# Aseeef/seq-align-gpu

Measured on AMD Instinct MI355X. Metric: GCUPS (DP cell updates/s) at 1/2/4/8 MI355X; bit-exact max scores vs CPU ref, higher is better.
Workload: dtype f16

## Files before the change

seq-align-gpu_amd/__init__.py:

```python
import ctypes as C
import os

import numpy as np

_HERE = os.path.dirname(os.path.abspath(__file__))
LIB_PATH = os.path.join(_HERE, "libswg.so")
DATA_DIR = os.path.join(_HERE, "data")
CLI_PATH = os.path.join(_HERE, "bin", "smith_waterman")

if not os.path.exists(LIB_PATH):
    raise ImportError(
        "libswg.so is not built: run `python seq-align-gpu_amd/build.py` "
        "(or __graft_entry__.build()); there is no Python/CPU fallback")

lib = C.CDLL(LIB_PATH, mode=C.RTLD_GLOBAL)

SWG_OK, SWG_ERR_ARG, SWG_ERR_HIP, SWG_ERR_NOMEM = 0, -1, -2, -3
SWG_ERR_STATE, SWG_ERR_RESIDUE, SWG_ERR_IO, SWG_ERR_NODEVICE = -4, -5, -6, -7

ABI_SYMBOLS = [
    "swg_create", "swg_destroy", "swg_last_error", "swg_global_error", "swg_abi_version", "swg_prune_last",
    "swg_set_option", "swg_set_scoring", "swg_set_query", "swg_set_query_pssm", "swg_db_pack", "swg_db_pack_shard", "swg_db_pack_shards", "swg_db_upload", "swg_db_view",
    "swg_db_free", "swg_db_save", "swg_db_load", "swg_db_count", "swg_db_total_count", "swg_db_residues",
    "swg_db_packed_bytes", "swg_db_order", "swg_search", "swg_search_begin", "swg_search_end", "swg_search_multi",
# ... 215 lines not shown
_sig("swg_synth_db_shard", C.c_int, [C.c_uint64, C.c_size_t, C.c_double, C.c_double, C.c_uint32, C.c_uint32,
                                     _vp, C.c_size_t, C.c_double, C.c_double, C.c_int, C.c_int,
                                     C.POINTER(_vp), C.POINTER(_vp), C.POINTER(_vp), C.POINTER(C.c_size_t),
                                     C.POINTER(C.c_uint64), C.POINTER(C.c_size_t)])
_sig("swg_synth_free", None, [_vp])
_sig("swg_pssm_load", C.c_int, [C.c_char_p, C.POINTER(Scoring), C.POINTER(_vp), C.POINTER(_vp), C.POINTER(C.c_size_t),
                                C.c_char_p, C.c_size_t])
_sig("swg_pssm_free", None, [_vp, _vp])
_sig("swg_debug_fail_alloc", None, [C.c_int])
_sig("swg_align_stats", C.c_int, [_vp, _vp, _vp, C.c_size_t, _vp, _vp])
_sig("swg_align_stats_multi", C.c_int, [_vp, _vp, _vp, _vp, C.c_size_t, _vp, C.c_size_t, _vp, _vp, _vp])
_sig("swg_align_stats_multi_pssm", C.c_int, [_vp, _vp, _vp, _vp, C.c_size_t, _vp, C.c_size_t, _vp, _vp, _vp])
_sig("swg_debug_bounds_last", C.c_int, [_vp, _vp])
_sig("swg_debug_sort_count", C.c_ulong, [])
_sig("swg_debug_engine", C.c_int, [_vp, C.c_size_t, C.c_int, C.c_int, _vp])
_sig("swg_debug_plan", C.c_int, [_vp, C.c_size_t, C.c_int, _vp])
_sig("swg_debug_plan_f16", C.c_int, [_vp, C.c_size_t, C.c_int, C.c_long, _vp])
_sig("swg_debug_plan_gapless", C.c_int, [_vp, C.c_size_t, C.c_int, _vp])
_sig("swg_debug_plan_forced", C.c_int, [_vp, C.c_size_t, C.c_int, C.c_long, C.c_long, C.c_long, C.c_int, C.c_long, C.c_int, _vp])
_sig("swg_debug_plan_streams", C.c_int, [_vp, _vp, _vp, C.c_size_t, C.c_int, C.c_long, C.c_long, C.c_long, C.c_long, _vp])
_sig("swg_debug_plan_systolic", C.c_int, [_vp, _vp, _vp, C.c_size_t, C.c_int, C.c_int, C.c_int, C.c_long, C.c_long, C.c_long, C.c_long, C.c_long, _vp])
_sig("swg_debug_systolic_variants", C.c_int, [C.c_int, _vp, C.c_size_t])
_sig("swg_debug_plan_batch", C.c_int, [_vp, C.c_size_t, C.c_size_t, C.c_int, C.c_int, C.c_int, C.c_long, C.c_long, C.c_long, _vp])
_sig("swg_debug_plan_lists", C.c_int, [_vp, C.c_size_t, C.c_size_t, C.c_int, C.c_int, C.c_long, C.c_long, C.c_long, _vp])
_sig("swg_debug_launch_log", None, [C.c_int])
_sig("swg_debug_launch_log_read", C.c_size_t, [_vp, C.c_size_t])
_sig("swg_debug_split", C.c_int, [_vp, C.c_size_t, C.c_uint64, _vp])
_sig("swg_debug_list_plan", C.c_int, [C.c_size_t, C.c_uint32, C.c_int, _vp, _vp])
_sig("swg_debug_pair_tokens", C.c_int, [_vp, _vp, C.c_int, _vp, C.c_size_t, C.POINTER(C.c_size_t)])
_sig("swg_debug_view_ranks", C.c_int, [_vp, _vp, C.c_size_t, _vp, C.POINTER(C.c_size_t)])
_sig("swg_debug_list_jobs", C.c_int, [_vp, _vp, _vp, C.c_size_t, _vp, C.c_size_t, C.POINTER(C.c_size_t), _vp])
_sig("swg_prune_last", C.c_int, [_vp, _vp])
_sig("swg_debug_prune_bound", C.c_int, [_vp, _vp, C.c_size_t, _vp, _vp, C.c_size_t, _vp, _vp])
_sig("swg_debug_prune_plan", C.c_int, [_vp, _vp])
_sig("swg_debug_prune_plan_above", C.c_int, [_vp, _vp])
_sig("swg_debug_above_multi_route", C.c_int, [C.c_long, C.c_int, C.c_int])
_sig("swg_debug_prune_stages", C.c_int, [_vp, _vp, C.c_size_t, C.POINTER(C.c_size_t)])
_sig("swg_debug_prune_kmer", C.c_int, [_vp, _vp, C.c_size_t, C.c_int, C.c_int, C.c_int, _vp, _vp, C.c_size_t, _vp, _vp])
_sig("swg_debug_prune_kmer_choice", C.c_int, [_vp, _vp])
_sig("swg_debug_prune_kmer_read", C.c_int, [_vp, _vp, C.c_int, _vp, _vp, C.c_size_t, _vp])
_sig("swg_debug_prune_kmer_seg", C.c_int, [_vp, _vp, C.c_size_t, C.c_int, C.c_int, C.c_int, C.c_int, _vp, _vp, C.c_size_t, _vp, _vp])
_sig("swg_debug_prune_kmer_choice_seg", C.c_int, [_vp, _vp])
_sig("swg_debug_prune_kmer_seg_read", C.c_int, [_vp, _vp, C.c_int, C.c_int, _vp, _vp, C.c_size_t, _vp])
_sig("swg_debug_prune_kmer_refine", C.c_int, [_vp, _vp, C.c_size_t, C.c_int, C.c_int, C.c_int, _vp, _vp, C.c_size_t, _vp, _vp])
_sig("swg_debug_prune_refine_choice", C.c_int, [_vp, _vp])
_sig("swg_debug_prune_refine_read", C.c_int, [_vp, _vp, C.c_int, _vp, _vp, _vp, C.c_size_t, _vp, C.c_size_t, _vp])
_sig("swg_debug_prune_stages3", C.c_int, [_vp, _vp, C.c_size_t, C.POINTER(C.c_size_t)])
_sig("swg_debug_prune_kmer_refine3", C.c_int, [_vp, _vp, C.c_size_t, C.c_int, C.c_int, C.c_int, _vp, _vp, C.c_size_t, _vp, _vp])
_sig("swg_debug_prune_refine3_choice", C.c_int, [_vp, _vp])
_sig("swg_debug_prune_kmer_refine4", C.c_int, [_vp, _vp, C.c_size_t, C.c_int, C.c_int, C.c_int, _vp, _vp, C.c_size_t, _vp])
_sig("swg_debug_prune_table_bits", C.c_int, [_vp, _vp, C.c_size_t, C.c_int])
_sig("swg_debug_prune_tables", C.c_int, [_vp, _vp])
_sig("swg_debug_prune_tables4", C.c_int, [_vp, _vp])
_sig("swg_debug_prune_refine4_read", C.c_int, [_vp, _vp, C.c_size_t, _vp])
_sig("swg_debug_prune_refine4_choice", C.c_int, [_vp, _vp])
_sig("swg_debug_prune_gate_choice", C.c_int, [_vp, _vp])
_sig("swg_debug_prune_gate", C.c_int, [_vp, _vp])
_sig("swg_debug_prune_stages5", C.c_int, [_vp, _vp, C.c_size_t, _vp])
_sig("swg_debug_prune_stages4", C.c_int, [_vp, _vp, C.c_size_t, C.POINTER(C.c_size_t)])
_sig("swg_debug_list_deal", C.c_int, [_vp, _vp, _vp, C.c_size_t, C.c_uint64, C.c_uint64, _vp, C.c_size_t, C.POINTER(C.c_size_t)])
_sig("swg_debug_calib_iters", C.c_int, [_vp, _vp, C.c_size_t, C.POINTER(C.c_size_t)])
_sig("swg_db_composition", C.c_int, [_vp, _vp, _vp])
_sig("swg_calibrate", C.c_int, [_vp, _vp, C.c_int, _vp])
_sig("swg_calibrate_multi", C.c_int, [_vp, _vp, _vp, C.c_size_t, _vp, C.c_int, _vp])
_sig("swg_calibrate_multi_pssm", C.c_int, [_vp, _vp, _vp, C.c_size_t, _vp, C.c_int, _vp])
_sig("swg_evalue", C.c_double, [_vp, C.c_uint64, C.c_int32])
_sig("swg_bitscore", C.c_double, [_vp, C.c_int32])
_sig("swg_evalue_min_score", C.c_int32, [_vp, C.c_uint64, C.c_double])
_sig("swg_synth_db_iid", C.c_int, [C.c_uint64, C.c_size_t, C.c_uint32, _vp, C.POINTER(_vp), C.POINTER(_vp)])
_sig("swg_gumbel_fit_hist", C.c_int, [_vp, C.c_size_t, C.POINTER(C.c_double), C.POINTER(C.c_double), C.POINTER(C.c_int)])
_sig("swg_matrix_lambda", C.c_int, [_vp, _vp, C.POINTER(C.c_double)])
_sig("swg_pssm_from_paths", C.c_int, [_vp, _vp, C.c_double, _vp, C.c_size_t, _vp, _vp, _vp, _vp, C.c_size_t, C.c_size_t, _vp, _vp, _vp])
_sig("swg_pssm_save", C.c_int, [C.c_char_p, _vp, _vp, C.c_size_t])
_sig("swg_pssm_build", C.c_int, [_vp, _vp, _vp, C.c_size_t, _vp, _vp, C.c_double, _vp, _vp, _vp])
_sig("swg_pssm_build_multi", C.c_int, [_vp, _vp, _vp, _vp, C.c_size_t, _vp, C.c_size_t, _vp, _vp, C.c_double, _vp, _vp, _vp])
_sig("swg_pssm_build_multi_pssm", C.c_int, [_vp, _vp, _vp, _vp, _vp, C.c_size_t, _vp, C.c_size_t, _vp, _vp, C.c_double, _vp, _vp, _vp])
_sig("swg_mask_params_default", None, [_vp])
_sig("swg_mask_tables", C.c_int, [_vp, _vp, C.POINTER(C.c_int64), C.POINTER(C.c_int64)])
_sig("swg_seg_mask", C.c_int, [_vp, C.c_size_t, _vp, _vp, C.POINTER(C.c_size_t)])
_sig("swg_seg_mask_segments", C.c_int, [_vp, C.c_size_t, _vp, _vp, C.POINTER(C.c_size_t), C.POINTER(C.c_size_t)])
_sig("swg_seg_mask_flat", C.c_int, [_vp, _vp, C.c_size_t, _vp, _vp])
_sig("swg_db_sequence", C.c_int, [_vp, C.c_uint32, _vp, C.c_size_t, C.POINTER(C.c_size_t)])
_sig("swg_db_mask", C.c_int, [_vp, _vp, _vp, C.POINTER(_vp)])
_sig("swg_db_mask_info", C.c_int, [_vp, _vp])
_sig("swg_debug_mask_fail_alloc", None, [C.c_int])


def _check(rc, ctx=None):
    if rc != SWG_OK:
        msg = lib.swg_last_error(ctx) if ctx else lib.swg_global_error()
        raise SwgError(rc, (msg or b"").decode("utf-8", "replace"))


def _i8(a):
    a = np.ascontiguousarray(a, dtype=np.int8)
    return a, a.ctypes.data_as(_vp)


def _pssm(pssm):
    a = np.asarray(pssm)
    if a.ndim != 2 or a.shape[1] != 32:
        raise ValueError("a PSSM is an (lq, 32) array, got shape %s" % (a.shape,))
    if a.dtype != np.int8 and a.size and (a.min() < -128 or a.max() > 127):
        raise ValueError("PSSM values must fit int8")
    p, pp = _i8(a)
    return p, pp, a.shape[0]
# ... 274 lines not shown


def debug_prune_kmer_choice(forced=0, pruned=1, lq=3000, pair_rows=1900000000, table_rate=0, fill_rate=0):
    a = np.array([forced, pruned, lq, pair_rows, table_rate, fill_rate], dtype=np.int64)
    out = np.zeros(1, dtype=np.int64)
    _check(lib.swg_debug_prune_kmer_choice(a.ctypes.data_as(_vp), out.ctypes.data_as(_vp)))
    return int(out[0])


KMER_MAX_SEGMENTS = 32
KMER_TABLE_BUDGET = 96 << 20


def debug_prune_kmer_seg(rows, query, gap_open, gap_extend, k, segments, flat, offsets, table=True):
    S = int(segments)
    return _prune_kmer_mirror(lib.swg_debug_prune_kmer_seg, rows, query, gap_open, gap_extend, (int(k), S), flat, offsets,
                              (KMER_CLASSES ** int(k), S) if table and k in (4, 5) and 1 <= S <= KMER_MAX_SEGMENTS else None)


def debug_prune_kmer_choice_seg(forced=0, segments=0, pruned=1, lq=3000, pair_rows=1900000000, table_rate=0, fill_rate=0):
    a = np.array([forced, pruned, lq, pair_rows, table_rate, fill_rate, segments], dtype=np.int64)
    out = np.zeros(4, dtype=np.int64)
    _check(lib.swg_debug_prune_kmer_choice_seg(a.ctypes.data_as(_vp), out.ctypes.data_as(_vp)))
    return int(out[0]), int(out[1]), int(out[2]), bool(out[3])


KMER_REFINE_SEGMENTS = 128
KMER_REFINE3_SEGMENTS = 256


def debug_prune_kmer_refine(rows, query, gap_open, gap_extend, segments, flat, offsets, table=True):
    S = int(segments)
    hook = lib.swg_debug_prune_kmer_refine3 if S == KMER_REFINE3_SEGMENTS else lib.swg_debug_prune_kmer_refine
    return _prune_kmer_mirror(hook, rows, query, gap_open, gap_extend, (S,), flat, offsets,
                              (KMER_CLASSES ** 4, S) if table and S in (32, 64, 128, 256) else None)


def debug_prune_kmer_refine4(rows, query, gap_open, gap_extend, segments, flat, offsets):
    r, rp = _i8(rows)
    lq = r.size // 32
    qp = None
    if query is not None:
        q, qp = _i8(query)
        lq = q.size
    f, fp = _i8(flat)
    off = np.ascontiguousarray(offsets, dtype=np.uint64)
    n = off.size - 1
    u = np.zeros(max(n, 1), dtype=np.uint64)
    _check(lib.swg_debug_prune_kmer_refine4(rp, qp, lq, int(gap_open), int(gap_extend), int(segments), fp, off.ctypes.data_as(_vp), n,
                                            u.ctypes.data_as(_vp)))
    return u[:n]


def debug_prune_table_bits(rows, query, k=4):
    r, rp = _i8(rows)
    lq = r.size // 32
    qp = None
    if query is not None:
        q, qp = _i8(query)
        lq = q.size
    rc = lib.swg_debug_prune_table_bits(rp, qp, lq, int(k))
    if rc < 0:
        _check(rc)
    return rc


def debug_prune_refine3_choice(forced=0, segments=0, refine=0, refine3=0, table_bits=8, pruned=1, lq=3000, pair_rows=1900000000,
                               table_rate=0, fill_rate=0):
    a = np.array([forced, pruned, lq, pair_rows, table_rate, fill_rate, segments, refine, refine3, table_bits], dtype=np.int64)
    out = np.zeros(4, dtype=np.int64)
    _check(lib.swg_debug_prune_refine3_choice(a.ctypes.data_as(_vp), out.ctypes.data_as(_vp)))
    return int(out[0]), int(out[1]), int(out[2]), int(out[3])


KMER_REFINE4_SEGMENTS = 256
PRUNE_REFINE4_FORCED = 5256


def debug_prune_refine4_choice(forced=0, segments=0, refine=0, refine3=0, refine4=0, table_bits=8, table_bits5=8, pruned=1, lq=3000,
                               pair_rows=1900000000, table_rate=0, fill_rate=0):
    a = np.array([forced, pruned, lq, pair_rows, table_rate, fill_rate, segments, refine, refine3, table_bits, refine4, table_bits5], dtype=np.int64)
    out = np.zeros(5, dtype=np.int64)
    _check(lib.swg_debug_prune_refine4_choice(a.ctypes.data_as(_vp), out.ctypes.data_as(_vp)))
    return tuple(int(v) for v in out)


def debug_prune_gate_choice(forced=0, segments=0, gate=0, pruned=1, lq=3000, pair_rows=1900000000, table_rate=0, fill_rate=0):
    a = np.array([forced, pruned, lq, pair_rows, table_rate, fill_rate, segments, 0, gate], dtype=np.int64)
    out = np.zeros(3, dtype=np.int64)
    _check(lib.swg_debug_prune_gate_choice(a.ctypes.data_as(_vp), out.ctypes.data_as(_vp)))
    return int(out[0]), int(out[1]), bool(out[2])


def debug_prune_refine_choice(forced=0, segments=0, refine=0, pruned=1, lq=3000, pair_rows=1900000000, table_rate=0, fill_rate=0):
    a = np.array([forced, pruned, lq, pair_rows, table_rate, fill_rate, segments, refine], dtype=np.int64)
    out = np.zeros(3, dtype=np.int64)
    _check(lib.swg_debug_prune_refine_choice(a.ctypes.data_as(_vp), out.ctypes.data_as(_vp)))
    return int(out[0]), int(out[1]), int(out[2])


def prune_list(bounds, begin, end, threshold):
    b = np.asarray(bounds)[begin:end]
    return (begin + np.nonzero(b >= threshold)[0]).astype(np.uint32)


PRUNE_PLAN_KEYS = ("mode", "k", "want_scores", "gap_open", "gap_extend", "bits", "use_diag", "n_classes", "work_queue", "both_forms",
                   "gapless", "batch", "range_pairs", "groups", "prune_head", "n_segments")


def debug_prune_plan(**ask):
    d = dict(mode=1, k=100, want_scores=0, gap_open=-2, gap_extend=-1, bits=16, use_diag=1, n_classes=1, work_queue=1, both_forms=0,
             gapless=0, batch=0, range_pairs=1000000, groups=1024, prune_head=4, n_segments=8)
    unknown = set(ask) - set(d)
    if unknown:
        raise TypeError("debug_prune_plan: unknown arguments %s" % sorted(unknown))
    d.update(ask)
    a = np.array([int(d[k]) for k in PRUNE_PLAN_KEYS], dtype=np.int64)
    out = np.zeros(2, dtype=np.int64)
    _check(lib.swg_debug_prune_plan(a.ctypes.data_as(_vp), out.ctypes.data_as(_vp)))
    return bool(out[0]), int(out[1])


PRUNE_PLAN_ABOVE_KEYS = ("mode", "gap_open", "gap_extend", "bits", "use_diag", "n_classes", "work_queue", "both_forms", "gapless", "batch",
                         "range_pairs", "groups", "n_segments", "prune_head")


def debug_prune_plan_above(**ask):
    d = dict(mode=1, gap_open=-2, gap_extend=-1, bits=16, use_diag=1, n_classes=1, work_queue=1, both_forms=0, gapless=0, batch=0,
             range_pairs=1000000, groups=1024, n_segments=8, prune_head=4)
    unknown = set(ask) - set(d)
    if unknown:
        raise TypeError("debug_prune_plan_above: unknown arguments %s" % sorted(unknown))
    d.update(ask)
    a = np.array([int(d[k]) for k in PRUNE_PLAN_ABOVE_KEYS], dtype=np.int64)
    out = np.zeros(2, dtype=np.int64)
    _check(lib.swg_debug_prune_plan_above(a.ctypes.data_as(_vp), out.ctypes.data_as(_vp)))
    return bool(out[0]), int(out[1])


def debug_above_multi_route(option=0, admitted=True, single_pruned=False):
    rc = lib.swg_debug_above_multi_route(int(option), 1 if admitted else 0, 1 if single_pruned else 0)
    if rc < 0:
        _check(rc)
    return rc


PRUNE_STAGE_QUEUED = ("threshold", "prefix_cut", "gate", "refine", "list")
_PRUNE_STAGE_BITS = ((0, "threshold"), (7, "bound"), (1, "prefix_cut"), (2, "gate"), (3, "refine"), (5, "refine3"), (6, "refine4"), (4, "list"))


def debug_prune_stages(segments, head_pairs=0, fixed=False, refine=0, prefix_cut=False, refine3=0, refine4=0, gate=False):
    head = [head_pairs, fixed, refine, prefix_cut, refine3, refine4] + ([1] if gate else [])
    a = np.array(head + [len(segments)] + [int(v) for sg in segments for v in sg], dtype=np.int64)
    out = np.zeros((2 * len(segments) + 1, 4), dtype=np.int64)
    n = C.c_size_t(0)
    hook = lib.swg_debug_prune_stages5 if gate else lib.swg_debug_prune_stages4
    _check(hook(a.ctypes.data_as(_vp), out.ctypes.data_as(_vp), out.shape[0], C.byref(n)))
    return [(int(b), int(e), int(sg), tuple(name for i, name in _PRUNE_STAGE_BITS if int(qd) >> i & 1))
            for b, e, sg, qd in out[:n.value]]


LAUNCH_FAMILIES = ("dyn", "lists", "q32", "qq", "streams", "systolic")


def debug_systolic_variants(bits):
    out = np.zeros((16, 2), dtype=np.int32)
    n = lib.swg_debug_systolic_variants(bits, out.ctypes.data_as(_vp), 16)
    assert 0 < n <= 16
    return [(int(k), int(w)) for k, w in out[:n]]


def debug_launch_log(on):
    lib.swg_debug_launch_log(1 if on else 0)


def debug_launch_log_read():
    seen = lib.swg_debug_launch_log_read(None, 0)
    out = np.zeros((max(seen, 1), 10), dtype=np.int32)
    lib.swg_debug_launch_log_read(out.ctypes.data_as(_vp), seen)
    kept = int(np.count_nonzero(out[:seen, 1]))
    if kept < seen:
        raise SwgError(SWG_ERR_STATE, "launch log: %d launches, %d kept" % (seen, kept))
    keys = ("family", "K", "G", "W", "form", "edges", "flag", "workgroups", "grid_rows", "list")
    recs = []
    for row in out[:seen]:
        r = dict(zip(keys, (int(v) for v in row)))
        r["family"] = LAUNCH_FAMILIES[r["family"]]
        r["fma"] = r["exact"] = r.pop("flag")
        recs.append(r)
    return recs


def synth_query(seed, lq):
    out = np.empty(lq, dtype=np.int8)
    lib.swg_synth_query(seed, lq, out.ctypes.data_as(_vp))
    return out


def hit_key(score, index):
    return int(lib.swg_hit_key(int(score), int(index)))


def key_hit(key):
    h = Hit()
    lib.swg_key_hit(int(key), C.byref(h))
    return int(h.score), int(h.index)


def topk_merge_keys(keys, k):
# ... 632 lines not shown
        t = np.zeros(KMER_CLASSES ** int(k), dtype=np.uint16) if k else None
        n = 0
        if bounds:
            _check(lib.swg_debug_prune_kmer_read(self.handle, db.handle, 0, None, None, 0, info.ctypes.data_as(_vp)), self.handle)
            n = int(info[2])
        b = np.zeros(max(n, 1), dtype=np.uint32) if bounds else None
        _check(lib.swg_debug_prune_kmer_read(self.handle, db.handle, int(k or 0), t.ctypes.data_as(_vp) if t is not None else None,
                                             b.ctypes.data_as(_vp) if b is not None else None, n, info.ctypes.data_as(_vp)), self.handle)
        return {"k": int(info[0]), "builds": int(info[1]), "pairs": int(info[2]), "table": t, "bounds": None if b is None else b[:int(info[2])]}

    def debug_prune_kmer_seg_read(self, db, k=None, segments=1, bounds=False):
        info = np.zeros(4, dtype=np.uint64)
        S = int(segments)
        t = np.zeros((KMER_CLASSES ** int(k), S), dtype=np.uint16) if k else None
        n = 0
        if bounds:
            _check(lib.swg_debug_prune_kmer_seg_read(self.handle, db.handle, 0, 0, None, None, 0, info.ctypes.data_as(_vp)), self.handle)
            n = int(info[2])
        b = np.zeros(max(n, 1), dtype=np.uint32) if bounds else None
        _check(lib.swg_debug_prune_kmer_seg_read(self.handle, db.handle, int(k or 0), S, t.ctypes.data_as(_vp) if t is not None else None,
                                                 b.ctypes.data_as(_vp) if b is not None else None, n, info.ctypes.data_as(_vp)), self.handle)
        return {"k": int(info[0]), "builds": int(info[1]), "pairs": int(info[2]), "segments": int(info[3]), "table": t,
                "bounds": None if b is None else b[:int(info[2])]}

    def debug_prune_refine_read(self, db, segments=None, arrays=True):
        info = np.zeros(7, dtype=np.uint64)
        _check(lib.swg_debug_prune_refine_read(self.handle, db.handle, 0, None, None, None, 0, None, 0, info.ctypes.data_as(_vp)), self.handle)
        n = int(info[2])
        if not arrays:
            return {"k": int(info[0]), "builds": int(info[1]), "pairs": n, "segments": int(info[3]), "refine": int(info[4]),
                    "refine_builds": int(info[5]), "table": None, "bounds": None, "stages": []}
        S = int(segments or 0)
        t = np.zeros((KMER_CLASSES ** 4, S), dtype=np.uint16) if S else None
        b = np.zeros(max(n, 1), dtype=np.uint32)
        l = np.zeros(max(n, 1), dtype=np.uint32)
        st = np.zeros((256, 4), dtype=np.uint32)
        _check(lib.swg_debug_prune_refine_read(self.handle, db.handle, S, t.ctypes.data_as(_vp) if t is not None else None, b.ctypes.data_as(_vp),
                                               l.ctypes.data_as(_vp), n, st.ctypes.data_as(_vp), 256, info.ctypes.data_as(_vp)), self.handle)
        stages = [(int(r[0]), int(r[1]), int(r[2]), l[int(r[0]):int(r[0]) + int(r[3])].copy()) for r in st[:int(info[6])]]
        return {"k": int(info[0]), "builds": int(info[1]), "pairs": n, "segments": int(info[3]), "refine": int(info[4]),
                "refine_builds": int(info[5]), "table": t, "bounds": b[:n], "stages": stages}

    def debug_prune_tables(self):
        out = np.zeros(7, dtype=np.int64)
        _check(lib.swg_debug_prune_tables(self.handle, out.ctypes.data_as(_vp)), self.handle)
        return {"refine3": int(out[0]), "refine3_builds": int(out[1]),
                "bits": dict(zip(("first4", "first5", "second", "third"), (int(v) for v in out[2:6]))), "auto_bits": int(out[6])}

    def debug_prune_tables4(self):
        out = np.zeros(4, dtype=np.int64)
        _check(lib.swg_debug_prune_tables4(self.handle, out.ctypes.data_as(_vp)), self.handle)
        return {"refine4": int(out[0]), "refine4_builds": int(out[1]), "bits": int(out[2]), "refused": bool(out[3])}

    def debug_prune_gate(self):
        out = np.zeros(1, dtype=np.int64)
        _check(lib.swg_debug_prune_gate(self.handle, out.ctypes.data_as(_vp)), self.handle)
        return bool(out[0])

    def debug_prune_refine4_read(self, blocks):
        b = np.ascontiguousarray(blocks, dtype=np.uint32)
        out = np.zeros((max(b.size, 1), KMER_REFINE4_SEGMENTS), dtype=np.uint16)
        _check(lib.swg_debug_prune_refine4_read(self.handle, b.ctypes.data_as(_vp), b.size, out.ctypes.data_as(_vp)), self.handle)
        return out[:b.size]

    def debug_bounds_last(self):
        out = np.zeros(4, dtype=np.uint32)
        _check(lib.swg_debug_bounds_last(self.handle, out.ctypes.data_as(_vp)), self.handle)
        return dict(zip(("kernel_pairs", "fallback_pairs", "launches", "column_limit"), (int(v) for v in out)))

    def _align_multi(self, fn, db, qflat, qoff, hits, want_ops, ops_stride, bounds=False, stats=False):
        nq = len(qoff) - 1
        if len(hits) != nq:
            raise ValueError("hits: %d rows for %d queries" % (len(hits), nq))
        k = max((len(row) for row in hits), default=0)
        arr = (Hit * max(nq * k, 1))()
        nh = (C.c_size_t * max(nq, 1))()
        for i, row in enumerate(hits):
            nh[i] = len(row)
            for j, (sc, ix) in enumerate(row):
                arr[i * k + j].score, arr[i * k + j].index = int(sc), int(ix)
        out = (Alignment * max(nq * k, 1))()
        stride = 0 if bounds else int(ops_stride if ops_stride is not None else
                                      lib.swg_align_ops_bound_multi(db.handle, qoff.ctypes.data_as(_vp), nq))
        ops = C.create_string_buffer(max(1, nq * k * stride)) if want_ops else None
        args = (self.handle, db.handle, qflat.ctypes.data_as(_vp), qoff.ctypes.data_as(_vp), nq, C.cast(arr, _vp), k,
                C.cast(nh, _vp), C.cast(out, _vp))
        if stats:
            cnt = (AlignCounts * max(nq * k, 1))()
            _check(fn(*args, C.cast(cnt, _vp)), self.handle)
            return [[self._stats_dict(out[i * k + j], cnt[i * k + j]) for j in range(len(row))] for i, row in enumerate(hits)]
        _check(fn(*args) if bounds else fn(*args, C.cast(ops, _vp) if want_ops else None, stride), self.handle)
        raw = ops.raw if want_ops else None
        res = []
        for i, row in enumerate(hits):
            r = []
            for j in range(len(row)):
                h = i * k + j
                a = {f: int(getattr(out[h], f)) for f, _ in Alignment._fields_ if f != "reserved"}
                if want_ops:
                    a["ops"] = raw[h * stride:h * stride + a["n_ops"]].decode()
                r.append(a)
            res.append(r)
        return res

    @staticmethod
    def _hit_keys(hits, k, n):
# ... 118 lines not shown
```

seq-align-gpu_amd/csrc/swg_api.cpp:

```cpp
#include "swg_host_internal.h"
#include "../../include/swg_host.h"

#include <algorithm>
#include <atomic>
#include <chrono>
#include <climits>
#include <cmath>
#include <cstdarg>
#include <cstdio>
#include <cstdlib>
#include <cstring>
#include <new>
#include <vector>

static thread_local std::string g_err;
static std::atomic<uint64_t> g_epoch{1};

int swg_set_global_error(int code, const char *fmt, ...)
{
    char buf[512];
    va_list ap;
    va_start(ap, fmt);
    vsnprintf(buf, sizeof buf, fmt, ap);
    va_end(ap);
// ... 139 lines not shown
    const bool timing = getenv("SWG_TIMING") != nullptr;
    clk::time_point tp = clk::now();
    auto lap = [&](const char *what) {
        if (!timing) return;
        const clk::time_point t = clk::now();
        fprintf(stderr, "[swg_create] %-44s %8.2f ms\n", what, std::chrono::duration<double, std::milli>(t - tp).count());
        tp = t;
    };
    if (timing) fprintf(stderr, "[swg_create] %-44s %8.2f ms\n", "hipGetDeviceCount (HIP runtime start-up)", std::chrono::duration<double, std::milli>(tp - t_enter).count());
    int rc = [&]() -> int {
        HIP_TRY(ctx, hipSetDevice(dev));
        hipDeviceProp_t prop;
        HIP_TRY(ctx, hipGetDeviceProperties(&prop, dev));
        ctx->n_cu = prop.multiProcessorCount;
        lap("hipSetDevice + device properties");
        HIP_TRY(ctx, hipStreamCreateWithFlags(&ctx->stream, hipStreamNonBlocking));
        lap("the fill stream");
        const int rs = ensure_slot(ctx, &ctx->slots[0]);
        if (rs != SWG_OK) return rs;
        lap("events + pinned buffers of one search slot");
        ctx->cur = &ctx->slots[0];
        HIP_TRY(ctx, hipMalloc(&ctx->d_sub, 32 * 32));
        lap("first device allocation");
        if (timing) {
            HIP_TRY(ctx, swg_launch_zero2(ctx->d_sub, 16, reinterpret_cast<uint8_t *>(ctx->d_sub) + 16, 16, ctx->stream));
            HIP_TRY(ctx, hipStreamSynchronize(ctx->stream));
            lap("first kernel launch (code object load)");
        }
        return SWG_OK;
    }();
    if (rc != SWG_OK) {
        g_err = ctx->err;
        swg_destroy(ctx);
        return rc;
    }
    *out = ctx;
    return SWG_OK;
}

extern "C" void swg_destroy(swg_ctx *ctx)
{
    if (!ctx) return;
    (void)hipSetDevice(ctx->device);
    if (ctx->stream) (void)hipStreamSynchronize(ctx->stream);
    (void)hipFree(ctx->d_sub);
    (void)hipFree(ctx->d_query);
    (void)hipFree(ctx->d_pssm);
    (void)hipFree(ctx->d_kmer_cprof);
    (void)hipFree(ctx->kmer_first[0].d);
    (void)hipFree(ctx->kmer_first[1].d);
    (void)hipFree(ctx->kmer_second.d);
    (void)hipFree(ctx->kmer_third.d);
    (void)hipFree(ctx->kmer_fourth.d);
    (void)hipFree(ctx->d_profile[0]);
    (void)hipFree(ctx->d_profile[1]);
    (void)hipFree(ctx->d_profile[2]);
    (void)hipFree(ctx->d_profile[3]);
    (void)hipFree(ctx->d_profile[4]);
    (void)hipFree(ctx->d_profile[5]);
    (void)hipFree(ctx->d_profile[6]);
    (void)hipFree(ctx->d_profile[7]);
    (void)hipFree(ctx->d_scratch);
    for (SwgSlot &sl : ctx->slots) {
        for (auto &ev : sl.ev)
            if (ev) (void)hipEventDestroy(ev);
        if (sl.ev_done) (void)hipEventDestroy(sl.ev_done);
        (void)hipHostFree(sl.h_cand);
        (void)hipHostFree(sl.h_counters);
        (void)hipHostFree(sl.h_scores);
    }
    if (ctx->b16.db) swg_db_free(ctx->b16.db);
    if (ctx->calib.db) swg_db_free(ctx->calib.db);
    (void)hipHostFree(ctx->b16.h_stage);
    (void)hipHostFree(ctx->b16.h_meta);
    (void)hipFree(ctx->b16.d_stage);
    (void)hipFree(ctx->b16.d_pair_src);
    (void)hipFree(ctx->b16.d_pair_len);
    for (int i = 0; i < 4; ++i) {
        (void)hipHostFree(ctx->h_query_stage[i]);
        if (ctx->ev_query_stage[i]) (void)hipEventDestroy(ctx->ev_query_stage[i]);
    }
    if (ctx->stream2) (void)hipStreamDestroy(ctx->stream2);
    if (ctx->stream3) (void)hipStreamDestroy(ctx->stream3);
    if (ctx->stream) (void)hipStreamDestroy(ctx->stream);
    delete ctx;
}

extern "C" int swg_set_option(swg_ctx *ctx, const char *key, long value)
{
    if (!ctx || !key) return swg_set_ctx_error(ctx, SWG_ERR_ARG, "swg_set_option: NULL argument");
    if (!strcmp(key, "force_bits")) {
        if (value != 0 && value != 16 && value != 32)
            return swg_set_ctx_error(ctx, SWG_ERR_ARG, "force_bits must be 0, 16 or 32");
        ctx->opt_force_bits = value;
    } else if (!strcmp(key, "cols_per_wave")) {
        ctx->opt_cols = value;
    } else if (!strcmp(key, "max_waves")) {
        if (value < 0 || value > 16) return swg_set_ctx_error(ctx, SWG_ERR_ARG, "max_waves must be 0..16");
        ctx->opt_max_waves = value;
    } else if (!strcmp(key, "engine")) {
        if (value < 0 || value > 2) return swg_set_ctx_error(ctx, SWG_ERR_ARG, "engine must be 0 (auto), 1 (systolic) or 2 (diagonal)");
        ctx->opt_engine = value;
    } else if (!strcmp(key, "group_lanes")) {
        if (value != 0 && value != 16 && value != 32 && value != 64)
            return swg_set_ctx_error(ctx, SWG_ERR_ARG, "group_lanes must be 0, 16, 32 or 64");
        ctx->opt_group = value;
// ... 10 lines not shown
    } else if (!strcmp(key, "wide16")) {
        ctx->opt_wide = value != 0;
    } else if (!strcmp(key, "f16")) {
        if (value < 0 || value > 2) return swg_set_ctx_error(ctx, SWG_ERR_ARG, "f16 must be 0 (off), 1 (auto) or 2 (whenever the gap scores allow)");
        ctx->opt_f16 = value;
    } else if (!strcmp(key, "f16_pair")) {
        if (value < 0 || value > 2)
            return swg_set_ctx_error(ctx, SWG_ERR_ARG, "f16_pair must be 0 (auto), 1 (v_perm_b32) or 2 (v_pk_fma_f16 wherever it fits)");
        ctx->opt_f16_pair = value;
    } else if (!strcmp(key, "bounds_groups")) {
        if (value < 0) return swg_set_ctx_error(ctx, SWG_ERR_ARG, "bounds_groups must be 0 (auto) or the most lane groups of a bounds launch");
        ctx->opt_bounds_groups = value;
    } else if (!strcmp(key, "last_pass")) {
        ctx->opt_last_pass = value != 0;
    } else if (!strcmp(key, "qq")) {
        ctx->opt_qq = value != 0;
    } else if (!strcmp(key, "batch_geometry")) {
        if (value != 0 && value != 1)
            return swg_set_ctx_error(ctx, SWG_ERR_ARG, "batch_geometry must be 0 (a forced geometry sends a batch one by one) or 1 (the batch takes it)");
        ctx->opt_batch_geometry = value;
    } else if (!strcmp(key, "long_helps")) {
        ctx->opt_long_helps = value != 0;
    } else if (!strcmp(key, "segment_blocks")) {
        if (value < 0 || value > (long)SWG_DYN_SEG_BLOCKS)
            return swg_set_ctx_error(ctx, SWG_ERR_ARG, "segment_blocks must be 0 (default) .. 2^26-64");
        ctx->opt_seg_blocks = value ? (uint32_t)value : SWG_DYN_SEG_BLOCKS;
    } else if (!strcmp(key, "prune")) {
        if (value < 0 || value > 2)
            return swg_set_ctx_error(ctx, SWG_ERR_ARG, "prune must be 0 (off), 1 (auto) or 2 (wherever it is structurally possible: diagnostic)");
        ctx->opt_prune = value;
    } else if (!strcmp(key, "prune_head")) {
        if (value < 0 || value > 4096) return swg_set_ctx_error(ctx, SWG_ERR_ARG, "prune_head must be 0..4096 (pairs per lane group)");
        ctx->opt_prune_head = value;
    } else if (!strcmp(key, "prune_kmer")) {
        if (value != 0 && value != 1 && value != 4 && value != 5)
            return swg_set_ctx_error(ctx, SWG_ERR_ARG, "prune_kmer must be 0 (auto), 1 (the colmax bound), 4 or 5 (the k-mer bound of that k)");
        ctx->opt_prune_kmer = value;
    } else if (!strcmp(key, "prune_segments")) {
        if (value < 0 || value > (long)SWG_KMER_MAX_SEGMENTS)
            return swg_set_ctx_error(ctx, SWG_ERR_ARG, "prune_segments must be 0 (auto) or 1..32 (the segments of the k-mer bound's table; 1: unsegmented)");
        ctx->opt_prune_segments = value;
    } else if (!strcmp(key, "prune_refine")) {
        if (!swg_prune_refine_value_ok(value))
            return swg_set_ctx_error(ctx, SWG_ERR_ARG, "prune_refine must be 0 (auto), 1 (off), 64 or 128 (the segments of the second-level bound's table)");
        ctx->opt_prune_refine = value;
    } else if (!strcmp(key, "prune_refine3")) {
        if (!swg_prune_refine3_value_ok(value))
            return swg_set_ctx_error(ctx, SWG_ERR_ARG, "prune_refine3 must be 0 (auto), 1 (off) or 256 (the segments of the third-level bound's table)");
        ctx->opt_prune_refine3 = value;
    } else if (!strcmp(key, "prune_refine4")) {
        if (!swg_prune_refine4_value_ok(value))
            return swg_set_ctx_error(ctx, SWG_ERR_ARG, "prune_refine4 must be 0 (auto), 1 (off) or 5256 (the fourth-level bound's table: k = 5 in 256 segments)");
        ctx->opt_prune_refine4 = value;
    } else if (!strcmp(key, "prune_gate")) {
        if (!swg_prune_gate_value_ok(value))
            return swg_set_ctx_error(ctx, SWG_ERR_ARG, "prune_gate must be 0 (auto), 1 (off) or 2 (wherever the first-level bound is a segmented k-mer bound)");
        ctx->opt_prune_gate = value;
    } else if (!strcmp(key, "prune_table_bits")) {
        if (value != 0 && value != 16)
            return swg_set_ctx_error(ctx, SWG_ERR_ARG, "prune_table_bits must be 0 (auto: bytes where they hold every entry) or 16");
        ctx->opt_prune_table_bits = value;
    } else if (!strcmp(key, "prune_cut")) {
        if (value != 0 && value != 1)
            return swg_set_ctx_error(ctx, SWG_ERR_ARG, "prune_cut must be 0 (a stage's pairs are cut one by one) or 1 (the prefix of the length order)");
        ctx->opt_prune_cut = value;
    } else if (!strcmp(key, "above_batch")) {
        if (value < 0 || value > 2)
            return swg_set_ctx_error(ctx, SWG_ERR_ARG, "above_batch must be 0 (auto), 1 (one launch wherever the batch is admitted) or 2 (one query after another)");
        ctx->opt_above_batch = value;
    } else if (!strcmp(key, "calib_seqs")) {
        if (value < 2 || value > (1l << 20)) return swg_set_ctx_error(ctx, SWG_ERR_ARG, "calib_seqs must be 2..1048576 (random sequences a calibration scores)");
        ctx->opt_calib_seqs = value;
    } else if (!strcmp(key, "pssm_msa_mb")) {
        if (value < 0 || value > 65536) return swg_set_ctx_error(ctx, SWG_ERR_ARG, "pssm_msa_mb must be 0..65536 (MiB of device rows one group of queries of swg_pssm_build* may take; 0: every query alone)");
        ctx->opt_pssm_msa_mb = value;
    } else if (!strcmp(key, "calib_len")) {
        if (value < 8 || value > (1l << 14)) return swg_set_ctx_error(ctx, SWG_ERR_ARG, "calib_len must be 8..16384 (residues of a calibration's random sequences)");
        ctx->opt_calib_len = value;
    } else if (!strcmp(key, "calib_seed")) {
        if (value < 0) return swg_set_ctx_error(ctx, SWG_ERR_ARG, "calib_seed must be >= 0");
        ctx->opt_calib_seed = value;
    } else if (!strcmp(key, "q32_waves")) {
        ctx->opt_q32_waves = value;
    } else if (!strcmp(key, "wave_budget")) {
        ctx->opt_wave_budget = value;
    } else if (!strcmp(key, "batch")) {
        if (value < 0 || value > 8) return swg_set_ctx_error(ctx, SWG_ERR_ARG, "batch must be 0..8 (pairs one queue request claims; 0 and 1: one)");
        ctx->opt_batch = value;
    } else if (!strcmp(key, "batch_blocks")) {
        if (value < 0) return swg_set_ctx_error(ctx, SWG_ERR_ARG, "batch_blocks must be >= 0 (token blocks; 0: from the geometry)");
        ctx->opt_batch_blocks = value;
    } else if (!strcmp(key, "work_queue")) {
        ctx->opt_dynamic = value != 0;
    } else if (!strcmp(key, "prio_share")) {
        if (value < 0) return swg_set_ctx_error(ctx, SWG_ERR_ARG, "prio_share must be >= 0 (percent)");
        ctx->opt_prio_share = value;
    } else if (!strcmp(key, "long_split")) {
        if (value < -1) return swg_set_ctx_error(ctx, SWG_ERR_ARG, "long_split must be -1 (off), 0 (auto) or a row count");
        ctx->opt_long_split = value;
    } else if (!strcmp(key, "workgroups")) {
        if (value < 0) return swg_set_ctx_error(ctx, SWG_ERR_ARG, "workgroups must be >= 0");
        ctx->opt_workgroups = value;
    } else {
        return swg_set_ctx_error(ctx, SWG_ERR_ARG, "swg_set_option: unknown key '%s'", key);
    }
    return SWG_OK;
// ... 734 lines not shown
    if (F->cut) {
        q.q2_begin = q.q2_end = 0;
        q.queue2 = nullptr;
    }
    return SWG_OK;
}

static int enqueue_pruned_fill(swg_ctx *ctx, swg_db *db, const SwgPrunePlan &pr, size_t k, DynFill *F)
{
    const SwgPairTokens &T = db->ptok;
    const SwgDiagPlan &pl = F->wk.plan[F->c];
    hipStream_t qs = F->qs;
    uint32_t *thr = db->d_counters + SWG_PRUNE_WORD_T, *cut_word = db->d_counters + SWG_PRUNE_WORD_CUT, *gate = db->d_counters + SWG_PRUNE_WORD_GATE;
    const uint32_t n_pairs = (uint32_t)swg_db_pair_count(db);
    const SwgPruneLayout L = swg_prune_layout(db->d_pair_bound, n_pairs);
    if (pr.fixed) HIP_TRY(ctx, hipMemsetD32Async(reinterpret_cast<hipDeviceptr_t>(thr), (int)pr.fixed_T, 1, qs));
    const std::vector<SwgPruneStage> stages = swg_prune_stages(pr, F->segs);
    auto first_level = [&](uint32_t b, uint32_t en, const uint32_t *gated_by) -> int {
        if (pr.kmer > 1 && pr.segments > 1)
            HIP_TRY(ctx, swg_launch_pair_bound_kmer_seg(T.d_tok, T.d_pair_off, b, en, pr.kmer, (uint32_t)pr.segments, ctx->prune_colmax, ctx->kmer_first[pr.kmer - 4].d,
                                                        ctx->kmer_first[pr.kmer - 4].bits, gated_by, L.bounds, L.ids, qs));
        else if (pr.kmer > 1)
            HIP_TRY(ctx, swg_launch_pair_bound_kmer(T.d_tok, T.d_pair_off, en, pr.kmer, ctx->prune_colmax, ctx->kmer_first[pr.kmer - 4].d,
                                                    ctx->kmer_first[pr.kmer - 4].bits, L.bounds, L.ids, qs));
        else
            HIP_TRY(ctx, swg_launch_pair_bound(T.d_tok, T.d_pair_off, en, ctx->prune_colmax, L.bounds, L.ids, qs));
        return SWG_OK;
    };
    const SwgPruneBoundRange br = swg_prune_bound_range(stages, n_pairs);
    if (br.stage == stages.size()) {
        const int rc = first_level(br.begin, br.end, nullptr);
        if (rc != SWG_OK) return rc;
    } else if (br.skip_end > br.skip_begin)
        HIP_TRY(ctx, hipMemsetD32Async(reinterpret_cast<hipDeviceptr_t>(L.bounds + br.skip_begin), (int)SWG_PRUNE_NOT_BOUNDED, br.skip_end - br.skip_begin, qs));
    db->prune_stages.clear();
    for (const SwgPruneStage &st : stages) {
        if (st.queued & SWG_STAGE_THRESHOLD)
            HIP_TRY(ctx, swg_launch_prune_threshold(db->d_scores, db->d_order, (uint32_t)((size_t)db->n_bins * SWG_BIN), (uint32_t)k, db->d_hist, thr, qs));
        if (st.queued & SWG_STAGE_BOUND) {
            const int rc = first_level(br.begin, br.end, thr);
            if (rc != SWG_OK) return rc;
        }
        if (st.queued & SWG_STAGE_PREFIX_CUT) HIP_TRY(ctx, swg_launch_prune_cut(L.bounds, T.d_pair_off, st.begin, st.end, thr, cut_word, qs));
        if (st.queued & SWG_STAGE_GATE) HIP_TRY(ctx, swg_launch_prune_refine_gate(L.bounds, st.begin, st.end, thr, gate, qs));
        if (st.queued & SWG_STAGE_REFINE)
            HIP_TRY(ctx, swg_launch_pair_bound_refine(T.d_tok, T.d_pair_off, st.begin, st.end, (uint32_t)pr.refine, ctx->prune_colmax, ctx->kmer_second.d,
                                                      ctx->kmer_second.bits, st.queued & SWG_STAGE_GATE ? gate : thr, L.bounds, qs));
        if (st.queued & SWG_STAGE_REFINE3)
            HIP_TRY(ctx, swg_launch_pair_bound_refine(T.d_tok, T.d_pair_off, st.begin, st.end, (uint32_t)pr.refine3, ctx->prune_colmax, ctx->kmer_third.d,
                                                      ctx->kmer_third.bits, st.queued & SWG_STAGE_GATE ? gate : thr, L.bounds, qs));
        if (st.queued & SWG_STAGE_REFINE4)
            HIP_TRY(ctx, swg_launch_pair_bound_refine(T.d_tok, T.d_pair_off, st.begin, st.end, (uint32_t)pr.refine4, ctx->prune_colmax, ctx->kmer_fourth.d,
                                                      ctx->kmer_fourth.bits, st.queued & SWG_STAGE_GATE ? gate : thr, L.bounds, qs, 5));
        if (st.queued & SWG_STAGE_LIST) {
            const size_t rec = db->prune_stages.size() / 2;
            HIP_TRY(ctx, swg_launch_prune_list(L.bounds, T.d_pair_off, st.begin, st.end, thr, L.tiles, L.lists + st.begin, cut_word,
                                               rec < SWG_PRUNE_STAGE_RECS ? L.recs + 2 * rec : nullptr, qs));
            db->prune_stages.push_back(st.begin), db->prune_stages.push_back(st.end);
        }
        F->q.list = st.queued & SWG_STAGE_PREFIX_CUT ? L.ids + st.begin : st.queued & SWG_STAGE_LIST ? L.lists + st.begin : nullptr;
        F->q.list_count = F->q.list ? cut_word : nullptr;
        for (int pass = 0; pass < pl.npass; ++pass) {
            const int rc = F->launch(pass, F->segs[st.segment], st.begin, st.end, F->form, ctx->d_profile[diag_profile_slot(pl, F->c)], false);
            if (rc != SWG_OK) return rc;
        }
    }
    F->q.list = nullptr, F->q.list_count = nullptr;
    return SWG_OK;
}

static int launch_diag(swg_ctx *ctx, swg_db *db, const SwgDiagWork &wk, int go, int ge, bool *two_ends,
                       const SwgPrunePlan *prune = nullptr, size_t prune_k = 0)
{
    hipStream_t s = ctx->stream;
    *two_ends = false;
    static const char *trace_path = getenv("SWG_TRACE");
    uint64_t *d_trace[2] = {nullptr, nullptr};
    if (trace_path)
        for (int c = 0; c < wk.n_classes; ++c) {
            const size_t bytes = (size_t)wk.plan[c].workgroups * wk.plan[c].W * 4 * 8;
            HIP_TRY(ctx, hipMalloc(&d_trace[c], bytes));
            HIP_TRY(ctx, hipMemsetAsync(d_trace[c], 0, bytes, s));
        }
    HIP_TRY(ctx, hipEventRecord(ctx->cur->ev[1], s));
    int rf = fork_long_class(ctx, wk);
    if (rf != SWG_OK) return rf;
    for (int c = wk.n_classes - 1; c >= 0; --c) {
        const SwgDiagLayout &L = db->diag[c];
        const SwgDiagPlan &pl = wk.plan[c];
        if (diag_class_is_dynamic(ctx, db, pl)) {
            DynFill F{ctx, db, wk, c};
            int rc = dyn_fill_begin(&F, go, ge, d_trace[c]);
            if (rc != SWG_OK) return rc;
            const uint32_t class_begin = F.q.q_begin, class_end = F.q.q_end;
            const bool split = c == 0 && wk.n_classes == 1 && F.form != 2 && pl.f16_from > class_begin && pl.f16_from < class_end;
            const bool pruned = prune && prune->on && c == 0 && wk.n_classes == 1 && !split && db->d_pair_bound;
            if (c == 0) ctx->cur->pruned = pruned;
            if (pruned) {
                if ((rc = enqueue_pruned_fill(ctx, db, *prune, prune_k, &F)) != SWG_OK) return rc;
            } else
            for (int part = 0; part < (split ? 2 : 1); ++part) {
                const int pform = split && part == 1 ? 2 : F.form;
                const uint32_t part_begin = split && part == 1 ? pl.f16_from : class_begin;
                const uint32_t part_end = split && part == 0 ? pl.f16_from : class_end;
                const uint8_t *prof = ctx->d_profile[split && part == 1 ? 7 : diag_profile_slot(pl, c)];
                F.q.go = gap_word(pform, go);
// ... 823 lines not shown
{
    P->prune = SwgPrunePlan();
    if (!P->use_diag || P->bits != 16) return SWG_OK;
    const SwgDiagWork &wk = P->wk;
    const SwgDiagPlan &pl = wk.plan[0];
    SwgPruneAsk a;
    a.mode = (int)ctx->opt_prune;
    a.k = k;
    a.want_scores = want_scores;
    a.gap_open = ctx->gap_open;
    a.gap_extend = ctx->gap_extend;
    a.bits = P->bits;
    a.use_diag = P->use_diag;
    a.n_classes = wk.n_classes;
    a.work_queue = diag_class_is_dynamic(ctx, db, pl) && db->ptok.ok;
    a.both_forms = P->split_at != 0u;
    a.gapless = P->gapless;
    a.batch = ctx->in_batch;
    a.prune_head = ctx->opt_prune_head;
    a.fixed = ctx->above_min > 0;
    if (a.mode == 0 || !a.work_queue || wk.n_classes != 1) return SWG_OK;
    a.range_pairs = wk.pair_end[0] - wk.pair_begin[0];
    a.groups = diag_class_streams(ctx, db, wk, 0);
    const int form = diag_class_form(ctx, db, pl);
    std::vector<std::pair<uint32_t, uint32_t>> segs;
    bool cut = false;
    if (!token_segments(db->ptok, (uint32_t)wk.pair_begin[0], (uint32_t)wk.pair_end[0], ctx->opt_seg_blocks, pl.npass > 1 || form == 1, &segs, &cut))
        return SWG_OK;
    a.n_segments = segs.size();
    P->prune = swg_prune_plan(a);
    ctx->prune_choice = SwgPruneChoice();
    if (!P->prune.on) return SWG_OK;
    P->prune.fixed_T = P->prune.fixed ? (uint32_t)ctx->above_min : 0u;
    SwgKmerAsk ka;
    ka.forced = ctx->opt_prune_kmer;
    ka.forced_segments = ctx->opt_prune_segments;
    ka.forced_refine = ctx->opt_prune_refine;
    ka.forced_refine3 = ctx->opt_prune_refine3;
    ka.forced_refine4 = ctx->opt_prune_refine4;
    ensure_prune_colmax(ctx);
    ka.table_bits = kmer_table_bits(ctx, 4);
    ka.table_bits5 = kmer_table_bits(ctx, 5);
    ka.pruned = true;
    ka.lq = ctx->query_len();
    ka.pair_rows = 4ull * (db->ptok.pair_blocks_prefix[wk.pair_end[0]] - db->ptok.pair_blocks_prefix[wk.pair_begin[0]]);
    ka.fill_rate = swg_kmer_fill_rate(ka.lq);
    P->prune.kmer = swg_prune_kmer_choice(ka, &P->prune.segments);
    P->prune.prefix_cut = ctx->opt_prune_cut == 1 && !P->prune.fixed;
    P->prune.refine = P->prune.prefix_cut ? 0 : swg_prune_refine_choice(ka, P->prune.kmer, P->prune.segments);
    P->prune.refine3 = P->prune.prefix_cut ? 0 : swg_prune_refine3_choice(ka, P->prune.kmer, P->prune.segments, P->prune.refine);
    P->prune.refine4 = P->prune.prefix_cut || ctx->kmer_fourth_refused
                           ? 0
                           : swg_prune_refine4_choice(ka, P->prune.kmer, P->prune.segments, P->prune.refine, P->prune.refine3);
    ka.forced_gate = ctx->opt_prune_gate;
    P->prune.gate = !P->prune.prefix_cut && swg_prune_gate_choice(ka, P->prune.kmer, P->prune.segments);
    ctx->prune_choice = SwgPruneChoice{P->prune.kmer, P->prune.segments, P->prune.refine, P->prune.refine3, P->prune.refine4, P->prune.gate ? 1 : 0};
    return SWG_OK;
}

static int ensure_kmer_table(swg_ctx *ctx, SwgKmerTable *t, int k, int S)
{
    const int bits = kmer_table_bits(ctx, k);
    if (t->holds(ctx->epoch, k, S, bits)) return SWG_OK;
    const size_t lq = ctx->query_len();
    int rc;
    if ((rc = device_grow(ctx, &ctx->d_kmer_cprof, &ctx->d_kmer_cprof_cap, lq * 32)) != SWG_OK) return rc;
    const size_t bytes = (size_t)swg_kmer_entries(k) * (size_t)S * (size_t)(bits / 8);
    if (t->cap < bytes) t->epoch = 0;
    if ((rc = device_grow(ctx, &t->d, &t->cap, bytes)) != SWG_OK) return rc;
    const long go = (long)ctx->gap_open + ctx->gap_extend, ge = ctx->gap_extend;
    HIP_TRY(ctx, swg_launch_kmer_table(ctx->d_sub, ctx->d_query, ctx->query_pssm ? ctx->d_pssm : nullptr, (uint32_t)lq, (uint32_t)-go, (uint32_t)-ge, k,
                                       (uint32_t)S, ctx->d_kmer_cprof, t->d, bits, ctx->stream));
    t->epoch = ctx->epoch, t->k = k, t->segments = S, t->bits = bits;
    ++(t == &ctx->kmer_fourth  ? ctx->kmer_refine4_builds
       : t == &ctx->kmer_third ? ctx->kmer_refine3_builds
       : t == &ctx->kmer_second ? ctx->kmer_refine_builds
                                : ctx->kmer_builds);
    return SWG_OK;
}

static bool reserve_kmer_fourth(swg_ctx *ctx)
{
    SwgKmerTable *t = &ctx->kmer_fourth;
    const size_t bytes = (size_t)swg_kmer_entries(5) * SWG_KMER_REFINE4_SEGMENTS;
    if (t->d && t->cap >= bytes) return true;
    (void)hipFree(t->d);
    t->d = nullptr, t->cap = 0, t->epoch = 0;
    uint8_t *d = nullptr;
    if (hipSetDevice(ctx->device) != hipSuccess || hipMalloc(&d, bytes) != hipSuccess) {
        (void)hipGetLastError();
        ctx->kmer_fourth_refused = true;
        return false;
    }
    t->d = d, t->cap = bytes;
    return true;
}

static int prepare_prune(swg_ctx *ctx, swg_db *db, const SwgPrunePlan &pr)
{
    int rc;
    ensure_prune_colmax(ctx);
    if (pr.kmer > 1) {
        const int k = pr.kmer, S = pr.segments;
        if (S < 1 || S > (int)SWG_KMER_MAX_SEGMENTS) return swg_set_ctx_error(ctx, SWG_ERR_ARG, "the k-mer bound's table: %d segments (1..32)", S);
        if (!swg_kmer_table_admitted(k, S))
            return swg_set_ctx_error(ctx, SWG_ERR_ARG, "the k-mer bound's table of k = %d in %d segments is %zu MB: above its budget of %zu MB (prune_kmer, prune_segments)", k,
                                     S, (size_t)swg_kmer_entries(k) * (size_t)S * sizeof(uint16_t) >> 20, (size_t)(SWG_KMER_TABLE_BUDGET >> 20));
        if ((rc = ensure_kmer_table(ctx, &ctx->kmer_first[k - 4], k, S)) != SWG_OK) return rc;
    }
    if (pr.refine) {
        if (pr.refine != 64 && pr.refine != 128) return swg_set_ctx_error(ctx, SWG_ERR_ARG, "the second-level bound's table: %d segments (64 or 128)", pr.refine);
        if ((rc = ensure_kmer_table(ctx, &ctx->kmer_second, 4, pr.refine)) != SWG_OK) return rc;
    }
    if (pr.refine3) {
        if (pr.refine3 != 256) return swg_set_ctx_error(ctx, SWG_ERR_ARG, "the third-level bound's table: %d segments (256)", pr.refine3);
        if ((rc = ensure_kmer_table(ctx, &ctx->kmer_third, 4, pr.refine3)) != SWG_OK) return rc;
    }
    if (pr.refine4) {
        if (pr.refine4 != (int)SWG_KMER_REFINE4_SEGMENTS || !swg_kmer_refine4_admitted(kmer_table_bits(ctx, 5)))
            return swg_set_ctx_error(ctx, SWG_ERR_ARG, "the fourth-level bound's table: %d segments (256) of bytes", pr.refine4);
        if ((rc = ensure_kmer_table(ctx, &ctx->kmer_fourth, 5, pr.refine4)) != SWG_OK) return rc;
    }
    swg_db::Bufs &b = db->bufs[ctx->cur - ctx->slots];
    const size_t n_pairs = (size_t)swg_db_pair_count(db);
    if ((rc = device_grow(ctx, &b.d_pair_bound, &b.pair_bound_cap, n_pairs, swg_prune_layout(b.d_pair_bound, n_pairs).words - n_pairs)) != SWG_OK) return rc;
    db->d_pair_bound = b.d_pair_bound;
    return SWG_OK;
}

static int prepare_search(swg_ctx *ctx, swg_db *db, const SwgSearchPlan &P)
{
    int rc = SWG_OK;
    const bool systolic_fill = !P.use_diag && !P.use_q32 && !(P.bits == 32 && P.use_diag32);
    const bool systolic_rescore = P.may_saturate && !P.use_diag32;
    const size_t bin32_scratch = P.bin32 && P.npass32 > 1 ? ((size_t)db->max_nblk * 4 + 4) * 4 * 16 * (size_t)ctx->n_cu : 0;
    if (P.bin32) {
        rc = ensure_profile_cols(ctx, 1, (uint32_t)(P.npass32 * 64 * SWG_DIAG32_K), 4, (1ull << 30) ^ (uint64_t)P.npass32);
        if (rc != SWG_OK) return rc;
        if ((rc = ensure_scratch(ctx, bin32_scratch)) != SWG_OK) return rc;
    }
    if (P.use_diag) {
        if ((rc = prepare_diag(ctx, db, P.wk)) == SWG_OK && P.prune.on) rc = prepare_prune(ctx, db, P.prune);
    } else if (systolic_fill) rc = ensure_profile(ctx, P.main_pl);
    if (rc != SWG_OK) return rc;
    if (systolic_rescore && (rc = ensure_profile(ctx, P.re_pl)) != SWG_OK) return rc;
    size_t need = bin32_scratch;
    if (systolic_fill && P.main_pl.npass > 1)
        need = std::max(need, (size_t)P.main_pl.workgroups * db->max_nblk * SWG_ROWS_PER_BLK * 64 * P.main_pl.info.nb);
    if (systolic_rescore && P.re_pl.npass > 1)
        need = std::max(need, (size_t)P.re_pl.workgroups * db->max_nblk * SWG_ROWS_PER_BLK * 64 * P.re_pl.info.nb);
    if ((rc = ensure_scratch(ctx, need)) != SWG_OK) return rc;
    if ((!P.use_diag && !P.use_q32) || (P.int32_level && !P.q32_ok)) return ensure_bins(ctx, db);
    return SWG_OK;
}

static int enqueue_fill(swg_ctx *ctx, swg_db *db, const SwgSearchPlan &P, SwgSlot *S)
{
    hipStream_t s = ctx->stream;
    const size_t n_slots = (size_t)db->n_bins * SWG_BIN;
    HIP_TRY(ctx, hipEventRecord(S->ev[0], s));
    HIP_TRY(ctx, swg_launch_zero2(db->d_scores, n_slots * 4, db->d_counters, SWG_COUNTER_BYTES, s));
    S->two_ends = false;
    S->fill_launches = 0;
    S->pruned = false;
    if (P.use_diag) return launch_diag(ctx, db, P.wk, P.go, P.ge, &S->two_ends, &P.prune, S->k);
    if (P.use_q32)
        return launch_q32(ctx, db, P.wk32, P.go, P.ge, nullptr, nullptr, 0, db->d_counters + SWG_QUEUE_WORD(0), &S->two_ends, true, P.exact32);
    if (!(P.bits == 32 && P.use_diag32)) return launch_systolic(ctx, db, P.main_pl, P.go, P.ge);
    SwgFillParams p = fill_params_base(ctx, db);
    p.profile = ctx->d_profile[1];
    p.queue = db->d_counters + SWG_WORD_WORK_QUEUE;
    p.n_items = (uint32_t)n_slots;
    p.npass = (uint32_t)P.npass32;
    p.go = P.go;
// ... 79 lines not shown
    }
    ++ctx->n_begun;
    S->dev_topk = k > 0 && !S->want_scores && k <= SWG_TOPK_CAND_CAP / 2;
    S->above_min = ctx->above_min;
    if (S->above_min > 0) {
        const swg_db::Bufs &b = db->bufs[S - ctx->slots];
        S->above_cap = b.d_above ? b.above_cap : SWG_ABOVE_KEYS_FLOOR;
        HIP_TRY(ctx, swg_launch_above_compact(db->d_scores, db->d_order, (uint32_t)n_slots, S->above_min, b.d_above ? b.d_above : db->d_keys,
                                              (uint32_t)S->above_cap, db->d_counters + SWG_ABOVE_WORD_COUNT, s));
    }
    if (S->dev_topk)
        HIP_TRY(ctx, swg_launch_topk(db->d_scores, db->d_order, (uint32_t)n_slots, (uint32_t)k, db->d_hist,
                                     db->d_counters + SWG_WORD_TOPK_THR, db->d_keys, SWG_TOPK_CAND_CAP, db->d_counters + SWG_WORD_TOPK_COUNT, s));
    HIP_TRY(ctx, hipEventRecord(S->ev[4], s));
    S->need_scores = S->want_scores || (k > 0 && !S->dev_topk);
    S->first_chunk = SWG_TOPK_CAND_CAP;
    if (S->dev_topk)
        HIP_TRY(ctx, hipMemcpyAsync(S->h_cand, db->d_keys, S->first_chunk * 8, hipMemcpyDeviceToHost, s));
    if (S->need_scores) {
        const int rc = slot_scores(ctx, S, n_slots);
        if (rc != SWG_OK) return rc;
        HIP_TRY(ctx, hipMemcpyAsync(S->h_scores, db->d_scores, n_slots * 4, hipMemcpyDeviceToHost, s));
    }
    HIP_TRY(ctx, hipMemcpyAsync(S->h_counters, db->d_counters, 128, hipMemcpyDeviceToHost, s));
    HIP_TRY(ctx, hipEventRecord(S->ev_done, s));
    return SWG_OK;
}

static int search_begin(swg_ctx *ctx, swg_db *db, bool want_scores, size_t k, bool allow_autotune, SwgSlot *S)
{
    if (!ctx || !db) return swg_set_ctx_error(ctx, SWG_ERR_ARG, "swg_search: NULL argument");
    if (!ctx->have_scoring) return swg_set_ctx_error(ctx, SWG_ERR_STATE, "swg_search: no scoring set");
    if (ctx->query_len() == 0) return swg_set_ctx_error(ctx, SWG_ERR_STATE, "swg_search: no query set");
    if (db->device != ctx->device || !db->d_codes)
        return swg_set_ctx_error(ctx, SWG_ERR_STATE, "swg_search: database is not resident on device %d",
                                 ctx->device);
    HIP_TRY(ctx, hipSetDevice(ctx->device));
    int rc = ensure_slot(ctx, S);
    if (rc != SWG_OK) return rc;
    ctx->cur = S;
    if ((rc = select_bufs(ctx, db, (int)(S - ctx->slots))) != SWG_OK) return rc;
    S->bufs = db->bufs[S - ctx->slots];
    S->db = db;
    S->k = k;
    S->want_scores = want_scores;
    memset(&S->st, 0, sizeof S->st);
    S->st.cells = (uint64_t)ctx->query_len() * db->residues;
    S->st.bytes_alg = db->residues + 8ull * db->n_local + 32ull * ctx->query_len() + 1024ull;
    S->plan = SwgSearchPlan();
    if (db->n_bins == 0) return SWG_OK;
    if ((rc = plan_search(ctx, db, allow_autotune, &S->plan)) != SWG_OK) return rc;
    if ((rc = plan_prune(ctx, db, want_scores, k, &S->plan)) != SWG_OK) return rc;
    if (S->plan.prune.refine4 && !reserve_kmer_fourth(ctx)) S->plan.prune.refine4 = 0, ctx->prune_choice.refine4 = 0;
    if ((rc = prepare_search(ctx, db, S->plan)) != SWG_OK) return rc;
    if ((rc = enqueue_fill(ctx, db, S->plan, S)) != SWG_OK) return rc;
    if ((rc = enqueue_rescore(ctx, db, S->plan, S)) != SWG_OK) return rc;
    return enqueue_readout(ctx, db, S);
}

static void deliver_scores(const swg_db *db, const int32_t *h_scores, size_t n_slots, int32_t *scores_out, swg_hit *topk_out,
                           size_t k, size_t *n_hits)
{
    if (scores_out)
        for (size_t i = 0; i < n_slots; ++i) {
            const uint32_t oi = db->order[i];
            if (oi != 0xFFFFFFFFu) scores_out[oi] = h_scores[i];
        }
    if (k > 0 && topk_out) {
        std::vector<uint64_t> keys;
        keys.reserve(db->n_local);
        for (size_t i = 0; i < n_slots; ++i) {
            const uint32_t oi = db->order[i];
            if (oi != 0xFFFFFFFFu) keys.push_back(swg_hit_key(h_scores[i], oi));
        }
        const size_t m = std::min(k, keys.size());
        std::partial_sort(keys.begin(), keys.begin() + m, keys.end(), std::greater<uint64_t>());
        for (size_t i = 0; i < m; ++i) swg_key_hit(keys[i], &topk_out[i]);
        if (n_hits) *n_hits = m;
    } else if (n_hits) {
        *n_hits = 0;
    }
}

struct SwgAboveOut {
    swg_hit *hits_out = nullptr;
    size_t cap = 0;
    uint64_t n_total = 0;
};

static int deliver_above(swg_ctx *ctx, SwgSlot *S, hipStream_t s, SwgAboveOut *out, size_t *n_hits)
{
    swg_db *db = S->db;
    const size_t n_slots = (size_t)db->n_bins * SWG_BIN;
    const size_t count = S->h_counters[SWG_ABOVE_WORD_COUNT], kept = std::min(count, S->above_cap);
    out->n_total = count;
    const size_t m = std::min(out->cap, count);
    if (count > S->above_cap) {
        swg_db::Bufs &b = db->bufs[S - ctx->slots];
        const size_t want = std::min<size_t>(db->n_local, std::max<size_t>(count + count / 4, 2 * (size_t)SWG_ABOVE_KEYS_FLOOR));
        uint64_t *grown = nullptr;
        if (hipMalloc(&grown, want * 8) == hipSuccess) {
            (void)hipFree(b.d_above);
            b.d_above = grown;
            b.above_cap = want;
        } else
            (void)hipGetLastError();
// ... 210 lines not shown
            const size_t n = std::min<size_t>(std::min<size_t>(db->prune_stages.size() / 2, SWG_PRUNE_STAGE_RECS), stages_cap);
            std::vector<uint32_t> recs(2 * n);
            if (n) HIP_TRY(ctx, hipMemcpy(recs.data(), L.recs, 2 * n * sizeof(uint32_t), hipMemcpyDeviceToHost));
            for (size_t i = 0; i < n; ++i)
                stages_out[4 * i] = db->prune_stages[2 * i], stages_out[4 * i + 1] = db->prune_stages[2 * i + 1], stages_out[4 * i + 2] = recs[2 * i],
                               stages_out[4 * i + 3] = recs[2 * i + 1];
            info[6] = n;
        }
    }
    return SWG_OK;
}
extern "C" int swg_debug_prune_kmer_read(swg_ctx *ctx, const swg_db *db, int k, uint16_t *table_out, uint32_t *bound_out, size_t bound_cap,
                                         uint64_t *info)
{
    return debug_prune_read(ctx, db, "swg_debug_prune_kmer_read", ctx && (k == 4 || k == 5) ? &ctx->kmer_first[k - 4] : nullptr, k, 1, table_out, bound_out, nullptr,
                            bound_cap, nullptr, 0, 3, info);
}
extern "C" int swg_debug_prune_kmer_seg_read(swg_ctx *ctx, const swg_db *db, int k, int S, uint16_t *table_out, uint32_t *bound_out, size_t bound_cap,
                                             uint64_t *info)
{
    return debug_prune_read(ctx, db, "swg_debug_prune_kmer_seg_read", ctx && (k == 4 || k == 5) ? &ctx->kmer_first[k - 4] : nullptr, k, S, table_out, bound_out, nullptr,
                            bound_cap, nullptr, 0, 4, info);
}
extern "C" int swg_debug_prune_refine_read(swg_ctx *ctx, const swg_db *db, int S2, uint16_t *table_out, uint32_t *bound_out, uint32_t *list_out, size_t pair_cap,
                                           uint32_t *stages_out, size_t stages_cap, uint64_t *info)
{
    return debug_prune_read(ctx, db, "swg_debug_prune_refine_read", ctx ? (S2 == 256 ? &ctx->kmer_third : &ctx->kmer_second) : nullptr, 4, S2, table_out, bound_out,
                            list_out, pair_cap, stages_out, stages_cap, 7, info);
}
extern "C" int swg_debug_prune_tables(swg_ctx *ctx, int64_t *out)
{
    if (!ctx || !out) return swg_set_ctx_error(ctx, SWG_ERR_ARG, "swg_debug_prune_tables: NULL argument");
    const SwgKmerTable *t[4] = {&ctx->kmer_first[0], &ctx->kmer_first[1], &ctx->kmer_second, &ctx->kmer_third};
    out[0] = ctx->prune_choice.refine3;
    out[1] = (int64_t)ctx->kmer_refine3_builds;
    for (int i = 0; i < 4; ++i) out[2 + i] = t[i]->d && t[i]->epoch == ctx->epoch ? t[i]->bits : 0;
    out[6] = 0;
    if (ctx->query_len() > 0) {
        ensure_prune_colmax(ctx);
        out[6] = swg_kmer_table_bits(ctx->prune_colmax, 4);
    }
    return SWG_OK;
}

extern "C" int swg_debug_prune_tables4(swg_ctx *ctx, int64_t *out)
{
    if (!ctx || !out) return swg_set_ctx_error(ctx, SWG_ERR_ARG, "swg_debug_prune_tables4: NULL argument");
    out[0] = ctx->prune_choice.refine4;
    out[1] = (int64_t)ctx->kmer_refine4_builds;
    out[2] = ctx->kmer_fourth.d && ctx->kmer_fourth.epoch == ctx->epoch ? ctx->kmer_fourth.bits : 0;
    out[3] = ctx->kmer_fourth_refused ? 1 : 0;
    return SWG_OK;
}
extern "C" int swg_debug_prune_gate(swg_ctx *ctx, int64_t *out)
{
    if (!ctx || !out) return swg_set_ctx_error(ctx, SWG_ERR_ARG, "swg_debug_prune_gate: NULL argument");
    out[0] = ctx->prune_choice.gate;
    return SWG_OK;
}
extern "C" int swg_debug_prune_refine4_read(swg_ctx *ctx, const uint32_t *blocks, size_t n, uint16_t *out)
{
    if (!ctx || (n > 0 && (!blocks || !out))) return swg_set_ctx_error(ctx, SWG_ERR_ARG, "swg_debug_prune_refine4_read: NULL argument");
    const SwgKmerTable &t = ctx->kmer_fourth;
    HIP_TRY(ctx, hipSetDevice(ctx->device));
    HIP_TRY(ctx, hipDeviceSynchronize());
    if (!t.holds(ctx->epoch, 5, (int)SWG_KMER_REFINE4_SEGMENTS, 8))
        return swg_set_ctx_error(ctx, SWG_ERR_STATE, "swg_debug_prune_refine4_read: no fourth-level table for the current query and scoring");
    uint8_t row[SWG_KMER_REFINE4_SEGMENTS];
    for (size_t i = 0; i < n; ++i) {
        if (blocks[i] >= swg_kmer_entries(5)) return swg_set_ctx_error(ctx, SWG_ERR_ARG, "swg_debug_prune_refine4_read: block %u", blocks[i]);
        HIP_TRY(ctx, hipMemcpy(row, t.d + (size_t)blocks[i] * SWG_KMER_REFINE4_SEGMENTS, sizeof row, hipMemcpyDeviceToHost));
        std::copy(row, row + SWG_KMER_REFINE4_SEGMENTS, out + i * SWG_KMER_REFINE4_SEGMENTS);
    }
    return SWG_OK;
}

extern "C" int swg_prune_last(const swg_ctx *ctx, swg_prune_info *out)
{
    if (!ctx || !out) return SWG_ERR_ARG;
    *out = ctx->prune_last;
    return SWG_OK;
}

static int search_begin_ticket(swg_ctx *ctx, swg_db *db, bool want_scores, size_t k, bool allow_autotune, int *ticket)
{
    return ctx_guarded(ctx, "swg_search_begin", [&]() -> int {
        fail_alloc_here(1);
        if (!ctx || !db || !ticket) return swg_set_ctx_error(ctx, SWG_ERR_ARG, "swg_search_begin: NULL argument");
        int slot = -1;
        for (int i = 0; i < SWG_MAX_INFLIGHT; ++i) {
            const int c = (ctx->next_slot + i) % SWG_MAX_INFLIGHT;
            if (!ctx->slots[c].busy) {
                slot = c;
                break;
            }
        }
        if (slot < 0)
            return swg_set_ctx_error(ctx, SWG_ERR_STATE, "swg_search_begin: %d searches already in flight", SWG_MAX_INFLIGHT);
        const int rc = search_begin(ctx, db, want_scores, k, allow_autotune, &ctx->slots[slot]);
        if (rc != SWG_OK) return rc;
        ctx->slots[slot].busy = true;
        ctx->next_slot = (slot + 1) % SWG_MAX_INFLIGHT;
        *ticket = slot;
        return SWG_OK;
    });
}

extern "C" int swg_search_begin(swg_ctx *ctx, const swg_db *db, int want_scores, size_t k, int *ticket)
{
    return search_begin_ticket(ctx, const_cast<swg_db *>(db), want_scores != 0, k, ctx && ctx->opt_autotune != 0, ticket);
}

extern "C" int swg_search_end(swg_ctx *ctx, int ticket, int32_t *scores_out, swg_hit *topk_out, size_t *n_hits,
                              swg_stats *stats)
{
    bool valid = false;
    const int rc = ctx_guarded(ctx, "swg_search_end", [&]() -> int {
        fail_alloc_here(2);
        if (!ctx || ticket < 0 || ticket >= SWG_MAX_INFLIGHT || !ctx->slots[ticket].busy)
            return swg_set_ctx_error(ctx, SWG_ERR_ARG, "swg_search_end: no search in flight under that ticket");
        valid = true;
        return search_end(ctx, &ctx->slots[ticket], scores_out, topk_out, n_hits, stats);
    });
// ... 1835 lines not shown
```

seq-align-gpu_amd/csrc/swg_diag_host.cpp:

```cpp
#include "swg_host_internal.h"
#include "../../include/swg_host.h"

#include <algorithm>
#include <atomic>
#include <cmath>
#include <cstring>
#include <mutex>
#include <queue>

static std::mutex g_plan_cache_mutex;

static const double kCyclesPerInstr[5] = {0.0, 6.8, 4.55, 4.27, 4.35};
static const double kHotCycles = 13.0;

uint64_t swg_db_pair_count(const swg_db *db) { return (db->n_local + 1) / 2; }

uint64_t swg_db_pair_rows(const swg_db *db, uint64_t pair_begin, uint64_t pair_end, uint64_t *longest_rows)
{
    const uint64_t n = swg_db_pair_count(db);
    std::vector<uint64_t> &pre = const_cast<swg_db *>(db)->pair_rows_prefix;
    if (pre.size() != n + 1) {
        pre.assign(n + 1, 0);
        for (uint64_t p = 0; p < n; ++p) pre[p + 1] = pre[p] + 2ull + db->lens[2 * p];
    }
// ... 491 lines not shown
    }
    r.on = true;
    r.head_pairs = (uint32_t)head;
    return r;
}

extern "C" int swg_debug_prune_plan(const int64_t *in, int64_t *out)
{
    if (!in || !out || in[1] < 0 || in[12] < 0 || in[13] < 0 || in[15] < 0) return SWG_ERR_ARG;
    SwgPruneAsk a;
    a.mode = (int)in[0], a.k = (size_t)in[1], a.want_scores = in[2] != 0, a.gap_open = (int)in[3], a.gap_extend = (int)in[4];
    a.bits = (int)in[5], a.use_diag = in[6] != 0, a.n_classes = (int)in[7], a.work_queue = in[8] != 0, a.both_forms = in[9] != 0;
    a.gapless = in[10] != 0, a.batch = in[11] != 0, a.range_pairs = (uint64_t)in[12], a.groups = (uint64_t)in[13], a.prune_head = (long)in[14];
    a.n_segments = (size_t)in[15];
    const SwgPrunePlan r = swg_prune_plan(a);
    out[0] = r.on ? 1 : 0;
    out[1] = (int64_t)r.head_pairs;
    return SWG_OK;
}

extern "C" int swg_debug_prune_plan_above(const int64_t *in, int64_t *out)
{
    if (!in || !out || in[10] < 0 || in[11] < 0 || in[12] < 0) return SWG_ERR_ARG;
    SwgPruneAsk a;
    a.fixed = true;
    a.mode = (int)in[0], a.gap_open = (int)in[1], a.gap_extend = (int)in[2], a.bits = (int)in[3], a.use_diag = in[4] != 0, a.n_classes = (int)in[5];
    a.work_queue = in[6] != 0, a.both_forms = in[7] != 0, a.gapless = in[8] != 0, a.batch = in[9] != 0, a.range_pairs = (uint64_t)in[10];
    a.groups = (uint64_t)in[11], a.n_segments = (size_t)in[12], a.prune_head = (long)in[13];
    const SwgPrunePlan r = swg_prune_plan(a);
    out[0] = r.on ? 1 : 0;
    out[1] = (int64_t)r.head_pairs;
    return SWG_OK;
}

std::vector<SwgPruneStage> swg_prune_stages(const SwgPrunePlan &plan, const std::vector<std::pair<uint32_t, uint32_t>> &segments)
{
    std::vector<SwgPruneStage> stages;
    for (size_t i = 0; i < segments.size(); ++i) {
        const uint32_t b = segments[i].first, en = segments[i].second;
        const uint32_t mid = segments.size() == 1 && plan.head_pairs > 0 ? std::min(en, b + plan.head_pairs) : en;
        stages.push_back(SwgPruneStage{b, mid, (uint32_t)i, 0u});
        if (mid < en) stages.push_back(SwgPruneStage{mid, en, (uint32_t)i, 0u});
    }
    for (size_t si = 0; si < stages.size(); ++si) {
        if (si == 0 && !plan.fixed) continue;
        uint32_t q = plan.fixed ? 0u : SWG_STAGE_THRESHOLD;
        if (plan.gate && si == (plan.fixed ? 0u : 1u)) q |= SWG_STAGE_BOUND;
        if (plan.prefix_cut) q |= SWG_STAGE_PREFIX_CUT;
        else {
            if (plan.refine && plan.fixed && si == 0 && stages.size() > 1) q |= SWG_STAGE_GATE;
            if (plan.refine) q |= SWG_STAGE_REFINE;
            if (plan.refine3) q |= SWG_STAGE_REFINE3;
            if (plan.refine4) q |= SWG_STAGE_REFINE4;
            q |= SWG_STAGE_LIST;
        }
        stages[si].queued = q;
    }
    return stages;
}

SwgPruneBoundRange swg_prune_bound_range(const std::vector<SwgPruneStage> &stages, uint32_t n_pairs)
{
    for (size_t i = 0; i < stages.size(); ++i)
        if (stages[i].queued & SWG_STAGE_BOUND) return SwgPruneBoundRange{i, stages[i].begin, stages.back().end, stages.front().begin, stages[i].begin};
    return SwgPruneBoundRange{stages.size(), 0u, n_pairs, 0u, 0u};
}

static int debug_prune_stages(const int64_t *in, int head, int64_t *out, size_t cap, size_t *n_out)
{
    if (!in || !n_out || (cap > 0 && !out) || in[0] < 0 || in[head - 1] < 0) return SWG_ERR_ARG;
    SwgPrunePlan plan;
    plan.on = true;
    plan.head_pairs = (uint32_t)in[0], plan.fixed = in[1] != 0, plan.refine = (int)in[2], plan.prefix_cut = in[3] != 0;
    plan.refine3 = head >= 6 ? (int)in[4] : 0;
    plan.refine4 = head >= 7 ? (int)in[5] : 0;
    plan.gate = head == 8 && in[6] != 0;
    std::vector<std::pair<uint32_t, uint32_t>> segments;
    for (int64_t i = 0; i < in[head - 1]; ++i) segments.emplace_back((uint32_t)in[head + 2 * i], (uint32_t)in[head + 1 + 2 * i]);
    const std::vector<SwgPruneStage> stages = swg_prune_stages(plan, segments);
    for (size_t i = 0; i < stages.size() && i < cap; ++i)
        out[4 * i] = stages[i].begin, out[4 * i + 1] = stages[i].end, out[4 * i + 2] = stages[i].segment, out[4 * i + 3] = stages[i].queued;
    *n_out = stages.size();
    return SWG_OK;
}
extern "C" int swg_debug_prune_stages(const int64_t *in, int64_t *out, size_t cap, size_t *n_out) { return debug_prune_stages(in, 5, out, cap, n_out); }
extern "C" int swg_debug_prune_stages3(const int64_t *in, int64_t *out, size_t cap, size_t *n_out) { return debug_prune_stages(in, 6, out, cap, n_out); }
extern "C" int swg_debug_prune_stages4(const int64_t *in, int64_t *out, size_t cap, size_t *n_out) { return debug_prune_stages(in, 7, out, cap, n_out); }
extern "C" int swg_debug_prune_stages5(const int64_t *in, int64_t *out, size_t cap, size_t *n_out) { return debug_prune_stages(in, 8, out, cap, n_out); }

void swg_kmer_cprof(const int8_t *rows, const int8_t *idx, size_t lq, int8_t *cprof)
{
    for (size_t i = 0; i < lq; ++i) {
        const int8_t *row = idx ? rows + 32 * ((uint8_t)idx[i] & 31) : rows + 32 * i;
        int8_t *out = cprof + SWG_KMER_CLASSES * i;
        for (uint32_t c = 0; c < SWG_KMER_CLASSES; ++c) out[c] = SWG_KMER_PAD_SCORE;
        for (uint32_t r = 1; r < 32; ++r) {
            const uint32_t c = swg_kmer_class(r);
            out[c] = std::max(out[c], row[r]);
        }
    }
}

static void kmer_row(const int8_t *cprof, size_t lq, int g, int e, size_t S, uint32_t c, const int *Mp, const int *Bp, const int *best_p, int *Mn,
                     int *Bn, int *best)
{
    const size_t W = (lq + S - 1) / S;
    int a = 0, up = 0;
    for (size_t s = 0; s < S; ++s) best[s] = best_p ? best_p[s] : 0;
    for (size_t s = 0, i = 0; i < lq; ++s) {
        int bs = best[s];
        for (const size_t end = std::min(lq, i + W); i < end; ++i) {
            const int sc = cprof[SWG_KMER_CLASSES * i + c];
            a = std::max(std::max(up - g, a - e), 0);
            const int b = Mp ? std::max(std::max(Mp[i] - g, Bp[i] - e), 0) : 0;
            const int diag = Mp && i ? Mp[i - 1] : 0;
            const int m = std::max(std::max(diag + sc, a), b);
            Mn[i] = m, Bn[i] = b, up = m;
            bs = std::max(bs, m);
        }
        best[s] = bs;
    }
}

static void kmer_extend(const int8_t *cprof, size_t lq, int g, int e, int k, size_t S, int depth, size_t prefix, const int *Mp, const int *Bp,
                        const int *best_p, std::vector<int> &work, uint16_t *table, uint32_t c_begin, uint32_t c_end)
{
    int *Mn = work.data() + (size_t)depth * (2 * lq + S), *Bn = Mn + lq, *best = Bn + lq;
    for (uint32_t c = c_begin; c < c_end; ++c) {
        kmer_row(cprof, lq, g, e, S, c, depth ? Mp : nullptr, Bp, best_p, Mn, Bn, best);
        const size_t at = prefix * SWG_KMER_CLASSES + c;
        if (depth + 1 == k)
            for (size_t s = 0; s < S; ++s) table[at * S + s] = (uint16_t)std::min(best[s], 65535);
        else kmer_extend(cprof, lq, g, e, k, S, depth + 1, at, Mn, Bn, best, work, table, 0, SWG_KMER_CLASSES);
    }
}

void swg_kmer_table_seg(const int8_t *cprof, size_t lq, int g, int e, int k, size_t S, uint16_t *table)
{
    g = std::min(g, 65536), e = std::min(e, 65536);
#pragma omp parallel for schedule(dynamic, 1)
    for (int c = 0; c < (int)SWG_KMER_CLASSES; ++c) {
        std::vector<int> work((size_t)k * (2 * lq + S));
        kmer_extend(cprof, lq, g, e, k, S, 0, 0, nullptr, nullptr, nullptr, work, table, (uint32_t)c, (uint32_t)c + 1u);
    }
}

template <class Entries>
static uint64_t kmer_bound_walk(Entries entries, int k, size_t S, const SwgColMax &cm, const int8_t *seq, size_t len)
{
    const size_t n_blocks = (2 + len + 3) / 4, n_rows = 4 * n_blocks;
    auto res = [&](size_t row) -> uint32_t { return row < 2 || row >= 2 + len ? 0u : (uint8_t)seq[row - 2] & 31u; };
    const size_t rows5 = k == 5 ? 20 * (n_blocks / 5) : 0;
    std::vector<uint64_t> H(S, 0);
    for (size_t r = 0; r < n_rows;) {
        const size_t rows = r < rows5 ? 5 : 4;
        size_t ix = 0;
        uint64_t sum = 0, run = 0;
        for (size_t j = 0; j < rows; ++j) ix = ix * SWG_KMER_CLASSES + swg_kmer_class(res(r + j)), sum += cm.v[res(r + j)];
        if (k == 5 && rows == 4) ix *= SWG_KMER_CLASSES;
        const uint16_t *t = entries(ix);
        for (size_t s = 0; s < S; ++s) {
            run = std::max(run, H[s]);
            H[s] = run + std::min<uint64_t>(t[s], sum);
        }
        r += rows;
    }
    return *std::max_element(H.begin(), H.end());
}

uint64_t swg_kmer_bound_seg(const uint16_t *table, int k, size_t S, const SwgColMax &cm, const int8_t *seq, size_t len)
{
    return kmer_bound_walk([&](size_t ix) { return table + ix * S; }, k, S, cm, seq, len);
}

static int debug_prune_kmer(bool admitted, const int8_t *rows, const int8_t *idx, size_t lq, int gap_open, int gap_extend, int k, int S,
                            const int8_t *flat, const uint64_t *offsets, size_t n, uint16_t *table_out, uint64_t *u_out)
{
    if (!admitted || !rows || lq == 0 || gap_open > 0 || gap_extend > 0 || (n > 0 && (!flat || !offsets || !u_out))) return SWG_ERR_ARG;
    std::vector<int8_t> cprof(lq * SWG_KMER_CLASSES);
    swg_kmer_cprof(rows, idx, lq, cprof.data());
    std::vector<uint16_t> own;
    if (!table_out) {
        own.resize(swg_kmer_entries(k) * (size_t)S);
        table_out = own.data();
    }
    swg_kmer_table_seg(cprof.data(), lq, -(gap_open + gap_extend), -gap_extend, k, (size_t)S, table_out);
    const SwgColMax cm = swg_prune_colmax(rows, idx, lq);
    for (size_t i = 0; i < n; ++i) u_out[i] = swg_kmer_bound_seg(table_out, k, (size_t)S, cm, flat + offsets[i], (size_t)(offsets[i + 1] - offsets[i]));
    return SWG_OK;
}
extern "C" int swg_debug_prune_kmer(const int8_t *rows, const int8_t *idx, size_t lq, int gap_open, int gap_extend, int k, const int8_t *flat,
                                    const uint64_t *offsets, size_t n, uint16_t *table_out, uint64_t *u_out)
{
    return debug_prune_kmer(k == 4 || k == 5, rows, idx, lq, gap_open, gap_extend, k, 1, flat, offsets, n, table_out, u_out);
}
extern "C" int swg_debug_prune_kmer_seg(const int8_t *rows, const int8_t *idx, size_t lq, int gap_open, int gap_extend, int k, int S,
                                        const int8_t *flat, const uint64_t *offsets, size_t n, uint16_t *table_out, uint64_t *u_out)
{
    return debug_prune_kmer((k == 4 || k == 5) && S >= 1 && S <= (int)SWG_KMER_MAX_SEGMENTS, rows, idx, lq, gap_open, gap_extend, k, S, flat, offsets, n,
                            table_out, u_out);
}
extern "C" int swg_debug_prune_kmer_refine(const int8_t *rows, const int8_t *idx, size_t lq, int gap_open, int gap_extend, int S2, const int8_t *flat,
                                           const uint64_t *offsets, size_t n, uint16_t *table_out, uint64_t *u_out)
{
    return debug_prune_kmer(S2 == 32 || S2 == 64 || S2 == 128, rows, idx, lq, gap_open, gap_extend, 4, S2, flat, offsets, n, table_out, u_out);
}
extern "C" int swg_debug_prune_kmer_refine3(const int8_t *rows, const int8_t *idx, size_t lq, int gap_open, int gap_extend, int S3, const int8_t *flat,
                                            const uint64_t *offsets, size_t n, uint16_t *table_out, uint64_t *u_out)
{
    return debug_prune_kmer(S3 == 256, rows, idx, lq, gap_open, gap_extend, 4, S3, flat, offsets, n, table_out, u_out);
}
#define SWG_REFINE4_BATCH 32768u
extern "C" int swg_debug_prune_kmer_refine4(const int8_t *rows, const int8_t *idx, size_t lq, int gap_open, int gap_extend, int S4, const int8_t *flat,
                                            const uint64_t *offsets, size_t n, uint64_t *u_out)
{
    if ((S4 != 128 && S4 != 256) || !rows || lq == 0 || gap_open > 0 || gap_extend > 0 || (n > 0 && (!flat || !offsets || !u_out))) return SWG_ERR_ARG;
    const size_t S = (size_t)S4, C = SWG_KMER_CLASSES;
    std::vector<int8_t> cprof(lq * C);
    swg_kmer_cprof(rows, idx, lq, cprof.data());
    const SwgColMax cm = swg_prune_colmax(rows, idx, lq);
    const int g = std::min(-(gap_open + gap_extend), 65536), e = std::min(-gap_extend, 65536);
    std::vector<size_t> batch{0};
    for (size_t i = 0, blocks = 0; i < n; ++i) {
        const size_t nb = (2 + (size_t)(offsets[i + 1] - offsets[i]) + 3) / 4;
        if (blocks > 0 && blocks + nb > SWG_REFINE4_BATCH) batch.push_back(i), blocks = 0;
        blocks += nb;
    }
    batch.push_back(n);
#pragma omp parallel for schedule(dynamic, 1)
    for (long bi = 0; bi < (long)batch.size() - 1; ++bi) {
        std::vector<uint32_t> held;
        const uint16_t none = 0;
        for (size_t i = batch[bi]; i < batch[bi + 1]; ++i)
            kmer_bound_walk([&](size_t ix) { held.push_back((uint32_t)ix); return &none; }, 5, 1, cm, flat + offsets[i],
                            (size_t)(offsets[i + 1] - offsets[i]));
        std::sort(held.begin(), held.end());
        held.erase(std::unique(held.begin(), held.end()), held.end());
        std::vector<uint16_t> entries(held.size() * S);
        std::vector<int> work(5 * (2 * lq + S));
        uint32_t prev[5] = {0, 0, 0, 0, 0};
        for (size_t h = 0; h < held.size(); ++h) {
            uint32_t c[5];
            for (uint32_t j = 5, v = held[h]; j-- > 0; v /= (uint32_t)C) c[j] = v % (uint32_t)C;
            int d = 0;
            while (h > 0 && d < 4 && c[d] == prev[d]) ++d;
            for (; d < 5; ++d) {
                int *Mn = work.data() + (size_t)d * (2 * lq + S), *Mp = d ? Mn - (2 * lq + S) : nullptr;
                kmer_row(cprof.data(), lq, g, e, S, c[d], Mp, Mp ? Mp + lq : nullptr, Mp ? Mp + 2 * lq : nullptr, Mn, Mn + lq, Mn + 2 * lq);
                prev[d] = c[d];
            }
            const int *best = work.data() + 4 * (2 * lq + S) + 2 * lq;
            for (size_t s = 0; s < S; ++s) entries[h * S + s] = (uint16_t)std::min(best[s], 65535);
        }
        for (size_t i = batch[bi]; i < batch[bi + 1]; ++i)
            u_out[i] = kmer_bound_walk(
                [&](size_t ix) { return entries.data() + (size_t)(std::lower_bound(held.begin(), held.end(), (uint32_t)ix) - held.begin()) * S; }, 5, S, cm,
                flat + offsets[i], (size_t)(offsets[i + 1] - offsets[i]));
    }
    return SWG_OK;
}
extern "C" int swg_debug_prune_table_bits(const int8_t *rows, const int8_t *idx, size_t lq, int k)
{
    if (!rows || lq == 0 || (k != 4 && k != 5)) return SWG_ERR_ARG;
    return swg_kmer_table_bits(swg_prune_colmax(rows, idx, lq), k);
}

struct SwgKmerCandidate {
    int k, S;
    double gain;
    double bound_row;
};
static const SwgKmerCandidate SWG_KMER_CANDIDATES[] = {
    {1, 1, 0.0, 0.0},         {4, 1, 0.1426, 3.1e-12},  {5, 1, 0.2006, 3.1e-12},
    {4, 16, 0.2493, 4.0e-12}, {4, 32, 0.2741, 6.1e-12}, {5, 8, 0.2760, 9.0e-12},
};
int swg_prune_kmer_choice(const SwgKmerAsk &a, int *segments)
{
    int S_out = 1;
    int k = 0;
    if (a.pruned) {
        const bool forced_k = a.forced == 1 || a.forced == 4 || a.forced == 5;
        const long forced_S = a.forced_segments >= 1 && a.forced_segments <= (long)SWG_KMER_MAX_SEGMENTS ? a.forced_segments : 0;
        if (forced_k) {
            k = (int)a.forced;
            S_out = k > 1 && forced_S ? (int)forced_S : 1;
        } else if (a.table_rate <= 0 || a.fill_rate <= 0 || a.lq == 0) {
            k = 1;
        } else {
            auto cost = [&](const SwgKmerCandidate &c) {
                return c.k == 1 ? 0.0 : swg_kmer_table_cells(c.k) * (double)a.lq / a.table_rate + c.bound_row * (double)a.pair_rows;
            };
            auto gain = [&](const SwgKmerCandidate &c) { return c.gain * (double)a.pair_rows / a.fill_rate; };
            const SwgKmerCandidate *cur = &SWG_KMER_CANDIDATES[0];
            for (const SwgKmerCandidate &c : SWG_KMER_CANDIDATES) {
                if (forced_S && c.S != 1) continue;
                if (c.gain > cur->gain && cost(c) - cost(*cur) <= 0.5 * (gain(c) - gain(*cur))) cur = &c;
            }
            k = cur->k, S_out = cur->S;
            if (forced_S && k > 1) {
                if (k == 5 && !swg_kmer_table_admitted(5, forced_S)) k = 4;
                S_out = (int)forced_S;
            }
        }
    }
    if (segments) *segments = k > 1 ? S_out : (k ? 1 : 0);
    return k;
}

static bool debug_kmer_ask(const int64_t *in, int64_t *out, int n_in, SwgKmerAsk *a)
{
// ... 77 lines not shown
    return refine3_pays(a) ? 256 : 0;
}

bool swg_prune_gate_choice(const SwgKmerAsk &a, int k, int S)
{
    if (!a.pruned || k <= 1 || S <= 1 || a.forced_gate == 1) return false;
    if (a.forced_gate == 2) return true;
    if (a.forced != 0 || a.forced_segments != 0) return false;
    return refine3_pays(a);
}

extern "C" int swg_debug_prune_gate_choice(const int64_t *in, int64_t *out)
{
    SwgKmerAsk a;
    if (!debug_kmer_ask(in, out, 8, &a)) return SWG_ERR_ARG;
    if (!swg_prune_gate_value_ok((long)in[8])) return SWG_ERR_ARG;
    a.forced_gate = (long)in[8];
    int S = 0;
    out[0] = swg_prune_kmer_choice(a, &S);
    out[1] = S;
    out[2] = swg_prune_gate_choice(a, (int)out[0], S) ? 1 : 0;
    return SWG_OK;
}

extern "C" int swg_debug_prune_refine3_choice(const int64_t *in, int64_t *out)
{
    SwgKmerAsk a;
    if (!debug_kmer_ask(in, out, 8, &a)) return SWG_ERR_ARG;
    if (!swg_prune_refine3_value_ok((long)in[8]) || (in[9] != 0 && in[9] != 8 && in[9] != 16)) return SWG_ERR_ARG;
    a.forced_refine3 = (long)in[8];
    a.table_bits = in[9] == 16 ? 16 : 8;
    int S = 0;
    out[0] = swg_prune_kmer_choice(a, &S);
    out[1] = S;
    out[2] = swg_prune_refine_choice(a, (int)out[0], S);
    out[3] = swg_prune_refine3_choice(a, (int)out[0], S, (int)out[2]);
    return SWG_OK;
}

#define SWG_REFINE4_GAIN 0.0374
#define SWG_REFINE4_BOUND_ROW 1.31e-12
int swg_prune_refine4_choice(const SwgKmerAsk &a, int k, int S, int S2, int S3)
{
    if (!a.pruned || k < 1 || !swg_kmer_refine4_admitted(a.table_bits5)) return 0;
    if (a.forced_refine4 == SWG_REFINE4_FORCED) return (int)SWG_KMER_REFINE4_SEGMENTS;
    if (a.forced_refine4 != 0 || a.forced != 0 || a.forced_segments != 0 || a.forced_refine != 0 || a.forced_refine3 != 0) return 0;
    if (k != 4 || S <= 1 || S2 != 128 || S3 != 256 || a.table_bits != 8) return 0;
    if (a.table_rate <= 0 || a.fill_rate <= 0 || a.lq == 0) return 0;
    const double cost = swg_kmer_table_cells(5) * (double)a.lq / a.table_rate + SWG_REFINE4_BOUND_ROW * (double)a.pair_rows;
    const double gain = SWG_REFINE4_GAIN * (double)a.pair_rows / a.fill_rate;
    return cost <= 0.5 * gain ? (int)SWG_KMER_REFINE4_SEGMENTS : 0;
}

extern "C" int swg_debug_prune_refine4_choice(const int64_t *in, int64_t *out)
{
    SwgKmerAsk a;
    if (!debug_kmer_ask(in, out, 8, &a)) return SWG_ERR_ARG;
    if (!swg_prune_refine3_value_ok((long)in[8]) || (in[9] != 0 && in[9] != 8 && in[9] != 16)) return SWG_ERR_ARG;
    if (!swg_prune_refine4_value_ok((long)in[10]) || (in[11] != 0 && in[11] != 8 && in[11] != 16)) return SWG_ERR_ARG;
    a.forced_refine3 = (long)in[8], a.forced_refine4 = (long)in[10];
    a.table_bits = in[9] == 16 ? 16 : 8, a.table_bits5 = in[11] == 16 ? 16 : 8;
    int S = 0;
    out[0] = swg_prune_kmer_choice(a, &S);
    out[1] = S;
    out[2] = swg_prune_refine_choice(a, (int)out[0], S);
    out[3] = swg_prune_refine3_choice(a, (int)out[0], S, (int)out[2]);
    out[4] = swg_prune_refine4_choice(a, (int)out[0], S, (int)out[2], (int)out[3]);
    return SWG_OK;
}

uint32_t swg_split_rows(size_t lq, uint64_t qbound)
{
    if (qbound == 0) return 0u;
    return (uint32_t)std::min<uint64_t>(((uint64_t)SWG_F16_CEILING * lq + qbound - 1) / qbound, 1u << 30);
}

void swg_db_split_at(swg_db *db, uint32_t rows)
{
    if (db->split_rows == rows) return;
    const size_t n = db->lens.size();
    const size_t first_short = (size_t)(std::partition_point(db->lens.begin(), db->lens.end(), [rows](uint32_t l) { return l >= rows; }) -
                                        db->lens.begin());
    db->split_rows = rows;
    db->split_pair = (uint32_t)((first_short + 1) / 2);
    uint64_t sum = 0;
    for (size_t i = std::min(n, (size_t)db->split_pair * 2); i < n; ++i) sum += db->lens[i];
    db->split_residues = sum;
}

extern "C" int swg_debug_split(swg_db *db, size_t lq, uint64_t qbound, uint64_t *out)
{
    if (!db || !out || lq == 0 || qbound == 0) return SWG_ERR_ARG;
    const uint32_t rows = swg_split_rows(lq, qbound);
    swg_db_split_at(db, rows);
    out[0] = rows;
    out[1] = db->split_pair;
    out[2] = db->split_residues;
    return SWG_OK;
}

double swg_systolic_estimate_ms(const swg_db *db, size_t lq, int n_cu, int *best_K, bool f16)
{
    *best_K = 0;
    if (db->n_bins == 0 || db->bin_nblk.size() != db->n_bins) return 1e300;
    uint64_t blocks = 0;
    for (uint32_t b : db->bin_nblk) blocks += b;
    const double rows = 4.0 * (double)blocks, longest = 4.0 * (double)db->max_nblk;
    double best = 1e300;
    for (int v = 0; v < swg_num_variants(16); ++v) {
        const SwgKernelInfo info = swg_variant_info(16, v);
        const int W = (int)((lq + (size_t)info.K - 1) / (size_t)info.K);
        if (W > info.max_waves) continue;
        if (info.K > 32) continue;
        const size_t lds = info.lds_per_wave * (size_t)W + info.lds_fixed;
        const int per_cu = swg_workgroups_per_cu(info.max_waves, W, lds);
        const double waves_per_simd = std::max(1.0, per_cu * W / 4.0);
        const double instr = (f16 ? 8.5 : 10.0) * info.K + 12.0;
        const double thr = (rows * W * instr * 4.06 + (double)db->n_bins * W * 5000.0) / (4.0 * n_cu);
        const double wps = std::min(4.0, waves_per_simd);
        const double n_wgs = std::max(1.0, (double)n_cu * per_cu);
// ... 142 lines not shown
```

seq-align-gpu_amd/csrc/swg_host_internal.h:

```cpp
#pragma once
#include "../../include/swg.h"
#include "swg_internal.h"

#include <algorithm>
#include <functional>
#include <map>
#include <memory>
#include <new>
#include <string>
#include <utility>
#include <vector>

template <class T> struct SwgNoInit {
    using value_type = T;
    SwgNoInit() = default;
    template <class U> SwgNoInit(const SwgNoInit<U> &) {}
    T *allocate(size_t n) { return static_cast<T *>(::operator new(n * sizeof(T))); }
    void deallocate(T *p, size_t) { ::operator delete(p); }
    template <class U> void construct(U *p) noexcept { ::new ((void *)p) U; }
    template <class U, class A0, class... A> void construct(U *p, A0 &&a0, A &&...a)
    {
        ::new ((void *)p) U(std::forward<A0>(a0), std::forward<A>(a)...);
    }
    template <class U> bool operator==(const SwgNoInit<U> &) const { return true; }
// ... 128 lines not shown
    uint32_t *d_counters = nullptr;
    uint64_t *d_keys = nullptr;
    uint32_t *d_hist = nullptr;
    uint32_t *d_pair_bound = nullptr;
    std::vector<uint32_t> prune_stages;
};

#define SWG_F16_GAP_MAX 2048
#define SWG_F16_CEILING 4096
#define SWG_I16_CEILING 32767
#define SWG_WIDE_CEILING 65535
inline bool swg_f16_gaps_ok(int go, int ge) { return -go <= SWG_F16_GAP_MAX && -ge <= SWG_F16_GAP_MAX; }

#define SWG_LDS_PER_CU ((size_t)160 * 1024)
inline int swg_workgroups_per_cu(int wave_budget, int W, size_t lds)
{
    return std::max(1, std::min<int>(wave_budget / W, (int)(SWG_LDS_PER_CU / lds)));
}

struct SwgScoreBound {
    uint64_t qbound = 0, bound = 0;
    int smax = 0;
};
SwgScoreBound swg_score_bound(const int8_t *rows, const int8_t *idx, size_t lq, uint64_t longest);
extern "C" int swg_debug_score_bound(const int8_t *rows, const int8_t *idx, size_t lq, uint64_t longest, uint64_t *out);

SwgColMax swg_prune_colmax(const int8_t *rows, const int8_t *idx, size_t lq);
uint64_t swg_prune_bound(const SwgColMax &cm, const int8_t *seq, size_t len);
struct SwgPruneAsk {
    int mode = 1;
    size_t k = 0;
    bool want_scores = false;
    int gap_open = 0, gap_extend = 0;
    int bits = 16;
    bool use_diag = true;
    int n_classes = 1;
    bool work_queue = true;
    bool both_forms = false;
    bool gapless = false;
    bool batch = false;
    uint64_t range_pairs = 0, groups = 0;
    long prune_head = 4;
    size_t n_segments = 1;
    bool fixed = false;
};
struct SwgPrunePlan {
    bool on = false;
    uint32_t head_pairs = 0;
    int kmer = 0;
    int segments = 0;
    int refine = 0;
    int refine3 = 0;
    int refine4 = 0;
    bool prefix_cut = false;
    bool gate = false;
    bool fixed = false;
    uint32_t fixed_T = 0;
};
#define SWG_PRUNE_STAGE_RECS 256u
struct SwgPruneLayout {
    uint32_t *bounds, *ids, *lists, *tiles, *recs;
    size_t words;
};
inline SwgPruneLayout swg_prune_layout(uint32_t *base, size_t n_pairs)
{
    const size_t tiles = 3 * n_pairs, recs = tiles + n_pairs / SWG_PRUNE_TILE + 2;
    auto at = [base](size_t word) { return base ? base + word : nullptr; };
    return SwgPruneLayout{base, at(n_pairs), at(2 * n_pairs), at(tiles), at(recs), recs + 2 * SWG_PRUNE_STAGE_RECS};
}
SwgPrunePlan swg_prune_plan(const SwgPruneAsk &a);
enum : uint32_t {
    SWG_STAGE_THRESHOLD = 1u, SWG_STAGE_PREFIX_CUT = 2u, SWG_STAGE_GATE = 4u, SWG_STAGE_REFINE = 8u, SWG_STAGE_LIST = 16u, SWG_STAGE_REFINE3 = 32u,
    SWG_STAGE_REFINE4 = 64u, SWG_STAGE_BOUND = 128u
};
struct SwgPruneStage {
    uint32_t begin, end;
    uint32_t segment;
    uint32_t queued;
};
std::vector<SwgPruneStage> swg_prune_stages(const SwgPrunePlan &plan, const std::vector<std::pair<uint32_t, uint32_t>> &segments);
#define SWG_PRUNE_NOT_BOUNDED 0xFFFFFFFFu
struct SwgPruneBoundRange {
    size_t stage;
    uint32_t begin, end, skip_begin, skip_end;
};
SwgPruneBoundRange swg_prune_bound_range(const std::vector<SwgPruneStage> &stages, uint32_t n_pairs);
extern "C" int swg_debug_prune_stages(const int64_t *in, int64_t *out, size_t cap, size_t *n_out);
extern "C" int swg_debug_prune_stages3(const int64_t *in, int64_t *out, size_t cap, size_t *n_out);
extern "C" int swg_debug_prune_stages4(const int64_t *in, int64_t *out, size_t cap, size_t *n_out);
extern "C" int swg_debug_prune_stages5(const int64_t *in, int64_t *out, size_t cap, size_t *n_out);
#define SWG_PRUNE_ABOVE_AUTO_PAIRS 16u
inline bool swg_prune_above_auto(uint64_t range_pairs, uint64_t groups) { return range_pairs >= SWG_PRUNE_ABOVE_AUTO_PAIRS * std::max<uint64_t>(1, groups); }
inline int swg_above_multi_route(long option, bool admitted, bool single_pruned)
{
    if (option == 2 || !admitted) return 2;
    if (option == 1) return 1;
    return single_pruned ? 2 : 1;
}
extern "C" int swg_debug_above_multi_route(long option, int admitted, int single_pruned);
extern "C" int swg_debug_prune_bound(const int8_t *rows, const int8_t *idx, size_t lq, const int8_t *flat, const uint64_t *offsets, size_t n,
                                     uint8_t *colmax_out, uint64_t *u_out);
extern "C" int swg_debug_prune_plan(const int64_t *in, int64_t *out);
extern "C" int swg_debug_prune_plan_above(const int64_t *in, int64_t *out);
void swg_kmer_cprof(const int8_t *rows, const int8_t *idx, size_t lq, int8_t *cprof);
void swg_kmer_table_seg(const int8_t *cprof, size_t lq, int g, int e, int k, size_t S, uint16_t *table);
uint64_t swg_kmer_bound_seg(const uint16_t *table, int k, size_t S, const SwgColMax &cm, const int8_t *seq, size_t len);
#define SWG_KMER_TABLE_RATE 4.6e12
#define SWG_KMER_FILL_PASS_RATE 9.4e9
inline double swg_kmer_table_cells(int k)
{
    return k == 5 ? (double)swg_kmer_entries(4) * (4 + SWG_KMER_CLASSES) : (double)swg_kmer_entries(k) * k;
}
inline double swg_kmer_fill_rate(size_t lq) { return SWG_KMER_FILL_PASS_RATE / (double)std::max<size_t>(1, (lq + 511) / 512); }
struct SwgKmerAsk {
    long forced = 0;
    long forced_segments = 0;
    long forced_refine = 0;
    long forced_refine3 = 0;
    long forced_refine4 = 0;
    long forced_gate = 0;
    int table_bits5 = 8;
    int table_bits = 8;
    bool pruned = false;
    size_t lq = 0;
    uint64_t pair_rows = 0;
    double table_rate = SWG_KMER_TABLE_RATE, fill_rate = 0;
};
inline bool swg_kmer_table_admitted(int k, long S)
{
    return S >= 1 && S <= (long)SWG_KMER_MAX_SEGMENTS && swg_kmer_entries(k) * (uint64_t)S * sizeof(uint16_t) <= SWG_KMER_TABLE_BUDGET;
}
int swg_prune_kmer_choice(const SwgKmerAsk &a, int *segments = nullptr);
extern "C" int swg_debug_prune_kmer(const int8_t *rows, const int8_t *idx, size_t lq, int gap_open, int gap_extend, int k, const int8_t *flat,
                                    const uint64_t *offsets, size_t n, uint16_t *table_out, uint64_t *u_out);
extern "C" int swg_debug_prune_kmer_seg(const int8_t *rows, const int8_t *idx, size_t lq, int gap_open, int gap_extend, int k, int S,
                                        const int8_t *flat, const uint64_t *offsets, size_t n, uint16_t *table_out, uint64_t *u_out);
extern "C" int swg_debug_prune_kmer_choice(const int64_t *in, int64_t *out);
extern "C" int swg_debug_prune_kmer_choice_seg(const int64_t *in, int64_t *out);
int swg_prune_refine_choice(const SwgKmerAsk &a, int k, int S);
inline bool swg_prune_refine_value_ok(long v) { return v == 0 || v == 1 || v == 64 || v == 128; }
extern "C" int swg_debug_prune_refine_choice(const int64_t *in, int64_t *out);
extern "C" int swg_debug_prune_kmer_refine(const int8_t *rows, const int8_t *idx, size_t lq, int gap_open, int gap_extend, int S2, const int8_t *flat,
                                           const uint64_t *offsets, size_t n, uint16_t *table_out, uint64_t *u_out);
int swg_prune_refine3_choice(const SwgKmerAsk &a, int k, int S, int S2);
inline bool swg_prune_refine3_value_ok(long v) { return v == 0 || v == 1 || v == 256; }
extern "C" int swg_debug_prune_refine3_choice(const int64_t *in, int64_t *out);
extern "C" int swg_debug_prune_kmer_refine3(const int8_t *rows, const int8_t *idx, size_t lq, int gap_open, int gap_extend, int S3, const int8_t *flat,
                                            const uint64_t *offsets, size_t n, uint16_t *table_out, uint64_t *u_out);
extern "C" int swg_debug_prune_table_bits(const int8_t *rows, const int8_t *idx, size_t lq, int k);
#define SWG_REFINE4_FORCED 5256
int swg_prune_refine4_choice(const SwgKmerAsk &a, int k, int S, int S2, int S3);
inline bool swg_prune_refine4_value_ok(long v) { return v == 0 || v == 1 || v == SWG_REFINE4_FORCED; }
extern "C" int swg_debug_prune_refine4_choice(const int64_t *in, int64_t *out);
extern "C" int swg_debug_prune_kmer_refine4(const int8_t *rows, const int8_t *idx, size_t lq, int gap_open, int gap_extend, int S4, const int8_t *flat,
                                            const uint64_t *offsets, size_t n, uint64_t *u_out);
bool swg_prune_gate_choice(const SwgKmerAsk &a, int k, int S);
inline bool swg_prune_gate_value_ok(long v) { return v == 0 || v == 1 || v == 2; }
extern "C" int swg_debug_prune_gate_choice(const int64_t *in, int64_t *out);
#define SWG_PRUNE_WORD_T 18u
#define SWG_PRUNE_WORD_CUT 20u
#define SWG_ABOVE_WORD_COUNT 24u
#define SWG_PRUNE_WORD_GATE 25u
#define SWG_ABOVE_KEYS_FLOOR SWG_TOPK_CAND_CAP

struct SwgSystolicPlan {
    int bits = 0, variant = 0, K = 0, W = 0, npass = 0, workgroups = 0;
    SwgKernelInfo info = {};
    int f16 = 0;
};

struct SwgSearchPlan {
    int bits = 0;
    bool fast_ok = false;
    int go = 0, ge = 0;
    int go32 = 0, ge32 = 0;
    bool gapless = false;
    bool gapless_cells = false;
    uint64_t score_bound = ~0ull, qbound = 0;
    uint64_t epoch = 0;
    bool use_f16 = false;
    bool wide = false;
    uint32_t split_at = 0, split_rows = 0;
    uint64_t split_residues = 0;
    bool rerun_wide = false;
    int32_t ceiling = 0;
    int32_t level_ceiling = 0;
    bool may_saturate = false;
    bool int32_level = false;
    bool q32_ok = false;
    bool bin32 = false;
    bool some_f16() const { return use_f16 || split_at != 0u; }
    bool use_diag = false, use_diag32 = false, use_q32 = false, exact32 = false;
    SwgDiagWork wk, wk32;
    SwgSystolicPlan main_pl, re_pl;
    int npass32 = 0;
    SwgPrunePlan prune;
};

struct SwgBatchPlan {
    bool one_launch = false;
    int go = 0, ge = 0;
    int form = 0;
    bool qq = false;
    SwgDiagWork wk;
    int qq_per_cu = 1;
    uint64_t bound_max = 0;
    size_t lq_max = 0;
    bool dev_topk = false;
    size_t n_slots = 0;
    size_t chunk_queries = 0, first_chunk = 0;
    size_t grid_rows(size_t Qb) const { return qq ? (Qb + 1) / 2 : Qb; }
    size_t score_rows(size_t Qb) const { return qq ? 2 * grid_rows(Qb) : Qb; }
    size_t score_rows_cap = 0, grid_rows_cap = 0;
    size_t order_entries = 0;
    uint32_t class_queue_dwords = 0;
    size_t rank_word_base = 0, queue_dwords = 0;
    size_t prof_row_bytes[2] = {0, 0};
};

struct SwgKmerTable {
    uint8_t *d = nullptr;
    size_t cap = 0;
    uint64_t epoch = 0;
    int k = 0, segments = 0;
    int bits = 0;
    bool holds(uint64_t e, int k_, int S, int bits_) const { return d && epoch == e && k == k_ && segments == S && bits == bits_; }
};
struct SwgPruneChoice {
    int kmer = 0, segments = 0, refine = 0, refine3 = 0, refine4 = 0;
    int gate = 0;
};

#define SWG_MAX_INFLIGHT 4
struct SwgSlot {
    hipEvent_t ev[8] = {nullptr, nullptr, nullptr, nullptr, nullptr, nullptr, nullptr, nullptr};
    hipEvent_t ev_done = nullptr;
    SwgSearchPlan plan;
    bool side = false;
    bool busy = false;
    swg_db *db = nullptr;
    swg_db::Bufs bufs;
    size_t k = 0, first_chunk = 0;
    bool want_scores = false, dev_topk = false, need_scores = false, two_ends = false;
    int fill_launches = 0;
    bool pruned = false;
    int32_t above_min = 0;
    size_t above_cap = 0;
    int fill_f16_launches = 0;
    swg_stats st;
    uint64_t *h_cand = nullptr;
    uint32_t *h_counters = nullptr;
    int32_t *h_scores = nullptr;
    size_t h_scores_cap = 0;
};

struct SwgBatch16Cache {
    swg_db *db = nullptr;
    size_t slots_cap = 0, pairs_cap = 0, stage_cap = 0;
    uint64_t blocks_cap = 0;
    uint8_t *h_stage = nullptr, *d_stage = nullptr;
    uint8_t *h_meta = nullptr;
    uint64_t *d_pair_src = nullptr;
    uint32_t *d_pair_len = nullptr;
};

struct swg_ctx {
    int device = 0;
    hipStream_t stream = nullptr;
    hipStream_t stream2 = nullptr;
    hipStream_t stream3 = nullptr;
    int n_cu = 0;
    unsigned long n_begun = 0;
    std::string err;
    bool have_scoring = false;
    int8_t sub[32][32];
    int gap_open = 0, gap_extend = 0;
    std::vector<int8_t> query;
    int8_t *h_query_stage[4] = {nullptr, nullptr, nullptr, nullptr};
    size_t h_query_stage_cap[4] = {0, 0, 0, 0};
    hipEvent_t ev_query_stage[4] = {nullptr, nullptr, nullptr, nullptr};
    int query_stage_next = 0;
    std::vector<int8_t> pssm;
    bool query_pssm = false;
    bool gapless = false;
    int32_t above_min = 0;
    size_t query_len() const { return query_pssm ? pssm.size() / 32 : query.size(); }
    long opt_force_bits = 0, opt_cols = 0, opt_max_waves = 0, opt_workgroups = 0, opt_engine = 0, opt_group = 0, opt_long_split = 0, opt_autotune = 1, opt_dynamic = 1, opt_prio_share = 150, opt_long_helps = 0, opt_wide = 1, opt_side_readout = 1, opt_f16 = 1, opt_qq = 1, opt_last_pass = 1, opt_f16_pair = 0;
    long opt_batch_geometry = 0;
    long opt_wave_budget = 0, opt_q32_waves = 0;
    long opt_bounds_groups = 0;
    uint32_t bounds_last[4] = {0, 0, 0, 0};
    long opt_batch = 8, opt_batch_blocks = 0;
    long opt_prune = 1, opt_prune_head = 4;
    bool in_batch = false;
    long opt_above_batch = 0;
    swg_prune_info prune_last = {};
    SwgPruneChoice prune_choice;
    SwgColMax prune_colmax;
    uint64_t prune_colmax_epoch = 0;
    long opt_prune_kmer = 0;
    long opt_prune_segments = 0;
    long opt_prune_refine = 0;
    long opt_prune_refine3 = 0;
    long opt_prune_refine4 = 0;
    long opt_prune_gate = 0;
    long opt_prune_table_bits = 0;
    long opt_prune_cut = 0;
    int8_t *d_kmer_cprof = nullptr;
    size_t d_kmer_cprof_cap = 0;
    SwgKmerTable kmer_first[2], kmer_second, kmer_third, kmer_fourth;
    uint64_t kmer_builds = 0, kmer_refine_builds = 0, kmer_refine3_builds = 0, kmer_refine4_builds = 0;
    bool kmer_fourth_refused = false;
    uint32_t opt_seg_blocks = SWG_DYN_SEG_BLOCKS;
    int8_t *d_sub = nullptr;
    int8_t *d_query = nullptr;
    size_t d_query_cap = 0;
    int8_t *d_pssm = nullptr;
    size_t d_pssm_cap = 0;
    uint8_t *d_profile[8] = {nullptr, nullptr, nullptr, nullptr, nullptr, nullptr, nullptr, nullptr};
    size_t d_profile_cap[8] = {0, 0, 0, 0, 0, 0, 0, 0};
    uint64_t profile_tag[8] = {0, 0, 0, 0, 0, 0, 0, 0};
    uint64_t epoch = 1;
    uint32_t *d_scratch = nullptr;
    size_t d_scratch_cap = 0;
    SwgBatch16Cache b16;
    long opt_calib_seqs = 8192, opt_calib_len = 384, opt_calib_seed = 1;
    struct {
        swg_db *db = nullptr;
        double freq[32] = {};
        long seqs = 0, len = 0, seed = 0;
    } calib;
    std::vector<int32_t> calib_iters;
    long opt_pssm_msa_mb = 1024;
    SwgSlot slots[SWG_MAX_INFLIGHT];
    SwgSlot *cur = nullptr;
    int next_slot = 0;
};

#define SWG_TAKE_HOST_ROUTE 1
int swg_set_global_error(int code, const char *fmt, ...) __attribute__((format(printf, 2, 3)));
int swg_set_ctx_error(swg_ctx *ctx, int code, const char *fmt, ...)
    __attribute__((format(printf, 3, 4)));
void swg_db_release_device(swg_db *db);
void swg_db_release_search_state(swg_db *db);
inline const uint8_t *swg_db_codes(const swg_db *db) { return (db->root ? db->root : db)->codes.data(); }
int swg_view_select(const swg_db *parent, const uint32_t *indices, size_t n, std::vector<uint32_t> *slots,
                    std::vector<uint8_t> *marks = nullptr);
swg_db *swg_view_host(swg_db *parent, const std::vector<uint32_t> &slots);
size_t swg_db_views_alive(const swg_db *db);
extern "C" int swg_debug_view_ranks(const swg_db *db, const uint32_t *indices, size_t n, uint32_t *out, size_t *n_out);
struct SwgListJobs {
    std::vector<uint32_t> slots;
    std::vector<uint64_t> row_pairs;
    std::vector<uint32_t> entry_job;
    std::vector<uint64_t> row_residues;
    std::vector<uint32_t> row_longest;
    std::vector<uint64_t> pair_blocks;
    uint64_t entry0 = 0;
};
int swg_list_jobs(const swg_db *db, const uint32_t *cand, const uint64_t *c_off, size_t q0, size_t nq, SwgListJobs *J);
void swg_lists_deal(const SwgListJobs &J, uint64_t per_wg, uint64_t resident, bool equal_shares, std::vector<uint2> *out);
extern "C" int swg_debug_list_deal(const swg_db *db, const uint32_t *cand, const uint64_t *c_off, size_t n_queries, uint64_t per_wg,
                                   uint64_t resident, uint32_t *out, size_t cap, size_t *n_wgs);
extern "C" int swg_debug_list_jobs(const swg_db *db, const uint32_t *cand, const uint64_t *c_off, size_t n_queries, uint32_t *slots_out,
                                   size_t cap, size_t *n_slots, uint64_t *row_pairs_out);
// ... 102 lines not shown
```

seq-align-gpu_amd/csrc/swg_internal.h:

```cpp
#pragma once
#include <hip/hip_runtime.h>
#include <stdint.h>

#define SWG_BIN 128
#define SWG_ROWS_PER_BLK 4
#define SWG_BIN_COLUMN(s) ((((s)&1u) * 64u) + ((s) >> 1))

struct SwgFillParams {
    const uint32_t *residues;
    const uint64_t *bin_off;
    const uint32_t *bin_nblk;
    uint32_t n_bins;
    const uint8_t *profile;
    int32_t *scores;
    uint32_t *queue;
    const uint32_t *list;
    const uint32_t *list_count;
    uint32_t n_items;
    uint32_t npass;
    int32_t go, ge;
    uint32_t *scratch;
    uint64_t scratch_wg_dwords;
};

// ... 166 lines not shown
                                 uint32_t *d_packed, hipStream_t stream);

hipError_t swg_launch_gather_view(const uint32_t *d_slots, uint32_t n_slots, uint32_t parent_slots, const uint64_t *p_code_off,
                                  const uint32_t *p_lens, const uint32_t *p_order, uint64_t *d_code_off, uint32_t *d_lens,
                                  uint32_t *d_order, hipStream_t stream);

hipError_t swg_launch_zero2(void *a, size_t a_bytes, void *b, size_t b_bytes, hipStream_t stream);
hipError_t swg_launch_collect_flagged_pairs(const int32_t *d_scores, uint32_t first_pair, uint32_t n_pairs, int32_t ceiling,
                                            uint32_t *d_list, uint32_t *d_count, uint32_t *d_seqs, const uint32_t *d_lens,
                                            uint32_t *d_rows16, hipStream_t stream);
hipError_t swg_launch_collect_saturated(const int32_t *d_scores, uint32_t n_slots, int32_t ceiling,
                                        uint32_t *d_list, uint32_t *d_count, const uint32_t *d_lens, uint32_t *d_rows16,
                                        hipStream_t stream);

#define SWG_TOPK_CAND_CAP 8192u
hipError_t swg_launch_topk(const int32_t *d_scores, const uint32_t *d_order, uint32_t n_slots, uint32_t k,
                           uint32_t *d_hist, uint32_t *d_thr, uint64_t *d_cand, uint32_t cap, uint32_t *d_count,
                           hipStream_t stream);
hipError_t swg_launch_above_compact(const int32_t *d_scores, const uint32_t *d_order, uint32_t n_slots, int32_t min_score, uint64_t *d_keys, uint32_t cap,
                                    uint32_t *d_count, hipStream_t stream);
hipError_t swg_launch_above_rows_count(const int32_t *d_scores, uint64_t row_stride, const uint32_t *d_order, uint32_t n_slots, uint32_t n_rows,
                                       const int32_t *d_thr, uint32_t *d_counts, hipStream_t stream);
hipError_t swg_launch_above_rows_scatter(const int32_t *d_scores, uint64_t row_stride, const uint32_t *d_order, uint32_t n_slots, uint32_t n_rows,
                                         const int32_t *d_thr, const uint32_t *d_counts, const uint64_t *d_offsets, uint32_t *d_cursors,
                                         uint64_t *d_keys, uint64_t keys_cap, hipStream_t stream);
struct SwgColMax {
    uint8_t v[32];
};
hipError_t swg_launch_pair_bound(const uint4 *d_tok, const uint32_t *d_pair_off, uint32_t n_pairs, const SwgColMax &cm,
                                 uint32_t *d_bound, uint32_t *d_ids, hipStream_t stream);
#define SWG_KMER_CLASSES 22u
#define SWG_KMER_STD_MASK 0x2DF7BFAu
#define SWG_KMER_PAD_SCORE (-128)
static inline __host__ __device__ uint32_t swg_kmer_class(uint32_t r)
{
    r &= 31u;
    if (r == 0u) return 0u;
    if (!((SWG_KMER_STD_MASK >> r) & 1u)) return SWG_KMER_CLASSES - 1u;
    uint32_t c = 0u;
    for (uint32_t i = 1u; i <= r; ++i) c += (SWG_KMER_STD_MASK >> i) & 1u;
    return c;
}
static inline uint64_t swg_kmer_entries(int k) { return k == 5 ? 5153632ull : k == 4 ? 234256ull : 0ull; }
#define SWG_KMER_MAX_SEGMENTS 32u
#define SWG_KMER_REFINE_SEGMENTS 256u
#define SWG_KMER_TABLE_BUDGET (96ull << 20)
static inline int swg_kmer_table_bits(const SwgColMax &cm, int k)
{
    uint32_t m = 0u;
    for (int r = 0; r < 32; ++r) m = cm.v[r] > m ? cm.v[r] : m;
    return (uint32_t)k * m <= 255u ? 8 : 16;
}
hipError_t swg_launch_kmer_table(const int8_t *d_sub, const int8_t *d_query, const int8_t *d_pssm, uint32_t lq, uint32_t g, uint32_t e,
                                 int k, uint32_t S, int8_t *d_cprof, void *d_table, int bits, hipStream_t stream);
hipError_t swg_launch_pair_bound_kmer(const uint4 *d_tok, const uint32_t *d_pair_off, uint32_t n_pairs, int k, const SwgColMax &cm,
                                      const void *d_table, int bits, uint32_t *d_bound, uint32_t *d_ids, hipStream_t stream);
hipError_t swg_launch_pair_bound_kmer_seg(const uint4 *d_tok, const uint32_t *d_pair_off, uint32_t begin, uint32_t end, int k, uint32_t S, const SwgColMax &cm,
                                          const void *d_table, int bits, const uint32_t *d_thr, uint32_t *d_bound, uint32_t *d_ids, hipStream_t stream);
hipError_t swg_launch_prune_threshold(const int32_t *d_scores, const uint32_t *d_order, uint32_t n_slots, uint32_t k, uint32_t *d_hist,
                                      uint32_t *d_thr, hipStream_t stream);
hipError_t swg_launch_prune_cut(const uint32_t *d_bound, const uint32_t *d_pair_off, uint32_t begin, uint32_t end, const uint32_t *d_thr,
                                uint32_t *d_out, hipStream_t stream);
hipError_t swg_launch_pair_bound_refine(const uint4 *d_tok, const uint32_t *d_pair_off, uint32_t begin, uint32_t end, uint32_t S2, const SwgColMax &cm,
                                        const void *d_table, int bits, const uint32_t *d_thr, uint32_t *d_bound, hipStream_t stream, int k = 4);
#define SWG_KMER_REFINE4_SEGMENTS 256u
#define SWG_KMER_REFINE4_BUDGET (2ull << 30)
static inline bool swg_kmer_refine4_admitted(int bits) { return bits == 8 && swg_kmer_entries(5) * SWG_KMER_REFINE4_SEGMENTS <= SWG_KMER_REFINE4_BUDGET; }
#define SWG_PRUNE_TILE 1024u
hipError_t swg_launch_prune_refine_gate(const uint32_t *d_bound, uint32_t begin, uint32_t end, const uint32_t *d_thr, uint32_t *d_gate, hipStream_t stream);
hipError_t swg_launch_prune_list(const uint32_t *d_bound, const uint32_t *d_pair_off, uint32_t begin, uint32_t end, const uint32_t *d_thr,
                                 uint32_t *d_tiles, uint32_t *d_list, uint32_t *d_out, uint32_t *d_rec, hipStream_t stream);
#define SWG_TOPK_MULTI_CAP 1024u
hipError_t swg_launch_topk_multi(const int32_t *d_scores, uint64_t score_stride, const uint32_t *d_order, uint32_t n_slots,
                                 uint32_t n_queries, uint32_t k, uint32_t *d_hist, uint32_t *d_meta, uint64_t *d_cand, uint32_t cap,
                                 hipStream_t stream);

hipError_t swg_launch_db_composition(const uint32_t *d_codes, const uint64_t *d_code_off, const uint32_t *d_lens, uint32_t n_slots,
                                     unsigned long long *d_counts, hipStream_t stream);
#define SWG_CALIB_BINS 4096u
struct SwgCalibFit {
    double lambda, mu;
    int32_t n_iter, status;
    uint32_t n, reserved;
};
hipError_t swg_launch_calib_fit(const int32_t *d_scores, uint64_t row_stride, const uint32_t *d_order, uint32_t n_slots, uint32_t n_rows,
                                SwgCalibFit *d_out, hipStream_t stream);
```

seq-align-gpu_amd/csrc/swg_kernels.hip:

```cpp
#include "swg_internal.h"
#include <type_traits>

#ifdef SWG_PART
#define SWG_HAS_PART(n) (SWG_PART == (n))
#else
#define SWG_HAS_PART(n) 1
#endif
#ifdef SWG_PROBE_VARIANT
#define SWG_APPLY(X, ...) X(__VA_ARGS__)
#define SWG_DIAG_VARIANTS(X) SWG_APPLY(X, SWG_PROBE_VARIANT)
#else
#define SWG_DIAG_VARIANTS(X)                                                                                          \
    X(24, 16) X(12, 16) X(8, 16) X(16, 16) X(32, 12) X(6, 16) X(10, 16) X(20, 16) X(28, 12) X(4, 16) X(14, 16) X(18, 16) \
    X(22, 16) X(2, 16) X(23, 16) X(21, 16) X(19, 16) X(17, 16) X(15, 16) X(13, 16) X(11, 16) X(9, 16) X(7, 16) X(31, 12)  \
    X(29, 12) X(27, 12) X(25, 12) X(30, 12) X(26, 12) X(5, 16) X(3, 16)
#endif

typedef short s16x2 __attribute__((ext_vector_type(2)));
typedef unsigned short u16x2 __attribute__((ext_vector_type(2)));

#define DEVINL __device__ __forceinline__

DEVINL uint32_t pk_add_i16_sat(uint32_t a, uint32_t b)
{
// ... 2408 lines not shown
#define SWG_KMER_CHUNK 256u
template <int K, class E>
__global__ __launch_bounds__(256) void swg_kmer_table_kernel(const int8_t *cprof, uint32_t lq, int g, int e, uint32_t n_entries, uint32_t S,
                                                             E *table)
{
    constexpr int top = sizeof(E) == 1 ? 255 : 65535;
    __shared__ uint4 rows4[SWG_KMER_CHUNK * 2u];
    const int8_t *rows = reinterpret_cast<const int8_t *>(rows4);
    const uint32_t idx = blockIdx.x * 256u + threadIdx.x;
    uint32_t c[K];
    {
        uint32_t v = idx < n_entries ? idx : 0u;
#pragma unroll
        for (int j = K - 1; j >= 0; --j) {
            c[j] = v % SWG_KMER_CLASSES;
            v /= SWG_KMER_CLASSES;
        }
    }
    int M[K], A[K], best = 0;
#pragma unroll
    for (int j = 0; j < K; ++j) M[j] = 0, A[j] = 0;
    const uint32_t W = (lq + S - 1u) / S;
    E *out = table + (size_t)(idx < n_entries ? idx : 0u) * S;
    uint32_t seg = 0u, seg_end = W < lq ? W : lq;
    for (uint32_t i0 = 0u; i0 < lq; i0 += SWG_KMER_CHUNK) {
        const uint32_t n = lq - i0 < SWG_KMER_CHUNK ? lq - i0 : SWG_KMER_CHUNK;
        __syncthreads();
        for (uint32_t w = threadIdx.x; w < n * 2u; w += 256u) rows4[w] = reinterpret_cast<const uint4 *>(cprof + 32u * (size_t)i0)[w];
        __syncthreads();
        for (uint32_t i = 0u; i < n; ++i) {
            const int8_t *row = rows + 32u * i;
            int diag = 0, left = 0, B = 0;
#pragma unroll
            for (int j = 0; j < K; ++j) {
                const int s = row[c[j]];
                const int a = max(max(M[j] - g, A[j] - e), 0);
                const int b = j ? max(max(left - g, B - e), 0) : 0;
                const int m = max(max(diag + s, a), b);
                diag = M[j];
                M[j] = m, A[j] = a, B = b, left = m;
                best = max(best, m);
            }
            if (i0 + i + 1u == seg_end) {
                if (idx < n_entries) out[seg] = (E)(best > top ? top : best);
                ++seg, best = 0;
                seg_end = seg_end + W < lq ? seg_end + W : lq;
            }
        }
    }
    if (idx < n_entries)
        for (; seg < S; ++seg) out[seg] = 0;
}

template <class E>
__global__ __launch_bounds__(256) void swg_kmer_table5_kernel(const int8_t *cprof, uint32_t lq, int g, int e, uint32_t n_prefixes, uint32_t S,
                                                              E *table)
{
    constexpr int top = sizeof(E) == 1 ? 255 : 65535;
    constexpr int NC = (int)SWG_KMER_CLASSES;
    constexpr uint32_t PACK = 8u / sizeof(E), EB = 8u * sizeof(E);
    __shared__ uint4 rows4[SWG_KMER_CHUNK * 2u];
    const int8_t *rows = reinterpret_cast<const int8_t *>(rows4);
    const uint32_t idx = blockIdx.x * 256u + threadIdx.x;
    const bool mine = idx < n_prefixes;
    uint32_t c[4];
    {
        uint32_t v = mine ? idx : 0u;
#pragma unroll
        for (int j = 3; j >= 0; --j) {
            c[j] = v % SWG_KMER_CLASSES;
            v /= SWG_KMER_CLASSES;
        }
    }
    int M[4], A[4], pbest = 0;
#pragma unroll
    for (int j = 0; j < 4; ++j) M[j] = 0, A[j] = 0;
    int M5[NC], A5[NC], best5[NC];
    uint32_t lo[NC], hi[NC];
#pragma unroll
    for (int k = 0; k < NC; ++k) M5[k] = 0, A5[k] = 0, best5[k] = 0, lo[k] = 0u, hi[k] = 0u;
    const uint32_t W = (lq + S - 1u) / S;
    const bool packed = S % PACK == 0u;
    E *out = table + (size_t)(mine ? idx : 0u) * NC * S;
    uint32_t seg = 0u, seg_end = W < lq ? W : lq;
    auto close_segment = [&](bool zero) {
        const uint32_t slot = seg % PACK;
#pragma unroll
        for (int k = 0; k < NC; ++k) {
            const int b = zero ? 0 : max(pbest, best5[k]);
            const uint32_t v = (uint32_t)(b > top ? top : b);
            best5[k] = 0;
            if (!packed) {
                if (mine) out[(size_t)k * S + seg] = (E)v;
                continue;
            }
            if (slot * EB < 32u) lo[k] |= v << ((slot * EB) & 31u);
            else hi[k] |= v << ((slot * EB) & 31u);
            if (slot == PACK - 1u) {
                if (mine) *reinterpret_cast<uint2 *>(out + (size_t)k * S + (seg - slot)) = make_uint2(lo[k], hi[k]);
                lo[k] = 0u, hi[k] = 0u;
            }
        }
        pbest = 0;
        ++seg;
    };
    for (uint32_t i0 = 0u; i0 < lq; i0 += SWG_KMER_CHUNK) {
        const uint32_t n = lq - i0 < SWG_KMER_CHUNK ? lq - i0 : SWG_KMER_CHUNK;
        __syncthreads();
        for (uint32_t w = threadIdx.x; w < n * 2u; w += 256u) rows4[w] = reinterpret_cast<const uint4 *>(cprof + 32u * (size_t)i0)[w];
        __syncthreads();
        for (uint32_t i = 0u; i < n; ++i) {
            const int8_t *row = rows + 32u * i;
            int diag = 0, left = 0, B = 0;
#pragma unroll
            for (int j = 0; j < 4; ++j) {
                const int s = row[c[j]];
                const int a = max(max(M[j] - g, A[j] - e), 0);
                const int b = j ? max(max(left - g, B - e), 0) : 0;
                const int m = max(max(diag + s, a), b);
                diag = M[j];
                M[j] = m, A[j] = a, B = b, left = m;
                pbest = max(pbest, m);
            }
            const int b5 = max(max(left - g, B - e), 0);
            const uint4 w0 = rows4[2u * i], w1 = rows4[2u * i + 1u];
            const uint32_t w[6] = {w0.x, w0.y, w0.z, w0.w, w1.x, w1.y};
#pragma unroll
            for (int k = 0; k < NC; ++k) {
                const int s = (int)(int8_t)(w[k >> 2] >> (8 * (k & 3)));
                const int a = max(max(M5[k] - g, A5[k] - e), 0);
                const int m = max(max(diag + s, a), b5);
                M5[k] = m, A5[k] = a;
                best5[k] = max(best5[k], m);
            }
            if (i0 + i + 1u == seg_end) {
                close_segment(false);
                seg_end = seg_end + W < lq ? seg_end + W : lq;
            }
        }
    }
    while (seg < S) close_segment(true);
}

hipError_t swg_launch_kmer_table(const int8_t *d_sub, const int8_t *d_query, const int8_t *d_pssm, uint32_t lq, uint32_t g, uint32_t e,
                                 int k, uint32_t S, int8_t *d_cprof, void *d_table, int bits, hipStream_t stream)
{
    const uint32_t n = (uint32_t)swg_kmer_entries(k);
    if (n == 0u || lq == 0u || lq > (1u << 24) || S == 0u || S > SWG_KMER_REFINE_SEGMENTS || (bits != 8 && bits != 16)) return hipErrorInvalidValue;
    const int gi = (int)(g > 65536u ? 65536u : g), ei = (int)(e > 65536u ? 65536u : e);
    hipLaunchKernelGGL(swg_kmer_cprof_kernel, dim3((lq * 32u + 255u) / 256u), dim3(256), 0, stream, d_sub, d_query, d_pssm, lq, d_cprof);
    const dim3 grid((n + 255u) / 256u);
    const uint32_t n4 = (uint32_t)swg_kmer_entries(4);
    if (k == 5 && bits == 8)
        hipLaunchKernelGGL((swg_kmer_table5_kernel<uint8_t>), dim3((n4 + 255u) / 256u), dim3(256), 0, stream, d_cprof, lq, gi, ei, n4, S, static_cast<uint8_t *>(d_table));
    else if (k == 5)
        hipLaunchKernelGGL((swg_kmer_table5_kernel<uint16_t>), dim3((n4 + 255u) / 256u), dim3(256), 0, stream, d_cprof, lq, gi, ei, n4, S, static_cast<uint16_t *>(d_table));
    else if (bits == 8)
        hipLaunchKernelGGL((swg_kmer_table_kernel<4, uint8_t>), grid, dim3(256), 0, stream, d_cprof, lq, gi, ei, n, S, static_cast<uint8_t *>(d_table));
    else
        hipLaunchKernelGGL((swg_kmer_table_kernel<4, uint16_t>), grid, dim3(256), 0, stream, d_cprof, lq, gi, ei, n, S, static_cast<uint16_t *>(d_table));
    return hipGetLastError();
}

template <int K, class E>
__global__ __launch_bounds__(256) void swg_pair_bound_kmer_kernel(const uint4 *tok, const uint32_t *pair_off, uint32_t n_pairs, SwgColMax cm,
                                                                  const E *table, uint32_t *bound, uint32_t *ids)
{
    __shared__ uint32_t lut[32];
    if (threadIdx.x < 32u) lut[threadIdx.x] = swg_kmer_class(threadIdx.x) | (uint32_t)cm.v[threadIdx.x] << 8;
    __syncthreads();
    const uint32_t p = blockIdx.x * 16u + (threadIdx.x >> 4), l = threadIdx.x & 15u;
    const uint32_t C = SWG_KMER_CLASSES;
    auto block4 = [&](uint32_t a, uint32_t b, uint32_t c, uint32_t d) -> uint32_t {
        const uint32_t ix = (((a & 255u) * C + (b & 255u)) * C + (c & 255u)) * C + (d & 255u);
        const uint32_t t = table[K == 5 ? ix * C : ix], u = (a >> 8) + (b >> 8) + (c >> 8) + (d >> 8);
        return t < u ? t : u;
    };
    auto block5 = [&](uint32_t a, uint32_t b, uint32_t c, uint32_t d, uint32_t e) -> uint32_t {
        const uint32_t ix = ((((a & 255u) * C + (b & 255u)) * C + (c & 255u)) * C + (d & 255u)) * C + (e & 255u);
        const uint32_t t = table[ix], u = (a >> 8) + (b >> 8) + (c >> 8) + (d >> 8) + (e >> 8);
        return t < u ? t : u;
    };
    uint32_t ux = 0u, uy = 0u;
    if (p < n_pairs) {
        const uint32_t b0 = pair_off[p], e = pair_off[p + 1u];
        uint32_t tail = b0;
        if (K == 5) {
            const uint32_t groups = (e - b0) / 5u;
            tail = b0 + 5u * groups;
            for (uint32_t gi = l; gi < groups; gi += 16u) {
                uint32_t x[20], y[20];
#pragma unroll
                for (int u = 0; u < 5; ++u) {
                    const uint4 k = tok[b0 + 5u * gi + (uint32_t)u];
                    x[4 * u] = lut[(k.x >> 3) & 31u], x[4 * u + 1] = lut[(k.y >> 3) & 31u], x[4 * u + 2] = lut[(k.z >> 3) & 31u], x[4 * u + 3] = lut[(k.w >> 3) & 31u];
                    y[4 * u] = lut[(k.x >> 11) & 31u], y[4 * u + 1] = lut[(k.y >> 11) & 31u], y[4 * u + 2] = lut[(k.z >> 11) & 31u], y[4 * u + 3] = lut[(k.w >> 11) & 31u];
                }
#pragma unroll
                for (int u = 0; u < 4; ++u) {
                    ux += block5(x[5 * u], x[5 * u + 1], x[5 * u + 2], x[5 * u + 3], x[5 * u + 4]);
                    uy += block5(y[5 * u], y[5 * u + 1], y[5 * u + 2], y[5 * u + 3], y[5 * u + 4]);
                }
            }
        }
        for (uint32_t b = tail + l; b < e; b += 16u) {
            const uint4 k = tok[b];
// ... 369 lines not shown
#pragma unroll
        for (int j = 0; j < PL; ++j) m = hx[j] > m ? hx[j] : m, m = hy[j] > m ? hy[j] : m;
        return (uint32_t)__shfl((int)swg_seg_prefix_max<32>(m, 0u, 0u, 0u), 31, 32);
    };
    const uint32_t b0 = pair_off[p], e = pair_off[p + 1u];
    constexpr int U = 4;
    uint32_t tail = b0;
    if (K == 5) {
        const uint32_t groups = (e - b0) / 5u;
        tail = b0 + 5u * groups;
        for (uint32_t g0 = 0u; g0 < groups; g0 += 32u) {
            uint32_t ux[4] = {0u, 0u, 0u, 0u}, uy[4] = {0u, 0u, 0u, 0u}, uc[4] = {0u, 0u, 0u, 0u};
            if (g0 + l < groups) {
                uint32_t x[20], y[20];
#pragma unroll
                for (int u = 0; u < 5; ++u) {
                    const uint4 k = tok[b0 + 5u * (g0 + l) + (uint32_t)u];
                    x[4 * u] = lut[(k.x >> 3) & 31u], x[4 * u + 1] = lut[(k.y >> 3) & 31u], x[4 * u + 2] = lut[(k.z >> 3) & 31u], x[4 * u + 3] = lut[(k.w >> 3) & 31u];
                    y[4 * u] = lut[(k.x >> 11) & 31u], y[4 * u + 1] = lut[(k.y >> 11) & 31u], y[4 * u + 2] = lut[(k.z >> 11) & 31u], y[4 * u + 3] = lut[(k.w >> 11) & 31u];
                }
#pragma unroll
                for (int u = 0; u < 4; ++u) {
                    uint32_t ix = 0u, iy = 0u, sx = 0u, sy = 0u;
#pragma unroll
                    for (int j = 0; j < 5; ++j) {
                        ix = ix * C + (x[5 * u + j] & 255u), sx += x[5 * u + j] >> 8;
                        iy = iy * C + (y[5 * u + j] & 255u), sy += y[5 * u + j] >> 8;
                    }
                    ux[u] = ix, uy[u] = iy, uc[u] = sx | sy << 16;
                }
            }
            const uint32_t cnt = groups - g0 < 32u ? groups - g0 : 32u;
            for (uint32_t j = 0u; j < cnt; ++j) swg_refine_round<PL, 4, true>(ux, uy, uc, (int)j, tl, S2, hx, hy, m0);
        }
    }
    for (uint32_t t0 = tail; t0 < e; t0 += 32u) {
        uint32_t ux[1] = {0u}, uy[1] = {0u}, uc[1] = {0u};
        if (t0 + l < e) {
            const uint4 k = tok[t0 + l];
            const uint32_t xa = lut[(k.x >> 3) & 31u], xb = lut[(k.y >> 3) & 31u], xc = lut[(k.z >> 3) & 31u], xd = lut[(k.w >> 3) & 31u];
            const uint32_t ya = lut[(k.x >> 11) & 31u], yb = lut[(k.y >> 11) & 31u], yc = lut[(k.z >> 11) & 31u], yd = lut[(k.w >> 11) & 31u];
            const uint32_t ix = (((xa & 255u) * C + (xb & 255u)) * C + (xc & 255u)) * C + (xd & 255u);
            const uint32_t iy = (((ya & 255u) * C + (yb & 255u)) * C + (yc & 255u)) * C + (yd & 255u);
            ux[0] = K == 5 ? ix * C : ix, uy[0] = K == 5 ? iy * C : iy;
            uc[0] = ((xa >> 8) + (xb >> 8) + (xc >> 8) + (xd >> 8)) | ((ya >> 8) + (yb >> 8) + (yc >> 8) + (yd >> 8)) << 16;
        }
        const uint32_t cnt = e - t0 < 32u ? e - t0 : 32u;
        for (uint32_t j0 = 0u; j0 < cnt; j0 += (uint32_t)U) swg_refine_round<PL, U, false>(ux, uy, uc, (int)j0, tl, S2, hx, hy, m0);
    }
    const uint32_t refined = group_max();
    if (l == 0u && refined < first) bound[p] = refined;
}

hipError_t swg_launch_pair_bound_refine(const uint4 *d_tok, const uint32_t *d_pair_off, uint32_t begin, uint32_t end, uint32_t S2, const SwgColMax &cm,
                                        const void *d_table, int bits, const uint32_t *d_thr, uint32_t *d_bound, hipStream_t stream, int k)
{
    if (end < begin || (S2 != 64u && S2 != 128u && S2 != 256u) || (bits != 8 && bits != 16)) return hipErrorInvalidValue;
    if (k != 4 && !(k == 5 && S2 == SWG_KMER_REFINE4_SEGMENTS && bits == 8)) return hipErrorInvalidValue;
    if (end == begin) return hipSuccess;
    const dim3 grid((end - begin + 7u) / 8u);
    const uint8_t *t8 = static_cast<const uint8_t *>(d_table);
    const uint16_t *t16 = static_cast<const uint16_t *>(d_table);
    if (k == 5) {
        hipLaunchKernelGGL((swg_pair_bound_refine_kernel<5, 8, uint8_t>), grid, dim3(256), 0, stream, d_tok, d_pair_off, begin, end, cm, t8, d_thr, d_bound);
        return hipGetLastError();
    }
#define SWG_REFINE_LAUNCH(PL, E, t) \
    hipLaunchKernelGGL((swg_pair_bound_refine_kernel<4, PL, E>), grid, dim3(256), 0, stream, d_tok, d_pair_off, begin, end, cm, t, d_thr, d_bound)
    if (S2 == 256u && bits == 8) SWG_REFINE_LAUNCH(8, uint8_t, t8);
    else if (S2 == 256u) SWG_REFINE_LAUNCH(8, uint16_t, t16);
    else if (S2 == 128u && bits == 8) SWG_REFINE_LAUNCH(4, uint8_t, t8);
    else if (S2 == 128u) SWG_REFINE_LAUNCH(4, uint16_t, t16);
    else if (bits == 8) SWG_REFINE_LAUNCH(2, uint8_t, t8);
    else SWG_REFINE_LAUNCH(2, uint16_t, t16);
#undef SWG_REFINE_LAUNCH
    return hipGetLastError();
}

__global__ __launch_bounds__(1024) void swg_prune_refine_gate_kernel(const uint32_t *bound, uint32_t begin, uint32_t end, const uint32_t *thr,
                                                                     uint32_t *gate)
{
    __shared__ uint32_t s_below[16];
    const uint32_t T = thr[0];
    uint32_t below = 0u;
    for (uint64_t p = (uint64_t)begin + threadIdx.x; p < end; p += 1024u) below += bound[p] < T ? 1u : 0u;
#pragma unroll
    for (int d = 32; d >= 1; d >>= 1) below += (uint32_t)__shfl_xor((int)below, d, 64);
    if ((threadIdx.x & 63u) == 0u) s_below[threadIdx.x >> 6] = below;
    __syncthreads();
    if (threadIdx.x == 0u) {
        uint64_t all = 0u;
        for (uint32_t w = 0u; w < 16u; ++w) all += s_below[w];
        gate[0] = all * 8u >= (uint64_t)(end - begin) && end > begin ? T : 0xFFFFFFFFu;
    }
}

hipError_t swg_launch_prune_refine_gate(const uint32_t *d_bound, uint32_t begin, uint32_t end, const uint32_t *d_thr, uint32_t *d_gate, hipStream_t stream)
{
    if (end < begin) return hipErrorInvalidValue;
    hipLaunchKernelGGL(swg_prune_refine_gate_kernel, dim3(1), dim3(1024), 0, stream, d_bound, begin, end, d_thr, d_gate);
    return hipGetLastError();
}

__device__ __forceinline__ uint32_t swg_prune_tile_keep(const uint32_t *bound, uint32_t begin, uint32_t end, uint32_t T, uint64_t &first)
{
    first = (uint64_t)begin + (uint64_t)blockIdx.x * SWG_PRUNE_TILE + threadIdx.x * 4u;
// ... 467 lines not shown
```

Baseline: 49790.

## Add fifth-level pruning bound using a second k=5 span table

Adds a new fifth-level refinement stage for the pair upper bound. It combines the existing k=5 segment table with a new 'spans' table and a diagonal-gap-aware step function, producing tighter bounds so more database pairs are pruned before the full DP fill. This costs an extra table build, extra device memory, and a heavier refine kernel per surviving pair. It is gated by an auto choice heuristic and an admission check, and it comes with debug hooks.

```diff
diff --git a/seq-align-gpu_amd/__init__.py b/seq-align-gpu_amd/__init__.py
--- a/seq-align-gpu_amd/__init__.py
+++ b/seq-align-gpu_amd/__init__.py
@@ -291,6 +291,11 @@
 _sig("swg_debug_prune_table_bits", C.c_int, [_vp, _vp, C.c_size_t, C.c_int])
 _sig("swg_debug_prune_tables", C.c_int, [_vp, _vp])
 _sig("swg_debug_prune_tables4", C.c_int, [_vp, _vp])
+_sig("swg_debug_prune_kmer_refine5", C.c_int, [_vp, _vp, C.c_size_t, C.c_int, C.c_int, C.c_int, C.c_int, _vp, _vp, C.c_size_t, _vp, _vp])
+_sig("swg_debug_prune_refine5_read", C.c_int, [_vp, _vp, C.c_size_t, _vp])
+_sig("swg_debug_prune_tables5", C.c_int, [_vp, _vp])
+_sig("swg_debug_prune_refine5_choice", C.c_int, [_vp, _vp])
+_sig("swg_debug_prune_stages6", C.c_int, [_vp, _vp, C.c_size_t, _vp])
 _sig("swg_debug_prune_refine4_read", C.c_int, [_vp, _vp, C.c_size_t, _vp])
 _sig("swg_debug_prune_refine4_choice", C.c_int, [_vp, _vp])
 _sig("swg_debug_prune_gate_choice", C.c_int, [_vp, _vp])
@@ -671,6 +676,26 @@
     return u[:n]
 
 
+REFINE5_EXPLICIT = 1
+
+
+def debug_prune_kmer_refine5(rows, query, gap_open, gap_extend, segments, flat, offsets, explicit=0):
+    r, rp = _i8(rows)
+    lq = r.size // 32
+    qp = None
+    if query is not None:
+        q, qp = _i8(query)
+        lq = q.size
+    f, fp = _i8(flat)
+    off = np.ascontiguousarray(offsets, dtype=np.uint64)
+    n = off.size - 1
+    u = np.zeros(max(n, 1), dtype=np.uint64)
+    on = C.c_int(0)
+    _check(lib.swg_debug_prune_kmer_refine5(rp, qp, lq, int(gap_open), int(gap_extend), int(segments), int(explicit), fp, off.ctypes.data_as(_vp), n,
+                                            u.ctypes.data_as(_vp), C.byref(on)))
+    return u[:n] if on.value else None
+
+
 def debug_prune_table_bits(rows, query, k=4):
     r, rp = _i8(rows)
     lq = r.size // 32
@@ -704,6 +729,18 @@
     return tuple(int(v) for v in out)
 
 
+PRUNE_REFINE5_FORCED = 5256
+
+
+def debug_prune_refine5_choice(forced=0, segments=0, refine=0, refine3=0, refine4=0, refine5=0, table_bits=8, table_bits5=8, admitted=True,
+                               fixed=False, pruned=1, lq=3000, pair_rows=1900000000, table_rate=0, fill_rate=0):
+    a = np.array([forced, pruned, lq, pair_rows, table_rate, fill_rate, segments, refine, refine3, table_bits, refine4, table_bits5, refine5,
+                  1 if admitted else 0, 1 if fixed else 0], dtype=np.int64)
+    out = np.zeros(6, dtype=np.int64)
+    _check(lib.swg_debug_prune_refine5_choice(a.ctypes.data_as(_vp), out.ctypes.data_as(_vp)))
+    return tuple(int(v) for v in out)
+
+
 def debug_prune_gate_choice(forced=0, segments=0, gate=0, pruned=1, lq=3000, pair_rows=1900000000, table_rate=0, fill_rate=0):
     a = np.array([forced, pruned, lq, pair_rows, table_rate, fill_rate, segments, 0, gate], dtype=np.int64)
     out = np.zeros(3, dtype=np.int64)
@@ -765,15 +802,16 @@
 
 
 PRUNE_STAGE_QUEUED = ("threshold", "prefix_cut", "gate", "refine", "list")
-_PRUNE_STAGE_BITS = ((0, "threshold"), (7, "bound"), (1, "prefix_cut"), (2, "gate"), (3, "refine"), (5, "refine3"), (6, "refine4"), (4, "list"))
-
-
-def debug_prune_stages(segments, head_pairs=0, fixed=False, refine=0, prefix_cut=False, refine3=0, refine4=0, gate=False):
-    head = [head_pairs, fixed, refine, prefix_cut, refine3, refine4] + ([1] if gate else [])
+_PRUNE_STAGE_BITS = ((0, "threshold"), (7, "bound"), (1, "prefix_cut"), (2, "gate"), (3, "refine"), (5, "refine3"), (6, "refine4"), (8, "refine5"),
+                     (4, "list"))
+
+
+def debug_prune_stages(segments, head_pairs=0, fixed=False, refine=0, prefix_cut=False, refine3=0, refine4=0, gate=False, refine5=0):
+    head = [head_pairs, fixed, refine, prefix_cut, refine3, refine4] + ([1 if gate else 0, refine5] if refine5 else [1] if gate else [])
     a = np.array(head + [len(segments)] + [int(v) for sg in segments for v in sg], dtype=np.int64)
     out = np.zeros((2 * len(segments) + 1, 4), dtype=np.int64)
     n = C.c_size_t(0)
-    hook = lib.swg_debug_prune_stages5 if gate else lib.swg_debug_prune_stages4
+    hook = lib.swg_debug_prune_stages6 if refine5 else lib.swg_debug_prune_stages5 if gate else lib.swg_debug_prune_stages4
     _check(hook(a.ctypes.data_as(_vp), out.ctypes.data_as(_vp), out.shape[0], C.byref(n)))
     return [(int(b), int(e), int(sg), tuple(name for i, name in _PRUNE_STAGE_BITS if int(qd) >> i & 1))
             for b, e, sg, qd in out[:n.value]]
@@ -1512,6 +1550,17 @@
         _check(lib.swg_debug_prune_tables4(self.handle, out.ctypes.data_as(_vp)), self.handle)
         return {"refine4": int(out[0]), "refine4_builds": int(out[1]), "bits": int(out[2]), "refused": bool(out[3])}
 
+    def debug_prune_tables5(self):
+        out = np.zeros(4, dtype=np.int64)
+        _check(lib.swg_debug_prune_tables5(self.handle, out.ctypes.data_as(_vp)), self.handle)
+        return {"refine5": int(out[0]), "refine5_builds": int(out[1]), "bits": int(out[2]), "refused": bool(out[3])}
+
+    def debug_prune_refine5_read(self, blocks):
+        b = np.ascontiguousarray(blocks, dtype=np.uint32)
+        out = np.zeros((max(b.size, 1), KMER_REFINE4_SEGMENTS), dtype=np.uint16)
+        _check(lib.swg_debug_prune_refine5_read(self.handle, b.ctypes.data_as(_vp), b.size, out.ctypes.data_as(_vp)), self.handle)
+        return out[:b.size]
+
     def debug_prune_gate(self):
         out = np.zeros(1, dtype=np.int64)
         _check(lib.swg_debug_prune_gate(self.handle, out.ctypes.data_as(_vp)), self.handle)
diff --git a/seq-align-gpu_amd/csrc/swg_api.cpp b/seq-align-gpu_amd/csrc/swg_api.cpp
--- a/seq-align-gpu_amd/csrc/swg_api.cpp
+++ b/seq-align-gpu_amd/csrc/swg_api.cpp
@@ -215,6 +215,7 @@
     (void)hipFree(ctx->kmer_second.d);
     (void)hipFree(ctx->kmer_third.d);
     (void)hipFree(ctx->kmer_fourth.d);
+    (void)hipFree(ctx->kmer_fifth.d);
     (void)hipFree(ctx->d_profile[0]);
     (void)hipFree(ctx->d_profile[1]);
     (void)hipFree(ctx->d_profile[2]);
@@ -331,6 +332,10 @@
         if (!swg_prune_refine4_value_ok(value))
             return swg_set_ctx_error(ctx, SWG_ERR_ARG, "prune_refine4 must be 0 (auto), 1 (off) or 5256 (the fourth-level bound's table: k = 5 in 256 segments)");
         ctx->opt_prune_refine4 = value;
+    } else if (!strcmp(key, "prune_refine5")) {
+        if (!swg_prune_refine5_value_ok(value))
+            return swg_set_ctx_error(ctx, SWG_ERR_ARG, "prune_refine5 must be 0 (auto), 1 (off) or 5256 (the fifth-level bound: both k = 5 tables in 256 segments)");
+        ctx->opt_prune_refine5 = value;
     } else if (!strcmp(key, "prune_gate")) {
         if (!swg_prune_gate_value_ok(value))
             return swg_set_ctx_error(ctx, SWG_ERR_ARG, "prune_gate must be 0 (auto), 1 (off) or 2 (wherever the first-level bound is a segmented k-mer bound)");
@@ -1171,6 +1176,10 @@
         if (st.queued & SWG_STAGE_REFINE4)
             HIP_TRY(ctx, swg_launch_pair_bound_refine(T.d_tok, T.d_pair_off, st.begin, st.end, (uint32_t)pr.refine4, ctx->prune_colmax, ctx->kmer_fourth.d,
                                                       ctx->kmer_fourth.bits, st.queued & SWG_STAGE_GATE ? gate : thr, L.bounds, qs, 5));
+        if (st.queued & SWG_STAGE_REFINE5)
+            HIP_TRY(ctx, swg_launch_pair_bound_refine5(T.d_tok, T.d_pair_off, st.begin, st.end, ctx->prune_colmax, ctx->kmer_fourth.d, ctx->kmer_fifth.d,
+                                                       (uint32_t)ctx->query_len(), (uint32_t)-(long)ctx->gap_extend, st.queued & SWG_STAGE_GATE ? gate : thr,
+                                                       L.bounds, qs));
         if (st.queued & SWG_STAGE_LIST) {
             const size_t rec = db->prune_stages.size() / 2;
             HIP_TRY(ctx, swg_launch_prune_list(L.bounds, T.d_pair_off, st.begin, st.end, thr, L.tiles, L.lists + st.begin, cut_word,
@@ -2100,13 +2109,17 @@
     P->prune.refine4 = P->prune.prefix_cut || ctx->kmer_fourth_refused
                            ? 0
                            : swg_prune_refine4_choice(ka, P->prune.kmer, P->prune.segments, P->prune.refine, P->prune.refine3);
+    ka.forced_refine5 = ctx->opt_prune_refine5;
+    ka.fixed = P->prune.fixed;
+    ka.refine5_ok = ctx->gap_extend <= 0 && swg_kmer_refine5_admitted(ctx->prune_colmax, (int)std::min<long>(-(long)ctx->gap_extend, 65536), ka.lq);
+    P->prune.refine5 = P->prune.prefix_cut || ctx->kmer_fourth_refused || ctx->kmer_fifth_refused ? 0 : swg_prune_refine5_choice(ka, P->prune.kmer, P->prune.refine4);
     ka.forced_gate = ctx->opt_prune_gate;
     P->prune.gate = !P->prune.prefix_cut && swg_prune_gate_choice(ka, P->prune.kmer, P->prune.segments);
-    ctx->prune_choice = SwgPruneChoice{P->prune.kmer, P->prune.segments, P->prune.refine, P->prune.refine3, P->prune.refine4, P->prune.gate ? 1 : 0};
-    return SWG_OK;
-}
-
-static int ensure_kmer_table(swg_ctx *ctx, SwgKmerTable *t, int k, int S)
+    ctx->prune_choice = SwgPruneChoice{P->prune.kmer, P->prune.segments, P->prune.refine, P->prune.refine3, P->prune.refine4, P->prune.gate ? 1 : 0, P->prune.refine5};
+    return SWG_OK;
+}
+
+static int ensure_kmer_table(swg_ctx *ctx, SwgKmerTable *t, int k, int S, bool spans = false)
 {
     const int bits = kmer_table_bits(ctx, k);
     if (t->holds(ctx->epoch, k, S, bits)) return SWG_OK;
@@ -2118,18 +2131,19 @@
     if ((rc = device_grow(ctx, &t->d, &t->cap, bytes)) != SWG_OK) return rc;
     const long go = (long)ctx->gap_open + ctx->gap_extend, ge = ctx->gap_extend;
     HIP_TRY(ctx, swg_launch_kmer_table(ctx->d_sub, ctx->d_query, ctx->query_pssm ? ctx->d_pssm : nullptr, (uint32_t)lq, (uint32_t)-go, (uint32_t)-ge, k,
-                                       (uint32_t)S, ctx->d_kmer_cprof, t->d, bits, ctx->stream));
+                                       (uint32_t)S, ctx->d_kmer_cprof, t->d, bits, ctx->stream, spans));
     t->epoch = ctx->epoch, t->k = k, t->segments = S, t->bits = bits;
-    ++(t == &ctx->kmer_fourth  ? ctx->kmer_refine4_builds
+    ++(t == &ctx->kmer_fifth   ? ctx->kmer_refine5_builds
+       : t == &ctx->kmer_fourth ? ctx->kmer_refine4_builds
        : t == &ctx->kmer_third ? ctx->kmer_refine3_builds
        : t == &ctx->kmer_second ? ctx->kmer_refine_builds
                                 : ctx->kmer_builds);
     return SWG_OK;
 }
 
-static bool reserve_kmer_fourth(swg_ctx *ctx)
-{
-    SwgKmerTable *t = &ctx->kmer_fourth;
+static bool reserve_kmer_fourth(swg_ctx *ctx, bool fifth = false)
+{
+    SwgKmerTable *t = fifth ? &ctx->kmer_fifth : &ctx->kmer_fourth;
     const size_t bytes = (size_t)swg_kmer_entries(5) * SWG_KMER_REFINE4_SEGMENTS;
     if (t->d && t->cap >= bytes) return true;
     (void)hipFree(t->d);
@@ -2137,7 +2151,7 @@
     uint8_t *d = nullptr;
     if (hipSetDevice(ctx->device) != hipSuccess || hipMalloc(&d, bytes) != hipSuccess) {
         (void)hipGetLastError();
-        ctx->kmer_fourth_refused = true;
+        (fifth ? ctx->kmer_fifth_refused : ctx->kmer_fourth_refused) = true;
         return false;
     }
     t->d = d, t->cap = bytes;
@@ -2168,6 +2182,12 @@
         if (pr.refine4 != (int)SWG_KMER_REFINE4_SEGMENTS || !swg_kmer_refine4_admitted(kmer_table_bits(ctx, 5)))
             return swg_set_ctx_error(ctx, SWG_ERR_ARG, "the fourth-level bound's table: %d segments (256) of bytes", pr.refine4);
         if ((rc = ensure_kmer_table(ctx, &ctx->kmer_fourth, 5, pr.refine4)) != SWG_OK) return rc;
+    }
+    if (pr.refine5) {
+        if (pr.refine5 != (int)SWG_KMER_REFINE4_SEGMENTS || !swg_kmer_refine4_admitted(kmer_table_bits(ctx, 5)))
+            return swg_set_ctx_error(ctx, SWG_ERR_ARG, "the fifth-level bound's tables: %d segments (256) of bytes", pr.refine5);
+        if ((rc = ensure_kmer_table(ctx, &ctx->kmer_fourth, 5, pr.refine5)) != SWG_OK) return rc;
+        if ((rc = ensure_kmer_table(ctx, &ctx->kmer_fifth, 5, pr.refine5, true)) != SWG_OK) return rc;
     }
     swg_db::Bufs &b = db->bufs[ctx->cur - ctx->slots];
     const size_t n_pairs = (size_t)swg_db_pair_count(db);
@@ -2353,6 +2373,7 @@
     if ((rc = plan_search(ctx, db, allow_autotune, &S->plan)) != SWG_OK) return rc;
     if ((rc = plan_prune(ctx, db, want_scores, k, &S->plan)) != SWG_OK) return rc;
     if (S->plan.prune.refine4 && !reserve_kmer_fourth(ctx)) S->plan.prune.refine4 = 0, ctx->prune_choice.refine4 = 0;
+    if (S->plan.prune.refine5 && (!reserve_kmer_fourth(ctx) || !reserve_kmer_fourth(ctx, true))) S->plan.prune.refine5 = 0, ctx->prune_choice.refine5 = 0;
     if ((rc = prepare_search(ctx, db, S->plan)) != SWG_OK) return rc;
     if ((rc = enqueue_fill(ctx, db, S->plan, S)) != SWG_OK) return rc;
     if ((rc = enqueue_rescore(ctx, db, S->plan, S)) != SWG_OK) return rc;
@@ -2669,23 +2690,41 @@
     out[3] = ctx->kmer_fourth_refused ? 1 : 0;
     return SWG_OK;
 }
+extern "C" int swg_debug_prune_tables5(swg_ctx *ctx, int64_t *out)
+{
+    if (!ctx || !out) return swg_set_ctx_error(ctx, SWG_ERR_ARG, "swg_debug_prune_tables5: NULL argument");
+    out[0] = ctx->prune_choice.refine5;
+    out[1] = (int64_t)ctx->kmer_refine5_builds;
+    out[2] = ctx->kmer_fifth.d && ctx->kmer_fifth.epoch == ctx->epoch ? ctx->kmer_fifth.bits : 0;
+    out[3] = ctx->kmer_fifth_refused ? 1 : 0;
+    return SWG_OK;
+}
 extern "C" int swg_debug_prune_gate(swg_ctx *ctx, int64_t *out)
 {
     if (!ctx || !out) return swg_set_ctx_error(ctx, SWG_ERR_ARG, "swg_debug_prune_gate: NULL argument");
     out[0] = ctx->prune_choice.gate;
     return SWG_OK;
 }
+static int debug_prune_refine45_read(swg_ctx *ctx, const SwgKmerTable &t, const uint32_t *blocks, size_t n, uint16_t *out);
 extern "C" int swg_debug_prune_refine4_read(swg_ctx *ctx, const uint32_t *blocks, size_t n, uint16_t *out)
 {
     if (!ctx || (n > 0 && (!blocks || !out))) return swg_set_ctx_error(ctx, SWG_ERR_ARG, "swg_debug_prune_refine4_read: NULL argument");
-    const SwgKmerTable &t = ctx->kmer_fourth;
+    return debug_prune_refine45_read(ctx, ctx->kmer_fourth, blocks, n, out);
+}
+extern "C" int swg_debug_prune_refine5_read(swg_ctx *ctx, const uint32_t *blocks, size_t n, uint16_t *out)
+{
+    if (!ctx || (n > 0 && (!blocks || !out))) return swg_set_ctx_error(ctx, SWG_ERR_ARG, "swg_debug_prune_refine5_read: NULL argument");
+    return debug_prune_refine45_read(ctx, ctx->kmer_fifth, blocks, n, out);
+}
+static int debug_prune_refine45_read(swg_ctx *ctx, const SwgKmerTable &t, const uint32_t *blocks, size_t n, uint16_t *out)
+{
     HIP_TRY(ctx, hipSetDevice(ctx->device));
     HIP_TRY(ctx, hipDeviceSynchronize());
     if (!t.holds(ctx->epoch, 5, (int)SWG_KMER_REFINE4_SEGMENTS, 8))
-        return swg_set_ctx_error(ctx, SWG_ERR_STATE, "swg_debug_prune_refine4_read: no fourth-level table for the current query and scoring");
+        return swg_set_ctx_error(ctx, SWG_ERR_STATE, "no table of 5-residue blocks in 256 segments of this kind for the current query and scoring");
     uint8_t row[SWG_KMER_REFINE4_SEGMENTS];
     for (size_t i = 0; i < n; ++i) {
-        if (blocks[i] >= swg_kmer_entries(5)) return swg_set_ctx_error(ctx, SWG_ERR_ARG, "swg_debug_prune_refine4_read: block %u", blocks[i]);
+        if (blocks[i] >= swg_kmer_entries(5)) return swg_set_ctx_error(ctx, SWG_ERR_ARG, "a table of 5-residue blocks: block %u", blocks[i]);
         HIP_TRY(ctx, hipMemcpy(row, t.d + (size_t)blocks[i] * SWG_KMER_REFINE4_SEGMENTS, sizeof row, hipMemcpyDeviceToHost));
         std::copy(row, row + SWG_KMER_REFINE4_SEGMENTS, out + i * SWG_KMER_REFINE4_SEGMENTS);
     }
diff --git a/seq-align-gpu_amd/csrc/swg_diag_host.cpp b/seq-align-gpu_amd/csrc/swg_diag_host.cpp
--- a/seq-align-gpu_amd/csrc/swg_diag_host.cpp
+++ b/seq-align-gpu_amd/csrc/swg_diag_host.cpp
@@ -567,6 +567,7 @@
             if (plan.refine) q |= SWG_STAGE_REFINE;
             if (plan.refine3) q |= SWG_STAGE_REFINE3;
             if (plan.refine4) q |= SWG_STAGE_REFINE4;
+            if (plan.refine5) q |= SWG_STAGE_REFINE5;
             q |= SWG_STAGE_LIST;
         }
         stages[si].queued = q;
@@ -589,7 +590,8 @@
     plan.head_pairs = (uint32_t)in[0], plan.fixed = in[1] != 0, plan.refine = (int)in[2], plan.prefix_cut = in[3] != 0;
     plan.refine3 = head >= 6 ? (int)in[4] : 0;
     plan.refine4 = head >= 7 ? (int)in[5] : 0;
-    plan.gate = head == 8 && in[6] != 0;
+    plan.gate = head >= 8 && in[6] != 0;
+    plan.refine5 = head >= 9 ? (int)in[7] : 0;
     std::vector<std::pair<uint32_t, uint32_t>> segments;
     for (int64_t i = 0; i < in[head - 1]; ++i) segments.emplace_back((uint32_t)in[head + 2 * i], (uint32_t)in[head + 1 + 2 * i]);
     const std::vector<SwgPruneStage> stages = swg_prune_stages(plan, segments);
@@ -602,6 +604,7 @@
 extern "C" int swg_debug_prune_stages3(const int64_t *in, int64_t *out, size_t cap, size_t *n_out) { return debug_prune_stages(in, 6, out, cap, n_out); }
 extern "C" int swg_debug_prune_stages4(const int64_t *in, int64_t *out, size_t cap, size_t *n_out) { return debug_prune_stages(in, 7, out, cap, n_out); }
 extern "C" int swg_debug_prune_stages5(const int64_t *in, int64_t *out, size_t cap, size_t *n_out) { return debug_prune_stages(in, 8, out, cap, n_out); }
+extern "C" int swg_debug_prune_stages6(const int64_t *in, int64_t *out, size_t cap, size_t *n_out) { return debug_prune_stages(in, 9, out, cap, n_out); }
 
 void swg_kmer_cprof(const int8_t *rows, const int8_t *idx, size_t lq, int8_t *cprof)
 {
@@ -660,26 +663,37 @@
     }
 }
 
-template <class Entries>
-static uint64_t kmer_bound_walk(Entries entries, int k, size_t S, const SwgColMax &cm, const int8_t *seq, size_t len)
+template <class Each>
+static void kmer_blocks(Each each, int k, const SwgColMax &cm, const int8_t *seq, size_t len)
 {
     const size_t n_blocks = (2 + len + 3) / 4, n_rows = 4 * n_blocks;
     auto res = [&](size_t row) -> uint32_t { return row < 2 || row >= 2 + len ? 0u : (uint8_t)seq[row - 2] & 31u; };
     const size_t rows5 = k == 5 ? 20 * (n_blocks / 5) : 0;
-    std::vector<uint64_t> H(S, 0);
     for (size_t r = 0; r < n_rows;) {
         const size_t rows = r < rows5 ? 5 : 4;
         size_t ix = 0;
-        uint64_t sum = 0, run = 0;
+        uint64_t sum = 0;
         for (size_t j = 0; j < rows; ++j) ix = ix * SWG_KMER_CLASSES + swg_kmer_class(res(r + j)), sum += cm.v[res(r + j)];
         if (k == 5 && rows == 4) ix *= SWG_KMER_CLASSES;
-        const uint16_t *t = entries(ix);
-        for (size_t s = 0; s < S; ++s) {
-            run = std::max(run, H[s]);
-            H[s] = run + std::min<uint64_t>(t[s], sum);
-        }
+        each(ix, sum);
         r += rows;
     }
+}
+
+template <class Entries>
+static uint64_t kmer_bound_walk(Entries entries, int k, size_t S, const SwgColMax &cm, const int8_t *seq, size_t len)
+{
+    std::vector<uint64_t> H(S, 0);
+    kmer_blocks(
+        [&](size_t ix, uint64_t sum) {
+            const uint16_t *t = entries(ix);
+            uint64_t run = 0;
+            for (size_t s = 0; s < S; ++s) {
+                run = std::max(run, H[s]);
+                H[s] = run + std::min<uint64_t>(t[s], sum);
+            }
+        },
+        k, cm, seq, len);
     return *std::max_element(H.begin(), H.end());
 }
 
@@ -726,6 +740,48 @@
     return debug_prune_kmer(S3 == 256, rows, idx, lq, gap_open, gap_extend, 4, S3, flat, offsets, n, table_out, u_out);
 }
 #define SWG_REFINE4_BATCH 32768u
+static std::vector<size_t> refine4_batches(const uint64_t *offsets, size_t n)
+{
+    std::vector<size_t> batch{0};
+    for (size_t i = 0, blocks = 0; i < n; ++i) {
+        const size_t nb = (2 + (size_t)(offsets[i + 1] - offsets[i]) + 3) / 4;
+        if (blocks > 0 && blocks + nb > SWG_REFINE4_BATCH) batch.push_back(i), blocks = 0;
+        blocks += nb;
+    }
+    batch.push_back(n);
+    return batch;
+}
+static std::vector<uint32_t> refine4_held(const SwgColMax &cm, const int8_t *flat, const uint64_t *offsets, size_t first, size_t last)
+{
+    std::vector<uint32_t> held;
+    for (size_t i = first; i < last; ++i)
+        kmer_blocks([&](size_t ix, uint64_t) { held.push_back((uint32_t)ix); }, 5, cm, flat + offsets[i], (size_t)(offsets[i + 1] - offsets[i]));
+    std::sort(held.begin(), held.end());
+    held.erase(std::unique(held.begin(), held.end()), held.end());
+    return held;
+}
+template <class Row>
+static std::vector<uint16_t> refine4_entries(Row row, const std::vector<uint32_t> &held, const int8_t *cprof, size_t lq, int g, int e, size_t S)
+{
+    const uint32_t C = SWG_KMER_CLASSES;
+    std::vector<uint16_t> entries(held.size() * S);
+    std::vector<int> work(5 * (2 * lq + S));
+    uint32_t prev[5] = {0, 0, 0, 0, 0};
+    for (size_t h = 0; h < held.size(); ++h) {
+        uint32_t c[5];
+        for (uint32_t j = 5, v = held[h]; j-- > 0; v /= C) c[j] = v % C;
+        int d = 0;
+        while (h > 0 && d < 4 && c[d] == prev[d]) ++d;
+        for (; d < 5; ++d) {
+            int *Mn = work.data() + (size_t)d * (2 * lq + S), *Mp = d ? Mn - (2 * lq + S) : nullptr;
+            row(cprof, lq, g, e, S, c[d], Mp, Mp ? Mp + lq : nullptr, Mp ? Mp + 2 * lq : nullptr, Mn, Mn + lq, Mn + 2 * lq);
+            prev[d] = c[d];
+        }
+        const int *best = work.data() + 4 * (2 * lq + S) + 2 * lq;
+        for (size_t s = 0; s < S; ++s) entries[h * S + s] = (uint16_t)std::min(best[s], 65535);
+    }
+    return entries;
+}
 extern "C" int swg_debug_prune_kmer_refine4(const int8_t *rows, const int8_t *idx, size_t lq, int gap_open, int gap_extend, int S4, const int8_t *flat,
                                             const uint64_t *offsets, size_t n, uint64_t *u_out)
 {
@@ -735,42 +791,87 @@
     swg_kmer_cprof(rows, idx, lq, cprof.data());
     const SwgColMax cm = swg_prune_colmax(rows, idx, lq);
     const int g = std::min(-(gap_open + gap_extend), 65536), e = std::min(-gap_extend, 65536);
-    std::vector<size_t> batch{0};
-    for (size_t i = 0, blocks = 0; i < n; ++i) {
-        const size_t nb = (2 + (size_t)(offsets[i + 1] - offsets[i]) + 3) / 4;
-        if (blocks > 0 && blocks + nb > SWG_REFINE4_BATCH) batch.push_back(i), blocks = 0;
-        blocks += nb;
-    }
-    batch.push_back(n);
+    const std::vector<size_t> batch = refine4_batches(offsets, n);
 #pragma omp parallel for schedule(dynamic, 1)
     for (long bi = 0; bi < (long)batch.size() - 1; ++bi) {
-        std::vector<uint32_t> held;
-        const uint16_t none = 0;
-        for (size_t i = batch[bi]; i < batch[bi + 1]; ++i)
-            kmer_bound_walk([&](size_t ix) { held.push_back((uint32_t)ix); return &none; }, 5, 1, cm, flat + offsets[i],
-                            (size_t)(offsets[i + 1] - offsets[i]));
-        std::sort(held.begin(), held.end());
-        held.erase(std::unique(held.begin(), held.end()), held.end());
-        std::vector<uint16_t> entries(held.size() * S);
-        std::vector<int> work(5 * (2 * lq + S));
-        uint32_t prev[5] = {0, 0, 0, 0, 0};
-        for (size_t h = 0; h < held.size(); ++h) {
-            uint32_t c[5];
-            for (uint32_t j = 5, v = held[h]; j-- > 0; v /= (uint32_t)C) c[j] = v % (uint32_t)C;
-            int d = 0;
-            while (h > 0 && d < 4 && c[d] == prev[d]) ++d;
-            for (; d < 5; ++d) {
-                int *Mn = work.data() + (size_t)d * (2 * lq + S), *Mp = d ? Mn - (2 * lq + S) : nullptr;
-                kmer_row(cprof.data(), lq, g, e, S, c[d], Mp, Mp ? Mp + lq : nullptr, Mp ? Mp + 2 * lq : nullptr, Mn, Mn + lq, Mn + 2 * lq);
-                prev[d] = c[d];
-            }
-            const int *best = work.data() + 4 * (2 * lq + S) + 2 * lq;
-            for (size_t s = 0; s < S; ++s) entries[h * S + s] = (uint16_t)std::min(best[s], 65535);
-        }
+        const std::vector<uint32_t> held = refine4_held(cm, flat, offsets, batch[bi], batch[bi + 1]);
+        const std::vector<uint16_t> entries = refine4_entries(kmer_row, held, cprof.data(), lq, g, e, S);
         for (size_t i = batch[bi]; i < batch[bi + 1]; ++i)
             u_out[i] = kmer_bound_walk(
                 [&](size_t ix) { return entries.data() + (size_t)(std::lower_bound(held.begin(), held.end(), (uint32_t)ix) - held.begin()) * S; }, 5, S, cm,
                 flat + offsets[i], (size_t)(offsets[i + 1] - offsets[i]));
+    }
+    return SWG_OK;
+}
+
+static void kmer_row2(const int8_t *cprof, size_t lq, int g, int e, size_t S, uint32_t c, const int *Mp, const int *Bp, const int *best_p, int *Mn,
+                      int *Bn, int *best)
+{
+    const size_t W = (lq + S - 1) / S;
+    int a = SWG_KMER_NO_CHAIN, up = SWG_KMER_NO_CHAIN;
+    for (size_t s = 0; s < S; ++s) best[s] = best_p ? best_p[s] : 0;
+    for (size_t s = 0, i = 0; i < lq; ++s) {
+        int bs = best[s];
+        for (const size_t end = std::min(lq, i + W); i < end; ++i) {
+            const int sc = cprof[SWG_KMER_CLASSES * i + c];
+            a = std::max(std::max(up - (g - e), a), SWG_KMER_NO_CHAIN);
+            const int b = Mp ? std::max(std::max(Mp[i] - g, Bp[i] - e), SWG_KMER_NO_CHAIN) : SWG_KMER_NO_CHAIN;
+            const int diag = Mp && i ? Mp[i - 1] : SWG_KMER_NO_CHAIN;
+            const int h = sc + std::max(0, diag + e);
+            const int m = std::max(std::max(h, a), b);
+            Mn[i] = m, Bn[i] = b, up = m;
+            bs = std::max(bs, h);
+        }
+        best[s] = bs;
+    }
+}
+
+static uint64_t kmer_bound_walk5(const uint16_t *t, const uint16_t *t2, const std::vector<uint32_t> &held, size_t S, size_t W, int e, size_t N,
+                                 const SwgColMax &cm, const int8_t *seq, size_t len)
+{
+    const int64_t c = (int64_t)e * (int64_t)W;
+    std::vector<int64_t> H(S, 0), Hn(S), PH(S), PC(S);
+    kmer_blocks(
+        [&](size_t ix, uint64_t sum) {
+            const size_t at = (size_t)(std::lower_bound(held.begin(), held.end(), (uint32_t)ix) - held.begin()) * S;
+            for (size_t s = 0; s < S; ++s) {
+                PH[s] = std::max(s ? PH[s - 1] : 0, H[s]);
+                PC[s] = std::max(s ? PC[s - 1] : INT64_MIN, H[s] + c * (int64_t)s);
+            }
+            for (size_t s = 0; s < S; ++s) {
+                const int64_t tm = (int64_t)std::min<uint64_t>(t[at + s], sum), v2 = t2[at + s];
+                int64_t best = std::max(H[s], std::max(H[s], s ? H[s - 1] : 0) + tm);
+                for (size_t n = 1; n <= N && n + 1 <= s; ++n) best = std::max(best, H[s - 1 - n] + std::min(tm, v2 - c * (int64_t)n));
+                if (s >= N + 2) best = std::max(best, std::min(tm + PH[s - 2 - N], v2 - c * (int64_t)(s - 1) + PC[s - 2 - N]));
+                Hn[s] = best;
+            }
+            H.swap(Hn);
+        },
+        5, cm, seq, len);
+    return (uint64_t)*std::max_element(H.begin(), H.end());
+}
+
+extern "C" int swg_debug_prune_kmer_refine5(const int8_t *rows, const int8_t *idx, size_t lq, int gap_open, int gap_extend, int S5, int n_explicit,
+                                            const int8_t *flat, const uint64_t *offsets, size_t n, uint64_t *u_out, int *on_out)
+{
+    if (S5 != 256 || n_explicit < 0 || !rows || lq == 0 || gap_open > 0 || gap_extend > 0 || !on_out || (n > 0 && (!flat || !offsets || !u_out)))
+        return SWG_ERR_ARG;
+    const size_t S = (size_t)S5, C = SWG_KMER_CLASSES, W = (lq + S - 1) / S;
+    const SwgColMax cm = swg_prune_colmax(rows, idx, lq);
+    const int g = std::min(-(gap_open + gap_extend), 65536), e = std::min(-gap_extend, 65536);
+    *on_out = swg_kmer_refine5_admitted(cm, e, lq) ? 1 : 0;
+    if (!*on_out) return SWG_OK;
+    std::vector<int8_t> cprof(lq * C);
+    swg_kmer_cprof(rows, idx, lq, cprof.data());
+    const std::vector<size_t> batch = refine4_batches(offsets, n);
+#pragma omp parallel for schedule(dynamic, 1)
+    for (long bi = 0; bi < (long)batch.size() - 1; ++bi) {
+        const std::vector<uint32_t> held = refine4_held(cm, flat, offsets, batch[bi], batch[bi + 1]);
+        const std::vector<uint16_t> t = refine4_entries(kmer_row, held, cprof.data(), lq, g, e, S);
+        const std::vector<uint16_t> t2 = refine4_entries(kmer_row2, held, cprof.data(), lq, g, e, S);
+        for (size_t i = batch[bi]; i < batch[bi + 1]; ++i)
+            u_out[i] = kmer_bound_walk5(t.data(), t2.data(), held, S, W, e, n_explicit ? (size_t)n_explicit : (size_t)SWG_REFINE5_EXPLICIT, cm,
+                                        flat + offsets[i], (size_t)(offsets[i + 1] - offsets[i]));
     }
     return SWG_OK;
 }
@@ -954,6 +1055,19 @@
     return cost <= 0.5 * gain ? (int)SWG_KMER_REFINE4_SEGMENTS : 0;
 }
 
+#define SWG_REFINE5_GAIN 0.0254
+#define SWG_REFINE5_BOUND_ROW 4.0e-12
+int swg_prune_refine5_choice(const SwgKmerAsk &a, int k, int S4)
+{
+    if (!a.pruned || k < 1 || !a.refine5_ok || !swg_kmer_refine4_admitted(a.table_bits5)) return 0;
+    if (a.forced_refine5 == SWG_REFINE5_FORCED) return (int)SWG_KMER_REFINE4_SEGMENTS;
+    if (a.forced_refine5 != 0 || a.forced_refine4 != 0 || S4 == 0 || a.fixed) return 0;
+    if (a.table_rate <= 0 || a.fill_rate <= 0 || a.lq == 0) return 0;
+    const double cost = swg_kmer_table_cells(5) * (double)a.lq / a.table_rate + SWG_REFINE5_BOUND_ROW * (double)a.pair_rows;
+    const double gain = SWG_REFINE5_GAIN * (double)a.pair_rows / a.fill_rate;
+    return cost <= 0.5 * gain ? (int)SWG_KMER_REFINE4_SEGMENTS : 0;
+}
+
 extern "C" int swg_debug_prune_refine4_choice(const int64_t *in, int64_t *out)
 {
     SwgKmerAsk a;
@@ -968,6 +1082,19 @@
     out[2] = swg_prune_refine_choice(a, (int)out[0], S);
     out[3] = swg_prune_refine3_choice(a, (int)out[0], S, (int)out[2]);
     out[4] = swg_prune_refine4_choice(a, (int)out[0], S, (int)out[2], (int)out[3]);
+    return SWG_OK;
+}
+
+extern "C" int swg_debug_prune_refine5_choice(const int64_t *in, int64_t *out)
+{
+    SwgKmerAsk a;
+    if (!debug_kmer_ask(in, out, 8, &a)) return SWG_ERR_ARG;
+    if (!swg_prune_refine5_value_ok((long)in[12]) || (in[13] != 0 && in[13] != 1) || (in[14] != 0 && in[14] != 1)) return SWG_ERR_ARG;
+    const int rc = swg_debug_prune_refine4_choice(in, out);
+    if (rc != SWG_OK) return rc;
+    a.forced_refine3 = (long)in[8], a.forced_refine4 = (long)in[10], a.forced_refine5 = (long)in[12];
+    a.table_bits = in[9] == 16 ? 16 : 8, a.table_bits5 = in[11] == 16 ? 16 : 8, a.refine5_ok = in[13] != 0, a.fixed = in[14] != 0;
+    out[5] = swg_prune_refine5_choice(a, (int)out[0], (int)out[4]);
     return SWG_OK;
 }
 
diff --git a/seq-align-gpu_amd/csrc/swg_host_internal.h b/seq-align-gpu_amd/csrc/swg_host_internal.h
--- a/seq-align-gpu_amd/csrc/swg_host_internal.h
+++ b/seq-align-gpu_amd/csrc/swg_host_internal.h
@@ -204,6 +204,7 @@
     int refine = 0;
     int refine3 = 0;
     int refine4 = 0;
+    int refine5 = 0;
     bool prefix_cut = false;
     bool gate = false;
     bool fixed = false;
@@ -223,7 +224,7 @@
 SwgPrunePlan swg_prune_plan(const SwgPruneAsk &a);
 enum : uint32_t {
     SWG_STAGE_THRESHOLD = 1u, SWG_STAGE_PREFIX_CUT = 2u, SWG_STAGE_GATE = 4u, SWG_STAGE_REFINE = 8u, SWG_STAGE_LIST = 16u, SWG_STAGE_REFINE3 = 32u,
-    SWG_STAGE_REFINE4 = 64u, SWG_STAGE_BOUND = 128u
+    SWG_STAGE_REFINE4 = 64u, SWG_STAGE_BOUND = 128u, SWG_STAGE_REFINE5 = 256u
 };
 struct SwgPruneStage {
     uint32_t begin, end;
@@ -241,6 +242,7 @@
 extern "C" int swg_debug_prune_stages3(const int64_t *in, int64_t *out, size_t cap, size_t *n_out);
 extern "C" int swg_debug_prune_stages4(const int64_t *in, int64_t *out, size_t cap, size_t *n_out);
 extern "C" int swg_debug_prune_stages5(const int64_t *in, int64_t *out, size_t cap, size_t *n_out);
+extern "C" int swg_debug_prune_stages6(const int64_t *in, int64_t *out, size_t cap, size_t *n_out);
 #define SWG_PRUNE_ABOVE_AUTO_PAIRS 16u
 inline bool swg_prune_above_auto(uint64_t range_pairs, uint64_t groups) { return range_pairs >= SWG_PRUNE_ABOVE_AUTO_PAIRS * std::max<uint64_t>(1, groups); }
 inline int swg_above_multi_route(long option, bool admitted, bool single_pruned)
@@ -270,6 +272,9 @@
     long forced_refine = 0;
     long forced_refine3 = 0;
     long forced_refine4 = 0;
+    long forced_refine5 = 0;
+    bool refine5_ok = false;
+    bool fixed = false;
     long forced_gate = 0;
     int table_bits5 = 8;
     int table_bits = 8;
@@ -306,6 +311,12 @@
 extern "C" int swg_debug_prune_refine4_choice(const int64_t *in, int64_t *out);
 extern "C" int swg_debug_prune_kmer_refine4(const int8_t *rows, const int8_t *idx, size_t lq, int gap_open, int gap_extend, int S4, const int8_t *flat,
                                             const uint64_t *offsets, size_t n, uint64_t *u_out);
+extern "C" int swg_debug_prune_kmer_refine5(const int8_t *rows, const int8_t *idx, size_t lq, int gap_open, int gap_extend, int S5, int n_explicit,
+                                            const int8_t *flat, const uint64_t *offsets, size_t n, uint64_t *u_out, int *on_out);
+#define SWG_REFINE5_FORCED 5256
+int swg_prune_refine5_choice(const SwgKmerAsk &a, int k, int S4);
+inline bool swg_prune_refine5_value_ok(long v) { return v == 0 || v == 1 || v == SWG_REFINE5_FORCED; }
+extern "C" int swg_debug_prune_refine5_choice(const int64_t *in, int64_t *out);
 bool swg_prune_gate_choice(const SwgKmerAsk &a, int k, int S);
 inline bool swg_prune_gate_value_ok(long v) { return v == 0 || v == 1 || v == 2; }
 extern "C" int swg_debug_prune_gate_choice(const int64_t *in, int64_t *out);
@@ -381,6 +392,7 @@
 struct SwgPruneChoice {
     int kmer = 0, segments = 0, refine = 0, refine3 = 0, refine4 = 0;
     int gate = 0;
+    int refine5 = 0;
 };
 
 #define SWG_MAX_INFLIGHT 4
@@ -455,6 +467,7 @@
     long opt_prune_refine = 0;
     long opt_prune_refine3 = 0;
     long opt_prune_refine4 = 0;
+    long opt_prune_refine5 = 0;
     long opt_prune_gate = 0;
     long opt_prune_table_bits = 0;
     long opt_prune_cut = 0;
@@ -463,6 +476,9 @@
     SwgKmerTable kmer_first[2], kmer_second, kmer_third, kmer_fourth;
     uint64_t kmer_builds = 0, kmer_refine_builds = 0, kmer_refine3_builds = 0, kmer_refine4_builds = 0;
     bool kmer_fourth_refused = false;
+    SwgKmerTable kmer_fifth;
+    uint64_t kmer_refine5_builds = 0;
+    bool kmer_fifth_refused = false;
     uint32_t opt_seg_blocks = SWG_DYN_SEG_BLOCKS;
     int8_t *d_sub = nullptr;
     int8_t *d_query = nullptr;
diff --git a/seq-align-gpu_amd/csrc/swg_internal.h b/seq-align-gpu_amd/csrc/swg_internal.h
--- a/seq-align-gpu_amd/csrc/swg_internal.h
+++ b/seq-align-gpu_amd/csrc/swg_internal.h
@@ -242,7 +242,7 @@
     return (uint32_t)k * m <= 255u ? 8 : 16;
 }
 hipError_t swg_launch_kmer_table(const int8_t *d_sub, const int8_t *d_query, const int8_t *d_pssm, uint32_t lq, uint32_t g, uint32_t e,
-                                 int k, uint32_t S, int8_t *d_cprof, void *d_table, int bits, hipStream_t stream);
+                                 int k, uint32_t S, int8_t *d_cprof, void *d_table, int bits, hipStream_t stream, bool spans = false);
 hipError_t swg_launch_pair_bound_kmer(const uint4 *d_tok, const uint32_t *d_pair_off, uint32_t n_pairs, int k, const SwgColMax &cm,
                                       const void *d_table, int bits, uint32_t *d_bound, uint32_t *d_ids, hipStream_t stream);
 hipError_t swg_launch_pair_bound_kmer_seg(const uint4 *d_tok, const uint32_t *d_pair_off, uint32_t begin, uint32_t end, int k, uint32_t S, const SwgColMax &cm,
@@ -256,6 +256,18 @@
 #define SWG_KMER_REFINE4_SEGMENTS 256u
 #define SWG_KMER_REFINE4_BUDGET (2ull << 30)
 static inline bool swg_kmer_refine4_admitted(int bits) { return bits == 8 && swg_kmer_entries(5) * SWG_KMER_REFINE4_SEGMENTS <= SWG_KMER_REFINE4_BUDGET; }
+#define SWG_REFINE5_EXPLICIT 1
+#define SWG_KMER_NO_CHAIN (-(1 << 28))
+static inline bool swg_kmer_refine5_admitted(const SwgColMax &cm, int e, size_t lq)
+{
+    uint32_t m = 0u;
+    for (int r = 0; r < 32; ++r) m = cm.v[r] > m ? cm.v[r] : m;
+    return e > 0 && e <= 255 && 5u * (m + (uint32_t)e) <= 255u && (uint64_t)e * lq < (1ull << 24);
+}
+hipError_t swg_launch_pair_bound_refine5(const uint4 *d_tok, const uint32_t *d_pair_off, uint32_t begin, uint32_t end, const SwgColMax &cm,
+                                         const uint8_t *d_table, const uint8_t *d_table2, uint32_t lq, uint32_t e, const uint32_t *d_thr, uint32_t *d_bound,
+                                         hipStream_t stream);
+
 #define SWG_PRUNE_TILE 1024u
 hipError_t swg_launch_prune_refine_gate(const uint32_t *d_bound, uint32_t begin, uint32_t end, const uint32_t *d_thr, uint32_t *d_gate, hipStream_t stream);
 hipError_t swg_launch_prune_list(const uint32_t *d_bound, const uint32_t *d_pair_off, uint32_t begin, uint32_t end, const uint32_t *d_thr,
diff --git a/seq-align-gpu_amd/csrc/swg_kernels.hip b/seq-align-gpu_amd/csrc/swg_kernels.hip
--- a/seq-align-gpu_amd/csrc/swg_kernels.hip
+++ b/seq-align-gpu_amd/csrc/swg_kernels.hip
@@ -2484,13 +2484,15 @@
         for (; seg < S; ++seg) out[seg] = 0;
 }
 
-template <class E>
+template <class E, bool SPAN = false>
 __global__ __launch_bounds__(256) void swg_kmer_table5_kernel(const int8_t *cprof, uint32_t lq, int g, int e, uint32_t n_prefixes, uint32_t S,
                                                               E *table)
 {
     constexpr int top = sizeof(E) == 1 ? 255 : 65535;
     constexpr int NC = (int)SWG_KMER_CLASSES;
     constexpr uint32_t PACK = 8u / sizeof(E), EB = 8u * sizeof(E);
+    constexpr int none = SPAN ? SWG_KMER_NO_CHAIN : 0;
+    const int ga = SPAN ? g - e : g, ea = SPAN ? 0 : e;
     __shared__ uint4 rows4[SWG_KMER_CHUNK * 2u];
     const int8_t *rows = reinterpret_cast<const int8_t *>(rows4);
     const uint32_t idx = blockIdx.x * 256u + threadIdx.x;
@@ -2506,11 +2508,11 @@
     }
     int M[4], A[4], pbest = 0;
 #pragma unroll
-    for (int j = 0; j < 4; ++j) M[j] = 0, A[j] = 0;
+    for (int j = 0; j < 4; ++j) M[j] = none, A[j] = none;
     int M5[NC], A5[NC], best5[NC];
     uint32_t lo[NC], hi[NC];
 #pragma unroll
-    for (int k = 0; k < NC; ++k) M5[k] = 0, A5[k] = 0, best5[k] = 0, lo[k] = 0u, hi[k] = 0u;
+    for (int k = 0; k < NC; ++k) M5[k] = none, A5[k] = none, best5[k] = 0, lo[k] = 0u, hi[k] = 0u;
     const uint32_t W = (lq + S - 1u) / S;
     const bool packed = S % PACK == 0u;
     E *out = table + (size_t)(mine ? idx : 0u) * NC * S;
@@ -2543,27 +2545,29 @@
         __syncthreads();
         for (uint32_t i = 0u; i < n; ++i) {
             const int8_t *row = rows + 32u * i;
-            int diag = 0, left = 0, B = 0;
+            int diag = none, left = none, B = none;
 #pragma unroll
             for (int j = 0; j < 4; ++j) {
                 const int s = row[c[j]];
-                const int a = max(max(M[j] - g, A[j] - e), 0);
-                const int b = j ? max(max(left - g, B - e), 0) : 0;
-                const int m = max(max(diag + s, a), b);
+                const int a = max(max(M[j] - ga, A[j] - ea), none);
+                const int b = j ? max(max(left - g, B - e), none) : none;
+                const int h = SPAN ? s + max(diag + e, 0) : diag + s;
+                const int m = max(max(h, a), b);
                 diag = M[j];
                 M[j] = m, A[j] = a, B = b, left = m;
-                pbest = max(pbest, m);
-            }
-            const int b5 = max(max(left - g, B - e), 0);
+                pbest = max(pbest, SPAN ? h : m);
+            }
+            const int b5 = max(max(left - g, B - e), none);
             const uint4 w0 = rows4[2u * i], w1 = rows4[2u * i + 1u];
             const uint32_t w[6] = {w0.x, w0.y, w0.z, w0.w, w1.x, w1.y};
 #pragma unroll
             for (int k = 0; k < NC; ++k) {
                 const int s = (int)(int8_t)(w[k >> 2] >> (8 * (k & 3)));
-                const int a = max(max(M5[k] - g, A5[k] - e), 0);
-                const int m = max(max(diag + s, a), b5);
+                const int a = max(max(M5[k] - ga, A5[k] - ea), none);
+                const int h = SPAN ? s + max(diag + e, 0) : diag + s;
+                const int m = max(max(h, a), b5);
                 M5[k] = m, A5[k] = a;
-                best5[k] = max(best5[k], m);
+                best5[k] = max(best5[k], SPAN ? h : m);
             }
             if (i0 + i + 1u == seg_end) {
                 close_segment(false);
@@ -2575,15 +2579,18 @@
 }
 
 hipError_t swg_launch_kmer_table(const int8_t *d_sub, const int8_t *d_query, const int8_t *d_pssm, uint32_t lq, uint32_t g, uint32_t e,
-                                 int k, uint32_t S, int8_t *d_cprof, void *d_table, int bits, hipStream_t stream)
+                                 int k, uint32_t S, int8_t *d_cprof, void *d_table, int bits, hipStream_t stream, bool spans)
 {
     const uint32_t n = (uint32_t)swg_kmer_entries(k);
     if (n == 0u || lq == 0u || lq > (1u << 24) || S == 0u || S > SWG_KMER_REFINE_SEGMENTS || (bits != 8 && bits != 16)) return hipErrorInvalidValue;
+    if (spans && (k != 5 || bits != 8 || e == 0u || e > 255u)) return hipErrorInvalidValue;
     const int gi = (int)(g > 65536u ? 65536u : g), ei = (int)(e > 65536u ? 65536u : e);
     hipLaunchKernelGGL(swg_kmer_cprof_kernel, dim3((lq * 32u + 255u) / 256u), dim3(256), 0, stream, d_sub, d_query, d_pssm, lq, d_cprof);
     const dim3 grid((n + 255u) / 256u);
     const uint32_t n4 = (uint32_t)swg_kmer_entries(4);
-    if (k == 5 && bits == 8)
+    if (spans)
+        hipLaunchKernelGGL((swg_kmer_table5_kernel<uint8_t, true>), dim3((n4 + 255u) / 256u), dim3(256), 0, stream, d_cprof, lq, gi, ei, n4, S, static_cast<uint8_t *>(d_table));
+    else if (k == 5 && bits == 8)
         hipLaunchKernelGGL((swg_kmer_table5_kernel<uint8_t>), dim3((n4 + 255u) / 256u), dim3(256), 0, stream, d_cprof, lq, gi, ei, n4, S, static_cast<uint8_t *>(d_table));
     else if (k == 5)
         hipLaunchKernelGGL((swg_kmer_table5_kernel<uint16_t>), dim3((n4 + 255u) / 256u), dim3(256), 0, stream, d_cprof, lq, gi, ei, n4, S, static_cast<uint16_t *>(d_table));
@@ -3059,6 +3066,148 @@
     if (l == 0u && refined < first) bound[p] = refined;
 }
 
+template <int N>
+__device__ __forceinline__ void swg_refine_step5(uint32_t (&h)[8], uint2 wt, uint2 wt2, uint32_t cs, uint32_t m0, int c, int cl)
+{
+    static_assert(N >= 0 && N + 2 <= 8, "what a segment needs from below comes from its own lane and the one below it");
+    auto below = [&](uint32_t v) { return (uint32_t)__builtin_amdgcn_update_dpp(0, (int)v, 0x138, 0xf, 0xf, true) & m0; };
+    uint32_t ph[8], pc[8];
+    ph[0] = h[0], pc[0] = h[0] + (uint32_t)cl;
+#pragma unroll
+    for (int j = 1; j < 8; ++j) {
+        const uint32_t v = h[j] + (uint32_t)(cl + c * j);
+        ph[j] = h[j] > ph[j - 1] ? h[j] : ph[j - 1];
+        pc[j] = v > pc[j - 1] ? v : pc[j - 1];
+    }
+    const uint32_t exh = swg_seg_prefix_max<32>(below(ph[7]), 0u, 0u, 0u), exc = swg_seg_prefix_max<32>(below(pc[7]), 0u, 0u, 0u);
+#pragma unroll
+    for (int j = 0; j < 8; ++j) ph[j] = exh > ph[j] ? exh : ph[j], pc[j] = exc > pc[j] ? exc : pc[j];
+    uint32_t qh[N + 1], qph[N + 2], qpc[N + 2];
+#pragma unroll
+    for (int i = 0; i < N + 1; ++i) qh[i] = below(h[7 - i]);
+#pragma unroll
+    for (int i = 0; i < N + 2; ++i) qph[i] = below(ph[7 - i]), qpc[i] = below(pc[7 - i]);
+    uint32_t hn[8];
+#pragma unroll
+    for (int j = 0; j < 8; ++j) {
+        const uint32_t wa = j < 4 ? wt.x : wt.y, wb = j < 4 ? wt2.x : wt2.y;
+        const uint32_t en = (wa >> (8 * (j & 3))) & 0xFFu;
+        const int tm = (int)(en < cs ? en : cs), t2 = (int)((wb >> (8 * (j & 3))) & 0xFFu);
+        const uint32_t h1 = j >= 1 ? h[j - 1] : qh[0];
+        int best = (int)(h[j] > h1 ? h[j] : h1) + tm;
+#pragma unroll
+        for (int n = 1; n <= N; ++n) {
+            const int hb = (int)(j - 1 - n >= 0 ? h[j - 1 - n >= 0 ? j - 1 - n : 0] : qh[n - j >= 0 && n - j <= N ? n - j : 0]);
+            best = max(best, hb + min(tm, t2 - c * n));
+        }
+        constexpr int D = N + 2;
+        const int fh = (int)(j >= D ? ph[j >= D ? j - D : 0] : qph[j < D ? D - 1 - j : 0]);
+        const int fc = (int)(j >= D ? pc[j >= D ? j - D : 0] : qpc[j < D ? D - 1 - j : 0]);
+        best = max(best, min(tm + fh, t2 - (cl + c * j - c) + fc));
+        hn[j] = (uint32_t)best;
+    }
+#pragma unroll
+    for (int j = 0; j < 8; ++j) h[j] = hn[j];
+}
+
+template <int U, bool ONE_UNIT>
+__device__ __forceinline__ void swg_refine_round5(const uint32_t (&ux)[ONE_UNIT ? U : 1], const uint32_t (&uy)[ONE_UNIT ? U : 1],
+                                                  const uint32_t (&uc)[ONE_UNIT ? U : 1], int src, const uint8_t *tl, const uint8_t *tl2, uint32_t (&hx)[8],
+                                                  uint32_t (&hy)[8], uint32_t m0, int c, int cl)
+{
+    uint2 tx[U], ty[U], sx[U], sy[U];
+    uint32_t cs[U];
+#pragma unroll
+    for (int u = 0; u < U; ++u) {
+        const int from = ONE_UNIT ? src : src + u, b = ONE_UNIT ? u : 0;
+        const uint32_t ix = (uint32_t)__shfl((int)ux[b], from, 32), iy = (uint32_t)__shfl((int)uy[b], from, 32);
+        cs[u] = (uint32_t)__shfl((int)uc[b], from, 32);
+        tx[u] = *reinterpret_cast<const uint2 *>(tl + (size_t)ix * 256u), sx[u] = *reinterpret_cast<const uint2 *>(tl2 + (size_t)ix * 256u);
+        ty[u] = *reinterpret_cast<const uint2 *>(tl + (size_t)iy * 256u), sy[u] = *reinterpret_cast<const uint2 *>(tl2 + (size_t)iy * 256u);
+    }
+#pragma unroll
+    for (int u = 0; u < U; ++u) {
+        swg_refine_step5<SWG_REFINE5_EXPLICIT>(hx, tx[u], sx[u], cs[u] & 0xFFFFu, m0, c, cl);
+        swg_refine_step5<SWG_REFINE5_EXPLICIT>(hy, ty[u], sy[u], cs[u] >> 16, m0, c, cl);
+    }
+}
+
+__global__ __launch_bounds__(256) __attribute__((amdgpu_waves_per_eu(4, 4))) void swg_pair_bound_refine5_kernel(const uint4 *tok, const uint32_t *pair_off, uint32_t begin, uint32_t end, SwgColMax cm,
+                                                                     const uint8_t *table, const uint8_t *table2, int c, const uint32_t *thr,
+                                                                     uint32_t *bound)
+{
+    __shared__ uint32_t lut[32];
+    if (threadIdx.x < 32u) lut[threadIdx.x] = swg_kmer_class(threadIdx.x) | (uint32_t)cm.v[threadIdx.x] << 8;
+    __syncthreads();
+    const uint32_t p = begin + blockIdx.x * 8u + (threadIdx.x >> 5), l = threadIdx.x & 31u;
+    if (p >= end) return;
+    const uint32_t T = thr[0], first = bound[p];
+    if (first < T) return;
+    const uint32_t C = SWG_KMER_CLASSES;
+    const uint8_t *tl = table + l * 8u, *tl2 = table2 + l * 8u;
+    const uint32_t m0 = l >= 1u ? 0xFFFFFFFFu : 0u;
+    const int cl = c * 8 * (int)l;
+    uint32_t hx[8], hy[8];
+#pragma unroll
+    for (int j = 0; j < 8; ++j) hx[j] = 0u, hy[j] = 0u;
+    const uint32_t b0 = pair_off[p], e = pair_off[p + 1u];
+    const uint32_t groups = (e - b0) / 5u, tail = b0 + 5u * groups;
+    for (uint32_t g0 = 0u; g0 < groups; g0 += 32u) {
+        uint32_t ux[4] = {0u, 0u, 0u, 0u}, uy[4] = {0u, 0u, 0u, 0u}, uc[4] = {0u, 0u, 0u, 0u};
+        if (g0 + l < groups) {
+            uint32_t x[20], y[20];
+#pragma unroll
+            for (int u = 0; u < 5; ++u) {
+                const uint4 k = tok[b0 + 5u * (g0 + l) + (uint32_t)u];
+                x[4 * u] = lut[(k.x >> 3) & 31u], x[4 * u + 1] = lut[(k.y >> 3) & 31u], x[4 * u + 2] = lut[(k.z >> 3) & 31u], x[4 * u + 3] = lut[(k.w >> 3) & 31u];
+                y[4 * u] = lut[(k.x >> 11) & 31u], y[4 * u + 1] = lut[(k.y >> 11) & 31u], y[4 * u + 2] = lut[(k.z >> 11) & 31u], y[4 * u + 3] = lut[(k.w >> 11) & 31u];
+            }
+#pragma unroll
+            for (int u = 0; u < 4; ++u) {
+                uint32_t ix = 0u, iy = 0u, sx = 0u, sy = 0u;
+#pragma unroll
+                for (int j = 0; j < 5; ++j) {
+                    ix = ix * C + (x[5 * u + j] & 255u), sx += x[5 * u + j] >> 8;
+                    iy = iy * C + (y[5 * u + j] & 255u), sy += y[5 * u + j] >> 8;
+                }
+                ux[u] = ix, uy[u] = iy, uc[u] = sx | sy << 16;
+            }
+        }
+        const uint32_t cnt = groups - g0 < 32u ? groups - g0 : 32u;
+        for (uint32_t j = 0u; j < cnt; ++j) swg_refine_round5<4, true>(ux, uy, uc, (int)j, tl, tl2, hx, hy, m0, c, cl);
+    }
+    for (uint32_t t0 = tail; t0 < e; t0 += 32u) {
+        uint32_t ux[1] = {0u}, uy[1] = {0u}, uc[1] = {0u};
+        if (t0 + l < e) {
+            const uint4 k = tok[t0 + l];
+            const uint32_t xa = lut[(k.x >> 3) & 31u], xb = lut[(k.y >> 3) & 31u], xc = lut[(k.z >> 3) & 31u], xd = lut[(k.w >> 3) & 31u];
+            const uint32_t ya = lut[(k.x >> 11) & 31u], yb = lut[(k.y >> 11) & 31u], yc = lut[(k.z >> 11) & 31u], yd = lut[(k.w >> 11) & 31u];
+            ux[0] = ((((xa & 255u) * C + (xb & 255u)) * C + (xc & 255u)) * C + (xd & 255u)) * C;
+            uy[0] = ((((ya & 255u) * C + (yb & 255u)) * C + (yc & 255u)) * C + (yd & 255u)) * C;
+            uc[0] = ((xa >> 8) + (xb >> 8) + (xc >> 8) + (xd >> 8)) | ((ya >> 8) + (yb >> 8) + (yc >> 8) + (yd >> 8)) << 16;
+        }
+        const uint32_t cnt = e - t0 < 32u ? e - t0 : 32u;
+        for (uint32_t j0 = 0u; j0 < cnt; j0 += 4u) swg_refine_round5<4, false>(ux, uy, uc, (int)j0, tl, tl2, hx, hy, m0, c, cl);
+    }
+    uint32_t m = 0u;
+#pragma unroll
+    for (int j = 0; j < 8; ++j) m = hx[j] > m ? hx[j] : m, m = hy[j] > m ? hy[j] : m;
+    const uint32_t refined = (uint32_t)__shfl((int)swg_seg_prefix_max<32>(m, 0u, 0u, 0u), 31, 32);
+    if (l == 0u && refined < first) bound[p] = refined;
+}
+
+hipError_t swg_launch_pair_bound_refine5(const uint4 *d_tok, const uint32_t *d_pair_off, uint32_t begin, uint32_t end, const SwgColMax &cm,
+                                         const uint8_t *d_table, const uint8_t *d_table2, uint32_t lq, uint32_t e, const uint32_t *d_thr, uint32_t *d_bound,
+                                         hipStream_t stream)
+{
+    if (end < begin || !swg_kmer_refine5_admitted(cm, (int)(e > 65536u ? 65536u : e), lq)) return hipErrorInvalidValue;
+    if (end == begin) return hipSuccess;
+    const uint32_t W = (lq + SWG_KMER_REFINE4_SEGMENTS - 1u) / SWG_KMER_REFINE4_SEGMENTS;
+    hipLaunchKernelGGL(swg_pair_bound_refine5_kernel, dim3((end - begin + 7u) / 8u), dim3(256), 0, stream, d_tok, d_pair_off, begin, end, cm, d_table, d_table2,
+                       (int)(e * W), d_thr, d_bound);
+    return hipGetLastError();
+}
+
 hipError_t swg_launch_pair_bound_refine(const uint4 *d_tok, const uint32_t *d_pair_off, uint32_t begin, uint32_t end, uint32_t S2, const SwgColMax &cm,
                                         const void *d_table, int bits, const uint32_t *d_thr, uint32_t *d_bound, hipStream_t stream, int k)
 {
```

Result: faster. 55890, median of 6 (+12.2%).
